# timlawrenz/DINO-X

Measured on AMD Instinct MI355X. Metric: training images/sec (source samples; 2 global views each) ViT-S/16 224px bs256/GPU, higher is better.
Workload: dtype bf16; 1 GPU; ViT-S/16 224x224x3 2.5D slice stacks, scale-aware, 2 views/sample, DINO+Gram loss, AdamW+EMA; per_gpu_batch=256, global_batch=256, local_crops=0, out_dim=8192, parallelism=dp1, hipgraph=False

## Files before the change

### dino-x_amd/csrc/block.hip

```cpp
#include <cstring>

#include "common.h"

using namespace dinox;

namespace {

dinox_gemm_args gemm_args(const void* A, const void* B, void* C, int64_t M, int64_t N, int64_t K, int out_dtype) {
  dinox_gemm_args g;
  memset(&g, 0, sizeof g);
  g.A = A; g.B = B; g.C = C;
  g.M = M; g.N = N; g.K = K;
  g.lda = K; g.ldb = K; g.ldc = N;
  g.batch = 1;
  g.strideC = M * N;
  g.in_dtype = DINOX_BF16;
  g.out_dtype = out_dtype;
  g.alpha = 1.0f;
  g.ldr = N;
  g.ldaux = N;
  return g;
}

int weight_grad(const void* dy, const void* x, float* dw, float* db, int64_t M, int64_t n_out, int64_t n_in, void* ws, int64_t ws_bytes, void* stream) {
  dinox_gemm_args g;
  memset(&g, 0, sizeof g);
  g.A = dy; g.B = x; g.C = dw;
  g.M = n_out; g.N = n_in; g.K = M;
  g.lda = n_out; g.ldb = n_in; g.ldc = n_in;
  g.batch = 1;
  g.strideC = n_out * n_in;
  g.transA = 1; g.transB = 1;
  g.in_dtype = DINOX_BF16;
  g.out_dtype = DINOX_F32;
  g.epilogue = DINOX_EPI_ACCUM;
  g.alpha = 1.0f;
  g.ldr = n_in;
  g.ldaux = n_in;
  g.colsum = db;
  const int64_t need = dinox_gemm_ws_bytes(&g);
  if (need > 0) {
    DX_REQUIRE(ws && need <= ws_bytes, DINOX_EINVAL, "block_backward: tn_ws of %lld bytes, the dW product [%lld x %lld] over %lld rows needs %lld",
               (long long)ws_bytes, (long long)n_out, (long long)n_in, (long long)M, (long long)need);
    g.ws = ws;
  }
  return dinox_gemm(&g, stream);
}

}

#define BLK_TRY(call)        \
  do {                       \
    const int rc_ = (call);  \
    if (rc_) return rc_;     \
  } while (0)

extern "C" int dinox_block_forward(const dinox_block_fwd_args* a, void* stream) {
  DX_REQUIRE(a, DINOX_EINVAL, "block_forward: null args");
  DX_REQUIRE(a->V > 0 && a->N > 0 && a->D > 0 && a->H > 0 && a->heads > 0 && a->D % a->heads == 0, DINOX_EINVAL,
             "block_forward: V=%lld N=%lld D=%d H=%d heads=%d", (long long)a->V, (long long)a->N, a->D, a->H, a->heads);
  DX_REQUIRE(a->x0 && a->o && a->x1 && a->xn2 && a->mean2 && a->rstd2 && a->act && a->x2, DINOX_EINVAL, "block_forward: null activation");
  DX_REQUIRE(a->qkv ? a->lse != nullptr : !a->train, DINOX_EINVAL, "block_forward: qkv / lse buffers (only a no-grad pass may leave qkv out)");
  DX_REQUIRE(a->n1w && a->n1b && a->n2w && a->n2b && a->wqkv && a->wproj && a->w1 && a->w2, DINOX_EINVAL, "block_forward: null parameter");
  DX_REQUIRE(a->xn1_in ? (a->mean1_in && a->rstd1_in) : (a->xn1 && a->mean1 && a->rstd1), DINOX_EINVAL, "block_forward: norm1 buffers");
  DX_REQUIRE(!a->next_g || (a->next_b && a->yn && a->meann && a->rstdn), DINOX_EINVAL, "block_forward: next LayerNorm buffers");
  DX_REQUIRE(!a->train || a->pre, DINOX_EINVAL, "block_forward: train without the side tensor");
  const int64_t M = a->V * a->N;
  const int D = a->D, H = a->H;
  const void* xn1 = a->xn1_in;
  if (!xn1) {
    BLK_TRY(dinox_layernorm_fwd(a->x0, a->n1w, a->n1b, a->xn1, a->mean1, a->rstd1, M, D, a->eps, DINOX_BF16, stream));
    xn1 = a->xn1;
  }
  if (!a->qkv) {
    BLK_TRY(dinox_qkv_attention_fwd(xn1, a->wqkv, a->bqkv, a->o, nullptr, a->lse, (int)a->V, (int)a->N, a->heads, D / a->heads, D, stream));
  } else {
    dinox_gemm_args g = gemm_args(xn1, a->wqkv, a->qkv, M, 3 * (int64_t)D, D, DINOX_BF16);
    if (a->bqkv) { g.epilogue |= DINOX_EPI_BIAS; g.bias = a->bqkv; }
    BLK_TRY(dinox_gemm(&g, stream));
    BLK_TRY(dinox_attention_fwd(a->qkv, a->o, a->lse, (int)a->V, (int)a->N, a->heads, D / a->heads, DINOX_BF16, stream));
  }
  if (a->fuse_proj_ln) {
    BLK_TRY(dinox_linear_residual_ln(a->o, a->wproj, a->bproj, a->x0, a->x1, a->n2w, a->n2b, a->eps, a->xn2, DINOX_BF16, a->mean2, a->rstd2, M, D, D, stream));
  } else {
    dinox_gemm_args g = gemm_args(a->o, a->wproj, a->x1, M, D, D, DINOX_F32);
    g.epilogue = DINOX_EPI_RESIDUAL | (a->bproj ? DINOX_EPI_BIAS : 0);
    g.bias = a->bproj;
    g.residual = a->x0;
    BLK_TRY(dinox_gemm(&g, stream));
    BLK_TRY(dinox_layernorm_fwd(a->x1, a->n2w, a->n2b, a->xn2, a->mean2, a->rstd2, M, D, a->eps, DINOX_BF16, stream));
  }
  {
    dinox_gemm_args g = gemm_args(a->xn2, a->w1, a->act, M, H, D, DINOX_BF16);
    g.epilogue = DINOX_EPI_GELU | DINOX_EPI_AUXGRAD | (a->b1 ? DINOX_EPI_BIAS : 0);
    g.bias = a->b1;
    g.aux = a->train ? a->pre : nullptr;
    BLK_TRY(dinox_gemm(&g, stream));
  }
  if (a->next_g && a->fuse_fc2_ln) {
    BLK_TRY(dinox_linear_residual_ln(a->act, a->w2, a->b2, a->x1, a->x2, a->next_g, a->next_b, a->next_eps, a->yn, a->next_dtype, a->meann, a->rstdn, M, D, H, stream));
  } else {
    dinox_gemm_args g = gemm_args(a->act, a->w2, a->x2, M, D, H, DINOX_F32);
    g.epilogue = DINOX_EPI_RESIDUAL | (a->b2 ? DINOX_EPI_BIAS : 0);
    g.bias = a->b2;
    g.residual = a->x1;
    BLK_TRY(dinox_gemm(&g, stream));
    if (a->next_g) BLK_TRY(dinox_layernorm_fwd(a->x2, a->next_g, a->next_b, a->yn, a->meann, a->rstdn, M, D, a->next_eps, a->next_dtype, stream));
  }
  return 0;
}

extern "C" int dinox_block_backward(const dinox_block_bwd_args* a, void* stream) {
  DX_REQUIRE(a, DINOX_EINVAL, "block_backward: null args");
  DX_REQUIRE(a->V > 0 && a->N > 0 && a->D > 0 && a->H > 0 && a->heads > 0 && a->D % a->heads == 0, DINOX_EINVAL,
             "block_backward: V=%lld N=%lld D=%d H=%d heads=%d", (long long)a->V, (long long)a->N, a->D, a->H, a->heads);
  DX_REQUIRE(a->g && (a->g_lowp || a->g_lowp_buf), DINOX_EINVAL, "block_backward: gradient");
  DX_REQUIRE(a->x0 && a->x1 && a->xn1 && a->xn2 && a->qkv && a->o && a->lse && a->pre && a->act && a->mean1 && a->rstd1 && a->mean2 && a->rstd2, DINOX_EINVAL,
             "block_backward: null saved tensor");
  DX_REQUIRE(a->n1w && a->n2w && a->wqkv_t && a->wproj_t && a->w1_t && a->w2_t, DINOX_EINVAL, "block_backward: null parameter");
  DX_REQUIRE(a->dwqkv && a->dwproj && a->dw1 && a->dw2 && a->dn1w && a->dn1b && a->dn2w && a->dn2b, DINOX_EINVAL, "block_backward: null gradient slice");
  DX_REQUIRE(a->dpre && a->dxn2 && a->d_o && a->dqkv && a->dxn1 && a->g1 && a->g1_lowp && a->g0_lowp && a->attn_ws && a->ln_ws, DINOX_EINVAL,
             "block_backward: null scratch");
  const int64_t M = a->V * a->N;
  const int D = a->D, H = a->H;
  const void* g_op = a->g_lowp;
  if (!g_op) {
    BLK_TRY(dinox_cast_bf16(a->g, a->g_lowp_buf, M * D, stream));
    g_op = a->g_lowp_buf;
  }
  {
    dinox_gemm_args g = gemm_args(g_op, a->w2_t, a->dpre, M, H, D, DINOX_BF16);
    g.epilogue = DINOX_EPI_DGELU | DINOX_EPI_AUXGRAD;
    g.aux = const_cast<void*>(a->pre);
    BLK_TRY(dinox_gemm(&g, stream));
  }
  BLK_TRY(weight_grad(g_op, a->act, a->dw2, a->db2, M, D, H, a->tn_ws, a->tn_ws_bytes, stream));
  const bool fuse_ln = (a->reserved & 1) != 0;
  if (!fuse_ln) {
    dinox_gemm_args g = gemm_args(a->dpre, a->w1_t, a->dxn2, M, D, H, DINOX_BF16);
    BLK_TRY(dinox_gemm(&g, stream));
  }
  BLK_TRY(weight_grad(a->dpre, a->xn2, a->dw1, a->db1, M, H, D, a->tn_ws, a->tn_ws_bytes, stream));
  if (fuse_ln)
    BLK_TRY(dinox_linear_ln_bwd(a->dpre, a->w1_t, a->x1, a->n2w, a->mean2, a->rstd2, a->g1, a->g, a->g1_lowp, a->dn2w, a->dn2b, a->ln_ws, M, (int)D,
                                (int)H, 1, stream));
  else
    BLK_TRY(dinox_layernorm_bwd(a->dxn2, a->x1, a->n2w, a->mean2, a->rstd2, a->g1, a->g, a->g1_lowp, a->dn2w, a->dn2b, a->ln_ws, M, D, DINOX_BF16, 1, stream));
  {
    dinox_gemm_args g = gemm_args(a->g1_lowp, a->wproj_t, a->d_o, M, D, D, DINOX_BF16);
    BLK_TRY(dinox_gemm(&g, stream));
  }
  BLK_TRY(weight_grad(a->g1_lowp, a->o, a->dwproj, a->dbproj, M, D, D, a->tn_ws, a->tn_ws_bytes, stream));
  BLK_TRY(dinox_attention_bwd(a->d_o, a->qkv, a->o, a->lse, a->dqkv, a->attn_ws, (int)a->V, (int)a->N, a->heads, D / a->heads, DINOX_BF16, stream));
  if (!fuse_ln) {
    dinox_gemm_args g = gemm_args(a->dqkv, a->wqkv_t, a->dxn1, M, D, 3 * (int64_t)D, DINOX_BF16);
    BLK_TRY(dinox_gemm(&g, stream));
  }
  BLK_TRY(weight_grad(a->dqkv, a->xn1, a->dwqkv, a->dbqkv, M, 3 * (int64_t)D, D, a->tn_ws, a->tn_ws_bytes, stream));
  if (fuse_ln)
    BLK_TRY(dinox_linear_ln_bwd(a->dqkv, a->wqkv_t, a->x0, a->n1w, a->mean1, a->rstd1, a->g1, a->g1, a->g0_lowp, a->dn1w, a->dn1b, a->ln_ws, M, (int)D,
                                3 * (int)D, 1, stream));
  else
    BLK_TRY(dinox_layernorm_bwd(a->dxn1, a->x0, a->n1w, a->mean1, a->rstd1, a->g1, a->g1, a->g0_lowp, a->dn1w, a->dn1b, a->ln_ws, M, D, DINOX_BF16, 1, stream));
  return 0;
}
```

### dino-x_amd/csrc/gemm.hip

```cpp
#include <cstring>

#include "common.h"
#include "kernels.h"

namespace dinox {

template <int DT>
__global__ __launch_bounds__(1024) void colsum_kernel(const void* __restrict__ x, float* __restrict__ out, int64_t M,
                                                      int64_t N, int64_t ldx, int accumulate) {
  __shared__ float red[16][64];
  const int c = threadIdx.x & 63, g = threadIdx.x >> 6;
  const int64_t n = (int64_t)blockIdx.x * 64 + c;
  float s0 = 0.f, s1 = 0.f, s2 = 0.f, s3 = 0.f;
  if (n < N) {
    int64_t r = g;
    for (; r + 48 < M; r += 64) {
      s0 += elem<DT>::ld(x, r * ldx + n);
      s1 += elem<DT>::ld(x, (r + 16) * ldx + n);
      s2 += elem<DT>::ld(x, (r + 32) * ldx + n);
      s3 += elem<DT>::ld(x, (r + 48) * ldx + n);
    }
    for (; r < M; r += 16) s0 += elem<DT>::ld(x, r * ldx + n);
  }
  red[g][c] = (s0 + s1) + (s2 + s3);
  __syncthreads();
  if (g == 0 && n < N) {
    float t[16];
#pragma unroll
    for (int k = 0; k < 16; ++k) t[k] = red[k][c];
    const float v = (((t[0] + t[1]) + (t[2] + t[3])) + ((t[4] + t[5]) + (t[6] + t[7]))) +
                    (((t[8] + t[9]) + (t[10] + t[11])) + ((t[12] + t[13]) + (t[14] + t[15])));
    out[n] = (accumulate ? out[n] : 0.f) + v;
  }
}

}

using namespace dinox;

#include <map>
#include <mutex>
#include <string>
#include <tuple>
#include <vector>
namespace {
struct TimerRec {
  int64_t launches = 0;
  std::vector<std::pair<hipEvent_t, hipEvent_t>> ev;
};
typedef std::tuple<std::string, int64_t, int64_t, int64_t, int64_t, int, int, int, int, int> TimerKey;
std::mutex g_timer_mu;
bool g_timer_on = false;
int g_timer_every = 16;
uint64_t g_timer_n = 0;
std::map<TimerKey, TimerRec> g_timer;
std::vector<hipEvent_t> g_timer_pool;

hipEvent_t timer_event() {
  if (!g_timer_pool.empty()) {
    hipEvent_t e = g_timer_pool.back();
    g_timer_pool.pop_back();
    return e;
  }
  hipEvent_t e = nullptr;
  (void)hipEventCreate(&e);
  return e;
}
}

static void to_params(const dinox_gemm_args* a, GemmParams& p) {
  p.A = a->A; p.B = a->B; p.C = a->C;
  p.M = a->M; p.N = a->N; p.K = a->K;
  p.lda = a->lda; p.ldb = a->ldb; p.ldc = a->ldc;
  p.batch = a->batch; p.strideA = a->strideA; p.strideB = a->strideB; p.strideC = a->strideC;
  p.transA = a->transA ? 1 : 0; p.transB = a->transB ? 1 : 0;
  p.in_dtype = a->in_dtype; p.out_dtype = a->out_dtype; p.epilogue = a->epilogue;
  p.alpha = a->alpha;
  p.bias = a->bias; p.residual = a->residual; p.ldr = a->ldr; p.aux = a->aux; p.ldaux = a->ldaux;
  p.colsum = a->colsum;
  p.ws = a->ws;
}

extern "C" int64_t dinox_gemm_ws_bytes(const dinox_gemm_args* a) {
  if (!a || a->M <= 0 || a->N <= 0 || a->K <= 0 || a->batch < 1) return 0;
  GemmParams p;
  to_params(a, p);
  return p.in_dtype == DINOX_BF16 ? gemm_bf16_ws_bytes(p) : 0;
}

extern "C" const char* dinox_gemm_kernel_name(const dinox_gemm_args* a) {
  if (!a) return "";
  GemmParams p;
  to_params(a, p);
  const char* v = gemm_variant_name(gemm_bf16_variant(p));
  return v ? v : "gemm_f32";
}

extern "C" int dinox_gemm(const dinox_gemm_args* a, void* stream) {
  DX_REQUIRE(a, DINOX_EINVAL, "gemm: null args");
  DX_REQUIRE(a->A && a->B && a->C, DINOX_EINVAL, "gemm: null operand");
  DX_REQUIRE(a->M > 0 && a->N > 0 && a->K > 0 && a->batch >= 1, DINOX_EINVAL, "gemm: M=%lld N=%lld K=%lld batch=%lld",
             (long long)a->M, (long long)a->N, (long long)a->K, (long long)a->batch);
  DX_REQUIRE((a->in_dtype == DINOX_F32 || a->in_dtype == DINOX_BF16) && (a->out_dtype == DINOX_F32 || a->out_dtype == DINOX_BF16),
             DINOX_EINVAL, "gemm: dtype in=%d out=%d", a->in_dtype, a->out_dtype);
  DX_REQUIRE(a->lda >= (a->transA ? a->M : a->K) && a->ldb >= (a->transB ? a->N : a->K) && a->ldc >= a->N, DINOX_EINVAL,
             "gemm: leading dimension too small (lda=%lld ldb=%lld ldc=%lld)", (long long)a->lda, (long long)a->ldb, (long long)a->ldc);
  const int e = a->epilogue;
  DX_REQUIRE(!(e & DINOX_EPI_BIAS) || a->bias, DINOX_EINVAL, "gemm: BIAS without bias pointer");
  DX_REQUIRE(!(e & DINOX_EPI_RESIDUAL) || (a->residual && a->ldr >= a->N), DINOX_EINVAL, "gemm: RESIDUAL without residual/ldr");
  DX_REQUIRE(!(e & DINOX_EPI_DGELU) || (a->aux && a->ldaux >= a->N), DINOX_EINVAL, "gemm: DGELU without aux/ldaux");
  DX_REQUIRE(!(e & DINOX_EPI_GELU) || !a->aux || a->ldaux >= a->N, DINOX_EINVAL, "gemm: GELU aux ldaux too small");
  DX_REQUIRE(!((e & DINOX_EPI_GELU) && (e & DINOX_EPI_DGELU)), DINOX_EINVAL, "gemm: GELU and DGELU are exclusive");
  DX_REQUIRE(!(e & DINOX_EPI_ACCUM) || a->out_dtype == DINOX_F32, DINOX_EINVAL, "gemm: ACCUM needs fp32 C");
  DX_REQUIRE(!a->colsum || (a->transA && a->batch == 1), DINOX_EINVAL, "gemm: colsum needs transA=1 and batch=1");
  GemmParams p;
  to_params(a, p);
  hipStream_t st = as_stream(stream);
  hipEvent_t e1 = nullptr;
  if (g_timer_on) {
    std::lock_guard<std::mutex> lk(g_timer_mu);
    if (g_timer_on) {
      const char* v = gemm_variant_name(gemm_bf16_variant(p));
      TimerRec& r = g_timer[TimerKey(v ? v : "gemm_f32", p.M, p.N, p.K, p.batch, p.epilogue, p.in_dtype, p.out_dtype,
                                     (p.aux && (p.epilogue & (DINOX_EPI_GELU | DINOX_EPI_DGELU))) ? 1 : 0, (p.batch > 1 && p.strideB == 0) ? 1 : 0)];
      r.launches++;
      ++g_timer_n;
      if (g_timer_every <= 1 || (((g_timer_n * 2654435761ull) & 0xffffffffull) * (uint64_t)g_timer_every >> 32) == 0) {
        hipEvent_t e0 = timer_event();
        e1 = timer_event();
        if (e0 && e1) {
          (void)hipEventRecord(e0, st);
          r.ev.emplace_back(e0, e1);
        } else {
          e1 = nullptr;
        }
      }
    }
  }
  int rc = DINOX_EUNSUPPORTED;
  if (p.in_dtype == DINOX_BF16) rc = launch_gemm_bf16(p, st);
  if (rc == DINOX_EUNSUPPORTED) {
    rc = 0;
    if (p.colsum)
      rc = dinox_colsum(p.A, p.colsum, p.K, p.M, p.lda, p.in_dtype, (p.epilogue & DINOX_EPI_ACCUM) ? 1 : 0, stream);
    if (!rc) rc = launch_gemm_f32(p, st);
  }
  if (e1) (void)hipEventRecord(e1, st);
  return rc;
}

extern "C" int dinox_gemm_timer_start(int every) {
  std::lock_guard<std::mutex> lk(g_timer_mu);
  for (auto& kv : g_timer)
    for (auto& pr : kv.second.ev) {
      g_timer_pool.push_back(pr.first);
      g_timer_pool.push_back(pr.second);
    }
  g_timer.clear();
  g_timer_every = every < 1 ? 1 : every;
  g_timer_n = 0;
  g_timer_on = true;
  return 0;
}

extern "C" int64_t dinox_gemm_timer_stop(char* buf, int64_t buflen) {
  std::lock_guard<std::mutex> lk(g_timer_mu);
  g_timer_on = false;
  std::string out;
  char line[512];
  for (auto& kv : g_timer) {
    double ms = 0.0;
    int64_t timed = 0;
    for (auto& pr : kv.second.ev) {
      float t = 0.f;
      if (hipEventSynchronize(pr.second) == hipSuccess && hipEventElapsedTime(&t, pr.first, pr.second) == hipSuccess) {
        ms += t;
        ++timed;
      }
      g_timer_pool.push_back(pr.first);
      g_timer_pool.push_back(pr.second);
    }
    const TimerKey& k = kv.first;
    snprintf(line, sizeof line, "%s %lld %lld %lld %lld %d %d %d %d %d %lld %lld %.6f\n", std::get<0>(k).c_str(), (long long)std::get<1>(k),
             (long long)std::get<2>(k), (long long)std::get<3>(k), (long long)std::get<4>(k), std::get<5>(k), std::get<6>(k), std::get<7>(k),
             std::get<8>(k), std::get<9>(k), (long long)kv.second.launches, (long long)timed, ms);
    out += line;
  }
  g_timer.clear();
  if (!buf || (int64_t)out.size() + 1 > buflen) return -1;
  memcpy(buf, out.c_str(), out.size() + 1);
  return (int64_t)out.size();
}

extern "C" int dinox_colsum(const void* x, float* out, int64_t M, int64_t N, int64_t ldx, int dtype, int accumulate,
                            void* stream) {
  DX_REQUIRE(x && out, DINOX_EINVAL, "colsum: null pointer");
  DX_REQUIRE(M > 0 && N > 0 && ldx >= N, DINOX_EINVAL, "colsum: M=%lld N=%lld ldx=%lld", (long long)M, (long long)N, (long long)ldx);
  DX_REQUIRE(dtype == DINOX_F32 || dtype == DINOX_BF16, DINOX_EINVAL, "colsum: dtype %d", dtype);
  hipStream_t st = as_stream(stream);
  dim3 grid((unsigned)ceil_div(N, 64));
  if (dtype == DINOX_F32)
    hipLaunchKernelGGL((colsum_kernel<DINOX_F32>), grid, dim3(1024), 0, st, x, out, M, N, ldx, accumulate ? 1 : 0);
  else
    hipLaunchKernelGGL((colsum_kernel<DINOX_BF16>), grid, dim3(1024), 0, st, x, out, M, N, ldx, accumulate ? 1 : 0);
  return check_launch("colsum");
}
```

### dino-x_amd/csrc/gemm_bf16.hip

```cpp
#include "common.h"
#include "kernels.h"

namespace dinox {

constexpr int GB_BM = 128, GB_BN = 128, GB_BK = 64, GB_THREADS = 256;
constexpr int GB_TILE_BYTES = 128 * 64 * 2;

typedef __attribute__((address_space(3))) s16x4 lds_s16x4;

__device__ __forceinline__ uint4 ldg16(const bf16_t* p) { return *reinterpret_cast<const uint4*>(p); }

__device__ __forceinline__ int xcd_remap(int bid, int nwg) {
  const int q = nwg >> 3, r = nwg & 7, xcd = bid & 7, idx = bid >> 3;
  return (xcd < r ? xcd * (q + 1) : r * (q + 1) + (xcd - r) * q) + idx;
}

struct NtStage {
  uint4 a[4], b[4];
};

__device__ __forceinline__ void nt_load(NtStage& s, const bf16_t* __restrict__ A, const bf16_t* __restrict__ B, int64_t lda,
                                        int64_t ldb, int64_t m0, int64_t n0, int64_t k0, int64_t M, int64_t N, int64_t K) {
  const int c = threadIdx.x & 7, r0 = threadIdx.x >> 3;
  const int64_t k = k0 + c * 8;
// ... 130 lines not shown
  const int o0 = k0 * 256 + ((((colb >> 6) ^ (k0 & 3)) << 6) | (colb & 63));
  const int o1 = k1 * 256 + ((((colb >> 6) ^ (k1 & 3)) << 6) | (colb & 63));
  const s16x4 lo = __builtin_amdgcn_ds_read_tr16_b64_v4i16((lds_s16x4*)(tile + o0));
  const s16x4 hi = __builtin_amdgcn_ds_read_tr16_b64_v4i16((lds_s16x4*)(tile + o1));
  s16x8 v;
  v[0] = lo[0]; v[1] = lo[1]; v[2] = lo[2]; v[3] = lo[3];
  v[4] = hi[0]; v[5] = hi[1]; v[6] = hi[2]; v[7] = hi[3];
  return __builtin_bit_cast(bf16x8, v);
}

template <int OUT_DT>
__global__ __launch_bounds__(GB_THREADS, 2) void gemm_bf16_tn(GemmParams p, int tiles_m, int tiles_n, int splits,
                                                              int64_t k_per_split) {
  extern __shared__ __attribute__((aligned(16))) char smem[];
  const int lane = threadIdx.x & 63, wv = threadIdx.x >> 6;
  const int wr = wv >> 1, wc = wv & 1;
  const int ntile = tiles_m * tiles_n;
  const int wid = xcd_remap(blockIdx.x, ntile * splits);
  const int split = wid / ntile, tile = wid % ntile;
  const int tm = tile / tiles_n, tn = tile % tiles_n;
  const int64_t m0 = (int64_t)tm * GB_BM, n0 = (int64_t)tn * GB_BN;
  const int64_t bz = blockIdx.y;
  const int64_t kbeg = (int64_t)split * k_per_split;
  int64_t kend = kbeg + k_per_split;
  if (kend > p.K) kend = p.K;
  const bf16_t* A = (const bf16_t*)p.A + bz * p.strideA;
  const bf16_t* B = (const bf16_t*)p.B + bz * p.strideB;

  f32x16 acc[2][2];
#pragma unroll
  for (int i = 0; i < 2; ++i)
#pragma unroll
    for (int j = 0; j < 2; ++j)
#pragma unroll
      for (int e = 0; e < 16; ++e) acc[i][j][e] = 0.f;

  const int nk = kend > kbeg ? (int)ceil_div(kend - kbeg, GB_BK) : 0;
  const bool cs_wave = p.colsum != nullptr && wc == 0;
  f32x16 csacc[2];
#pragma unroll
  for (int i = 0; i < 2; ++i)
#pragma unroll
    for (int e = 0; e < 16; ++e) csacc[i][e] = 0.f;
  s16x8 ones_s;
#pragma unroll
  for (int j = 0; j < 8; ++j) ones_s[j] = (short)0x3F80;
  const bf16x8 ones = __builtin_bit_cast(bf16x8, ones_s);
  TnStage st;
  if (nk > 0) {
    tn_load(st, A, B, p.lda, p.ldb, m0, n0, kbeg, kend, p.M, p.N);
    tn_store(st, smem, smem + GB_TILE_BYTES);
  }
  __syncthreads();
  for (int kt = 0; kt < nk; ++kt) {
    const int cur = kt & 1;
    const char* sa = smem + cur * 2 * GB_TILE_BYTES;
    const char* sb = sa + GB_TILE_BYTES;
    if (kt + 1 < nk) tn_load(st, A, B, p.lda, p.ldb, m0, n0, kbeg + (int64_t)(kt + 1) * GB_BK, kend, p.M, p.N);
#pragma unroll
    for (int ks = 0; ks < 4; ++ks) {
      bf16x8 af[2], bfr[2];
#pragma unroll
      for (int i = 0; i < 2; ++i) {
        af[i] = tn_frag(sa, ks * 16, wr * 64 + i * 32, lane);
        bfr[i] = tn_frag(sb, ks * 16, wc * 64 + i * 32, lane);
      }
#pragma unroll
      for (int i = 0; i < 2; ++i)
#pragma unroll
        for (int j = 0; j < 2; ++j) acc[i][j] = __builtin_amdgcn_mfma_f32_32x32x16_bf16(af[i], bfr[j], acc[i][j], 0, 0, 0);
      if (cs_wave && (kt % tiles_n) == tn) {
        csacc[0] = __builtin_amdgcn_mfma_f32_32x32x16_bf16(af[0], ones, csacc[0], 0, 0, 0);
        csacc[1] = __builtin_amdgcn_mfma_f32_32x32x16_bf16(af[1], ones, csacc[1], 0, 0, 0);
      }
    }
    if (kt + 1 < nk) {
      char* na = smem + (cur ^ 1) * 2 * GB_TILE_BYTES;
      tn_store(st, na, na + GB_TILE_BYTES);
    }
    __syncthreads();
  }

  const bool det = p.ws != nullptr && splits > 1;
  if (cs_wave && (lane & 31) == 0) {
    float* csp = det ? (float*)p.ws + (int64_t)splits * p.M * p.N + ((int64_t)split * tiles_n + tn) * p.M : nullptr;
#pragma unroll
    for (int i = 0; i < 2; ++i)
#pragma unroll
      for (int e = 0; e < 16; ++e) {
        const int64_t m = m0 + wr * 64 + i * 32 + (e & 3) + 8 * (e >> 2) + 4 * (lane >> 5);
        if (m < p.M) {
          if (det) csp[m] = csacc[i][e];
          else atomicAdd(p.colsum + m, csacc[i][e]);
        }
      }
  }

#pragma unroll
  for (int j = 0; j < 2; ++j) {
    const int64_t n = n0 + wc * 64 + j * 32 + (lane & 31);
    if (n >= p.N) continue;
    const float bias = (p.epilogue & DINOX_EPI_BIAS) ? p.bias[n] : 0.f;
#pragma unroll
    for (int i = 0; i < 2; ++i) {
#pragma unroll
      for (int e = 0; e < 16; ++e) {
        const int64_t m = m0 + wr * 64 + i * 32 + (e & 3) + 8 * (e >> 2) + 4 * (lane >> 5);
        if (m >= p.M) continue;
        if (det)
          ((float*)p.ws)[((int64_t)split * p.M + m) * p.N + n] = acc[i][j][e];
        else if (splits > 1)
          atomicAdd((float*)p.C + bz * p.strideC + m * p.ldc + n, acc[i][j][e] * p.alpha);
        else
          epilogue_store<OUT_DT>(p, bz, m, n, acc[i][j][e], bias);
      }
    }
  }
}

typedef __attribute__((address_space(3))) void lds_void_t;

template <int OUT_DT>
__global__ __launch_bounds__(GB_THREADS, 2) void gemm_bf16_tn_dma(GemmParams p, int tiles_m, int tiles_n, int splits, int64_t k_per_split) {
  extern __shared__ __attribute__((aligned(16))) char smem[];
  const int lane = threadIdx.x & 63, wv = threadIdx.x >> 6;
  const int wr = wv >> 1, wc = wv & 1;
  const int ntile = tiles_m * tiles_n;
  const int wid = xcd_remap(blockIdx.x, ntile * splits);
  const int split = wid / ntile, tile = wid % ntile;
  const int tm = tile / tiles_n, tn = tile % tiles_n;
  const int64_t m0 = (int64_t)tm * GB_BM, n0 = (int64_t)tn * GB_BN;
  const int64_t bz = blockIdx.y;
  const int64_t kbeg = (int64_t)split * k_per_split;
  int64_t kend = kbeg + k_per_split;
  if (kend > p.K) kend = p.K;
  const bf16_t* A = (const bf16_t*)p.A + bz * p.strideA;
  const bf16_t* B = (const bf16_t*)p.B + bz * p.strideB;

  f32x16 acc[2][2];
#pragma unroll
  for (int i = 0; i < 2; ++i)
#pragma unroll
    for (int j = 0; j < 2; ++j)
#pragma unroll
      for (int e = 0; e < 16; ++e) acc[i][j][e] = 0.f;

  const int nk = kend > kbeg ? (int)ceil_div(kend - kbeg, GB_BK) : 0;
  const bool cs_wave = p.colsum != nullptr && wc == 0;
  f32x16 csacc[2];
#pragma unroll
  for (int i = 0; i < 2; ++i)
#pragma unroll
    for (int e = 0; e < 16; ++e) csacc[i][e] = 0.f;
  s16x8 ones_s;
#pragma unroll
  for (int j = 0; j < 8; ++j) ones_s[j] = (short)0x3F80;
  const bf16x8 ones = __builtin_bit_cast(bf16x8, ones_s);
  const int wvu = __builtin_amdgcn_readfirstlane(wv);
  const auto rsA = __builtin_amdgcn_make_buffer_rsrc((void*)A, 0, (int)(p.K * p.lda * 2), 0x00020000);
  const auto rsB = __builtin_amdgcn_make_buffer_rsrc((void*)B, 0, (int)(p.K * p.ldb * 2), 0x00020000);
  unsigned voffA[4], voffB[4];
#pragma unroll
  for (int q = 0; q < 4; ++q) {
    const int r = (wvu * 4 + q) * 4 + (lane >> 4);
    const int cp = lane & 15;
    const int c = (((cp >> 2) ^ (r & 3)) << 2) | (cp & 3);
    int64_t ma = m0 + c * 8, nb = n0 + c * 8;
    ma = ma < p.M ? ma : p.M - 8;
    nb = nb < p.N ? nb : p.N - 8;
    voffA[q] = (unsigned)(((kbeg + r) * p.lda + ma) * 2);
    voffB[q] = (unsigned)(((kbeg + r) * p.ldb + nb) * 2);
  }
  const unsigned stepA = (unsigned)(GB_BK * p.lda * 2), stepB = (unsigned)(GB_BK * p.ldb * 2);
  auto stage = [&](int buf, int kt) {
    char* sa = smem + buf * 2 * GB_TILE_BYTES + wvu * 4096;
    char* sb = sa + GB_TILE_BYTES;
#pragma unroll
    for (int q = 0; q < 4; ++q) {
      __builtin_amdgcn_raw_ptr_buffer_load_lds(rsA, (lds_void_t*)(sa + q * 1024), 16, voffA[q] + kt * stepA, 0, 0, 0);
      __builtin_amdgcn_raw_ptr_buffer_load_lds(rsB, (lds_void_t*)(sb + q * 1024), 16, voffB[q] + kt * stepB, 0, 0, 0);
    }
  };
  if (nk > 0) stage(0, 0);
  __syncthreads();
  for (int kt = 0; kt < nk; ++kt) {
    const int cur = kt & 1;
    const char* sa = smem + cur * 2 * GB_TILE_BYTES;
    const char* sb = sa + GB_TILE_BYTES;
    if (kt + 1 < nk) stage(cur ^ 1, kt + 1);
#pragma unroll
    for (int ks = 0; ks < 4; ++ks) {
      bf16x8 af[2], bfr[2];
#pragma unroll
      for (int i = 0; i < 2; ++i) {
        af[i] = tn_frag(sa, ks * 16, wr * 64 + i * 32, lane);
        bfr[i] = tn_frag(sb, ks * 16, wc * 64 + i * 32, lane);
      }
#pragma unroll
      for (int i = 0; i < 2; ++i)
#pragma unroll
        for (int j = 0; j < 2; ++j) acc[i][j] = __builtin_amdgcn_mfma_f32_32x32x16_bf16(af[i], bfr[j], acc[i][j], 0, 0, 0);
      if (cs_wave && (kt % tiles_n) == tn) {
        csacc[0] = __builtin_amdgcn_mfma_f32_32x32x16_bf16(af[0], ones, csacc[0], 0, 0, 0);
        csacc[1] = __builtin_amdgcn_mfma_f32_32x32x16_bf16(af[1], ones, csacc[1], 0, 0, 0);
      }
    }
    __syncthreads();
  }

  const bool det = p.ws != nullptr && splits > 1;
  if (cs_wave && (lane & 31) == 0) {
    float* csp = det ? (float*)p.ws + (int64_t)splits * p.M * p.N + ((int64_t)split * tiles_n + tn) * p.M : nullptr;
#pragma unroll
    for (int i = 0; i < 2; ++i)
#pragma unroll
      for (int e = 0; e < 16; ++e) {
        const int64_t m = m0 + wr * 64 + i * 32 + (e & 3) + 8 * (e >> 2) + 4 * (lane >> 5);
        if (m < p.M) {
          if (det) csp[m] = csacc[i][e];
          else atomicAdd(p.colsum + m, csacc[i][e]);
        }
      }
  }

#pragma unroll
  for (int j = 0; j < 2; ++j) {
    const int64_t n = n0 + wc * 64 + j * 32 + (lane & 31);
    if (n >= p.N) continue;
    const float bias = (p.epilogue & DINOX_EPI_BIAS) ? p.bias[n] : 0.f;
#pragma unroll
    for (int i = 0; i < 2; ++i) {
#pragma unroll
      for (int e = 0; e < 16; ++e) {
        const int64_t m = m0 + wr * 64 + i * 32 + (e & 3) + 8 * (e >> 2) + 4 * (lane >> 5);
        if (m >= p.M) continue;
        if (det)
          ((float*)p.ws)[((int64_t)split * p.M + m) * p.N + n] = acc[i][j][e];
        else if (splits > 1)
          atomicAdd((float*)p.C + bz * p.strideC + m * p.ldc + n, acc[i][j][e] * p.alpha);
        else
          epilogue_store<OUT_DT>(p, bz, m, n, acc[i][j][e], bias);
      }
    }
  }
}

__global__ __launch_bounds__(256) void tn_reduce_kernel(const float* __restrict__ part, int splits, int64_t MN, float alpha, float* __restrict__ C,
                                                       int accumulate, const float* __restrict__ cs_part, int cs_terms, int64_t M,
                                                       float* __restrict__ colsum, int c_blocks) {
  __shared__ float4 red[4][64];
  const int l = threadIdx.x & 63, g = threadIdx.x >> 6;
  if ((int)blockIdx.x < c_blocks) {
    const int64_t n4 = MN >> 2, i = (int64_t)blockIdx.x * 64 + l;
    const int per = (splits + 3) >> 2, s_lo = g * per, s_hi = s_lo + per < splits ? s_lo + per : splits;
    float4 a = make_float4(0.f, 0.f, 0.f, 0.f);
    if (i < n4) {
      for (int s0 = s_lo; s0 < s_hi; s0 += 8) {
        float4 b[8];
#pragma unroll
        for (int u = 0; u < 8; ++u)
          b[u] = s0 + u < s_hi ? reinterpret_cast<const float4*>(part + (int64_t)(s0 + u) * MN)[i] : make_float4(0.f, 0.f, 0.f, 0.f);
#pragma unroll
        for (int u = 0; u < 8; ++u) {
          a.x += b[u].x; a.y += b[u].y; a.z += b[u].z; a.w += b[u].w;
        }
      }
    }
    red[g][l] = a;
    __syncthreads();
    if (g == 0 && i < n4) {
      const float4 r0 = red[0][l], r1 = red[1][l], r2 = red[2][l], r3 = red[3][l];
      float4 c = accumulate ? reinterpret_cast<const float4*>(C)[i] : make_float4(0.f, 0.f, 0.f, 0.f);
      c.x += alpha * ((r0.x + r1.x) + (r2.x + r3.x));
      c.y += alpha * ((r0.y + r1.y) + (r2.y + r3.y));
      c.z += alpha * ((r0.z + r1.z) + (r2.z + r3.z));
      c.w += alpha * ((r0.w + r1.w) + (r2.w + r3.w));
      reinterpret_cast<float4*>(C)[i] = c;
    }
    if (blockIdx.x == 0 && threadIdx.x < (MN & 3)) {
      const int64_t j = (n4 << 2) + threadIdx.x;
      float t = 0.f;
      for (int s2 = 0; s2 < splits; ++s2) t += part[(int64_t)s2 * MN + j];
      C[j] = (accumulate ? C[j] : 0.f) + alpha * t;
    }
  } else {
    const int64_t m = (int64_t)((int)blockIdx.x - c_blocks) * 64 + l;
    const int per = (cs_terms + 3) >> 2, t_lo = g * per, t_hi = t_lo + per < cs_terms ? t_lo + per : cs_terms;
    float a = 0.f;
    if (m < M) {
      for (int t0 = t_lo; t0 < t_hi; t0 += 8) {
        float b[8];
#pragma unroll
        for (int u = 0; u < 8; ++u) b[u] = t0 + u < t_hi ? cs_part[(int64_t)(t0 + u) * M + m] : 0.f;
#pragma unroll
        for (int u = 0; u < 8; ++u) a += b[u];
      }
    }
    red[g][l].x = a;
    __syncthreads();
    if (g == 0 && m < M) colsum[m] = (accumulate ? colsum[m] : 0.f) + ((red[0][l].x + red[1][l].x) + (red[2][l].x + red[3][l].x));
  }
}

static int launch_tn_reduce(const GemmParams& p, int splits, int tiles_n, hipStream_t st) {
  const int64_t MN = p.M * p.N;
  const int c_blocks = (int)ceil_div(MN >> 2, (int64_t)64);
  const int cs_blocks = p.colsum ? (int)ceil_div(p.M, (int64_t)64) : 0;
  const float* part = (const float*)p.ws;
  hipLaunchKernelGGL(tn_reduce_kernel, dim3((unsigned)(c_blocks + cs_blocks)), dim3(256), 0, st, part, splits, MN, p.alpha, (float*)p.C,
                     (p.epilogue & DINOX_EPI_ACCUM) ? 1 : 0, part + (int64_t)splits * MN, splits * tiles_n, p.M, p.colsum, c_blocks);
  return check_launch("gemm_bf16_tn_reduce");
}

static void tn_split_plan(const GemmParams& p, int& splits, int64_t& kps) {
  const int tiles_m = (int)ceil_div(p.M, GB_BM), tiles_n = (int)ceil_div(p.N, GB_BN);
  const int64_t ntile = (int64_t)tiles_m * tiles_n;
  splits = 1;
  const bool plain = (p.epilogue & ~DINOX_EPI_ACCUM) == 0 && p.out_dtype == DINOX_F32;
  if (plain) {
    const int64_t slots = 512, have = ntile * p.batch;
    splits = (int)(slots / have);
    const int64_t max_splits = ceil_div(p.K, 4 * GB_BK);
    if (splits > max_splits) splits = (int)max_splits;
    if (splits < 1) splits = 1;
  }
  kps = ceil_div(ceil_div(p.K, splits), GB_BK) * GB_BK;
  splits = (int)ceil_div(p.K, kps);
}

static bool aligned16(const void* p) { return (((uintptr_t)p) & 15) == 0; }

static GemmVariant nt_pp_choice(const GemmParams& p) {
  using V = GemmVariant;
  if (p.transA || p.transB) return V::None;
  const int mode = knob_int("DINOX_NT_PP", -1);
  if (mode == 0) return V::None;
  const bool ok256 = gemm_bf16_nt_pp_ok(p), ok128 = gemm_bf16_nt_pp128_ok(p);
  {
    const int m3 = knob_int("DINOX_NT_PP384", -1);
    if (m3 != 0 && mode != 2 && mode != 3 && gemm_bf16_nt_pp384_ok(p) &&
        (m3 > 0 || (p.out_dtype == DINOX_BF16 && !(p.epilogue & DINOX_EPI_RESIDUAL) && p.K >= 768 && p.M >= 8192)))
      return V::NtPp384;
  }
  if (mode == 2) return ok128 ? V::NtPp128 : V::None;
  if (mode == 3) return ok256 ? V::NtPp : V::None;
  const int64_t rem = p.N % 256;
  const bool narrow = p.N < 1024 && rem != 0 && rem <= 128;
  const V pick = narrow ? (ok128 ? V::NtPp128 : V::None) : (ok256 ? V::NtPp : V::None);
  if (mode >= 1 || pick == V::None) return pick;
  const int64_t units = ceil_div(p.M, (int64_t)256) * ceil_div(p.N, (int64_t)(narrow ? 128 : 256));
  if (narrow) {
    if (p.K >= 768) return units >= 192 ? pick : V::None;
    return (units >= 1024 && !(p.epilogue & DINOX_EPI_RESIDUAL)) ? pick : V::None;
  }
  if ((p.epilogue & DINOX_EPI_GELU) && p.K < 768) {
    if (knob_int("DINOX_FC1_AREG", 0) != 0 || units < 1024) return V::None;
  }
  return units >= 192 ? pick : V::None;
}

GemmVariant gemm_bf16_variant(const GemmParams& p) {
  using V = GemmVariant;
  if (p.in_dtype != DINOX_BF16) return V::None;
  if (!aligned16(p.A) || !aligned16(p.B) || (p.lda & 7) || (p.ldb & 7) || (p.strideA & 7) || (p.strideB & 7)) return V::None;
  if (const V pp = nt_pp_choice(p); pp != V::None) return pp;
  if (gemm_bf16_nt_glds_ok(p)) {
    const int64_t maxk = knob_int("DINOX_NT_AREG_MAXK", 576);
    static const bool no_areg = knob_set("DINOX_NT_NO_AREG");
    return !no_areg && p.K <= maxk && gemm_bf16_nt_areg_ok(p) ? V::NtAreg : V::NtGlds;
  }
  if (p.transA == 0 && p.transB == 0 && (p.K & 7) == 0) return V::Nt;
  if (p.transA == 1 && p.transB == 1 && (p.M & 7) == 0 && (p.N & 7) == 0) {
    if (p.ws) {
      int a, b, c;
      int64_t d;
      if (tn_big_plan(p, a, b, c, d)) return V::TnBig;
    }
    const bool small = p.K * p.lda * 2 < (int64_t)0x7fffffff && p.K * p.ldb * 2 < (int64_t)0x7fffffff && p.M >= 8 && p.N >= 8;
    return small ? V::TnDma : V::Tn;
  }
  return V::None;
}

static bool tn_det_ok(const GemmParams& p, GemmVariant variant, int splits) {
  return variant == GemmVariant::TnDma && splits > 1 && p.batch == 1 && p.ldc == p.N && p.out_dtype == DINOX_F32 &&
         (p.epilogue & ~DINOX_EPI_ACCUM) == 0;
}

int64_t gemm_bf16_ws_bytes(const GemmParams& p) {
  if (const int64_t big = tn_big_ws_bytes(p)) return big;
  const GemmVariant v = gemm_bf16_variant(p);
  if (v != GemmVariant::TnBig && v != GemmVariant::TnDma && v != GemmVariant::Tn) return 0;
  int splits;
  int64_t kps;
  tn_split_plan(p, splits, kps);
  if (!tn_det_ok(p, v, splits)) return 0;
  const int tiles_n = (int)ceil_div(p.N, GB_BN);
  return ((int64_t)splits * p.M * p.N + (p.colsum ? (int64_t)splits * tiles_n * p.M : 0)) * (int64_t)sizeof(float);
}

int launch_gemm_bf16(const GemmParams& p, hipStream_t st) {
  using V = GemmVariant;
  const V v = gemm_bf16_variant(p);
  switch (v) {
    case V::None: return DINOX_EUNSUPPORTED;
    case V::NtPp: return launch_gemm_bf16_nt_pp(p, st);
    case V::NtPp128: return launch_gemm_bf16_nt_pp128(p, st);
    case V::NtPp384: return launch_gemm_bf16_nt_pp384(p, st);
    case V::NtAreg: return launch_gemm_bf16_nt_areg(p, st);
    case V::NtGlds: return launch_gemm_bf16_nt_glds(p, st);
    case V::Nt: case V::TnBig: case V::TnDma: case V::Tn: break;
  }
  const int tiles_m = (int)ceil_div(p.M, GB_BM), tiles_n = (int)ceil_div(p.N, GB_BN);
  const int64_t ntile = (int64_t)tiles_m * tiles_n;
  if (ntile > 0x7fffffff || p.batch > 65535) return DINOX_EUNSUPPORTED;
  const size_t lds = 4 * GB_TILE_BYTES;
  const bool f32 = p.out_dtype == DINOX_F32;
  if (v == V::Nt) {
    dim3 grid((unsigned)ntile, (unsigned)p.batch);
    hipLaunchKernelGGL((f32 ? gemm_bf16_nt<DINOX_F32> : gemm_bf16_nt<DINOX_BF16>), grid, dim3(GB_THREADS), lds, st, p, tiles_m, tiles_n);
    return check_launch("gemm_bf16_nt");
  }
  if (v == V::TnBig) {
    int sp = 1, tn_ = 1;
    if (int rc = launch_gemm_bf16_tn_big(p, st, sp, tn_)) return rc;
    return launch_tn_reduce(p, sp, tn_, st);
  }
  int splits;
  int64_t kps;
  tn_split_plan(p, splits, kps);
  GemmParams q = p;
  const bool det = q.ws != nullptr && tn_det_ok(p, v, splits);
  if (!det) q.ws = nullptr;
  if (!det && splits > 1 && !(p.epilogue & DINOX_EPI_ACCUM)) {
    if (p.ldc == p.N && (p.batch == 1 || p.strideC == p.M * p.N)) {
      hipError_t e = hipMemsetAsync(p.C, 0, (size_t)p.batch * p.M * p.N * sizeof(float), st);
      if (e != hipSuccess) return fail((int)e, "gemm_bf16_tn: memset: %s", hipGetErrorString(e));
    } else {
      splits = 1;
      kps = ceil_div(p.K, GB_BK) * GB_BK;
    }
  }
  if (!det && p.colsum && !(p.epilogue & DINOX_EPI_ACCUM)) {
    hipError_t e = hipMemsetAsync(p.colsum, 0, (size_t)p.M * sizeof(float), st);
    if (e != hipSuccess) return fail((int)e, "gemm_bf16_tn: memset colsum: %s", hipGetErrorString(e));
  }
  if (ntile * splits > 0x7fffffff) return DINOX_EUNSUPPORTED;
  dim3 grid((unsigned)(ntile * splits), (unsigned)p.batch);
  const auto kern = v == V::TnDma ? (f32 ? gemm_bf16_tn_dma<DINOX_F32> : gemm_bf16_tn_dma<DINOX_BF16>) : (f32 ? gemm_bf16_tn<DINOX_F32> : gemm_bf16_tn<DINOX_BF16>);
  hipLaunchKernelGGL(kern, grid, dim3(GB_THREADS), lds, st, q, tiles_m, tiles_n, splits, kps);
  if (int rc = check_launch(gemm_variant_name(v))) return rc;
  if (det) return launch_tn_reduce(p, splits, tiles_n, st);
  return 0;
}

}
```

### dino-x_amd/csrc/kernels.h

```cpp
#pragma once
#include <type_traits>

#include "gemm_common.h"
#include "knobs.h"

namespace dinox {

#define GEMM_VARIANTS(X)                                                                                                       \
  X(NtPp, "gemm_bf16_nt_pp") X(NtPp128, "gemm_bf16_nt_pp128") X(NtPp384, "gemm_bf16_nt_pp384") X(NtAreg, "gemm_bf16_nt_areg") \
  X(NtGlds, "gemm_bf16_nt_glds") X(Nt, "gemm_bf16_nt") X(TnBig, "gemm_bf16_tn_big") X(TnDma, "gemm_bf16_tn_dma") X(Tn, "gemm_bf16_tn")
#define X(member, name) member,
enum class GemmVariant { None, GEMM_VARIANTS(X) };
#undef X
#define X(member, name) name,
inline const char* gemm_variant_name(GemmVariant v) {
  static const char* const names[] = {nullptr, GEMM_VARIANTS(X)};
  return names[(int)v];
}
#undef X

int launch_gemm_f32(const GemmParams& p, hipStream_t st);
GemmVariant gemm_bf16_variant(const GemmParams& p);
int launch_gemm_bf16(const GemmParams& p, hipStream_t st);
int64_t gemm_bf16_ws_bytes(const GemmParams& p);
bool gemm_bf16_nt_glds_ok(const GemmParams& p);
int launch_gemm_bf16_nt_glds(const GemmParams& p, hipStream_t st);
bool gemm_bf16_nt_areg_ok(const GemmParams& p);
int launch_gemm_bf16_nt_areg(const GemmParams& p, hipStream_t st);
bool gemm_bf16_nt_pp_ok(const GemmParams& p);
int launch_gemm_bf16_nt_pp(const GemmParams& p, hipStream_t st);
bool gemm_bf16_nt_pp128_ok(const GemmParams& p);
int launch_gemm_bf16_nt_pp128(const GemmParams& p, hipStream_t st);
bool gemm_bf16_nt_pp384_ok(const GemmParams& p);
int launch_gemm_bf16_nt_pp384(const GemmParams& p, hipStream_t st);
bool gemm_bf16_nt_pp384_ln_ok(int64_t M, int K);
int launch_gemm_bf16_nt_pp384_ln(const void* a, const void* w, const float* bias, const float* residual, float* x_out, const float* gamma,
                                 const float* beta, float eps, void* y, float* mean, float* rstd, int64_t M, int K, hipStream_t st);
int pp384_lnbwd_tiles(int64_t M);
int launch_gemm_bf16_nt_pp384_lnbwd(const void* a, const void* w, const float* x, const float* gamma, const float* mean, const float* rstd,
                                    float* dx, const float* dx_add, void* dx_lowp, float* ws, int64_t M, int K, hipStream_t st);
int tn_big_plan(const GemmParams& p, int& tiles_m, int& tiles_n, int& splits, int64_t& kps);
int64_t tn_big_ws_bytes(const GemmParams& p);
int launch_gemm_bf16_tn_big(const GemmParams& p, hipStream_t st, int& splits_out, int& tiles_n_out);

int launch_attention_ref_fwd(const void* qkv, void* o, float* lse, int B, int N, int heads, int d, int dtype, hipStream_t st);
int launch_attention_ref_bwd(const void* d_o, const void* qkv, const void* o, const float* lse, void* dqkv, int B, int N, int heads, int d, int dtype, hipStream_t st);
int launch_attention_bf16_fwd(const void* qkv, void* o, float* lse, int B, int N, int heads, int d, hipStream_t st);
int launch_attention_bf16_bwd(const void* d_o, const void* qkv, const void* o, const float* lse, void* dqkv, float* ws, int B, int N, int heads, int d, hipStream_t st);
bool attention_qkv_fused_ok(int B, int N, int heads, int d, int D);
int launch_attention_qkv_fused_fwd(const void* x, const void* w, const float* bias, void* o, void* qkv_out, float* lse, int B, int N, int heads, int d, int D, hipStream_t st);
int launch_attention_flash_fwd(const void* qkv, void* o, float* lse, int B, int N, int heads, int d, hipStream_t st);
int launch_attention_flash_bwd(const void* d_o, const void* qkv, const void* o, const float* lse, void* dqkv, float* ws, int B, int N, int heads, int d, hipStream_t st);

int launch_ntxent_rows(const float* S, int64_t lds, int M, float inv_tau, float* lse, float* row_loss, float* loss, hipStream_t st);
int launch_ntxent_coeff(const float* S, int64_t lds, const float* lse, int M, float inv_tau, float gscale, float* W, int64_t ldw, hipStream_t st);
int launch_normalize_bwd(const float* dxh, const float* xh, const float* norm, float* dx, int64_t V, int D, float eps, hipStream_t st);

bool attention_rows_ok(int B, int N, int heads, int d, int Q);
int launch_attention_rows(const void* qkv, const int* query_idx, float* probs, float* lse, int B, int N, int heads, int d, int Q, int dtype,
                          hipStream_t st);

bool attention_rollout_step_ok(int B, int N, int heads, int d);
size_t attention_rollout_step_ws_bytes(int B, int N, int heads);
int launch_attention_rollout_step(const void* qkv, const float* w_in, float* w_out, void* ws, int B, int N, int heads, int d, float residual,
                                  int dtype, hipStream_t st);

constexpr int MAE_MAX_L = 4096;
constexpr int MAE_MAX_PATCH = 32;
int launch_mae_mask_ids(const float* noise, int* ids_restore, int* ids_keep, int V, int L, int Lk, hipStream_t st);
int launch_mae_gather_unfold(const float* x, const int* ids_keep, void* u, int V, int H, int W, int patch, int Lk, int ld, int dtype,
                             hipStream_t st);
int launch_mae_tokens_fwd(const void* patches, const float* cls, const float* pos, const int* ids_keep, float* tok, int V, int L, int Lk,
                          int D, int dtype, hipStream_t st);
int launch_mae_tokens_bwd(const float* dtok, const int* ids_restore, void* dpatches, float* dcls, float* dpos, int V, int L, int Lk, int D,
                          int dtype, hipStream_t st);
int launch_mae_unshuffle_fwd(const void* e, const float* mask_token, const float* dpe, const int* ids_restore, float* xd, int V, int L,
                             int Lk, int D, int dtype, hipStream_t st);
int launch_mae_unshuffle_bwd(const float* g, const int* ids_keep, const int* ids_restore, void* de, float* dmask, float* ws, int V, int L,
                             int Lk, int D, int dtype, hipStream_t st);
int launch_mae_loss_fwd(const void* pred, const float* x, const int* ids_restore, float* loss, float* ws, int V, int H, int W, int patch,
                        int Lk, int lead, int dtype, hipStream_t st);
int launch_mae_loss_bwd(const void* pred, const float* x, const int* ids_restore, void* dpred, float gscale, int V, int H, int W, int patch,
                        int Lk, int lead, int dtype, int out_dtype, hipStream_t st);

enum { EPI_ACT_PLAIN = 0, EPI_ACT_GELU = 1, EPI_ACT_DGELU = 2 };

template <typename F>
static inline int with_epilogue_case(const GemmParams& p, F&& f) {
  const int act = (p.epilogue & DINOX_EPI_GELU) ? EPI_ACT_GELU : (p.epilogue & DINOX_EPI_DGELU) ? EPI_ACT_DGELU : EPI_ACT_PLAIN;
  const bool res = (p.epilogue & DINOX_EPI_RESIDUAL) != 0;
  auto cases = [&](auto out) -> int {
    switch (act * 2 + (res ? 1 : 0)) {
      case 0: return f(out, std::integral_constant<int, EPI_ACT_PLAIN>{}, std::false_type{});
      case 1: return f(out, std::integral_constant<int, EPI_ACT_PLAIN>{}, std::true_type{});
      case 2: return f(out, std::integral_constant<int, EPI_ACT_GELU>{}, std::false_type{});
      case 4: return f(out, std::integral_constant<int, EPI_ACT_DGELU>{}, std::false_type{});
      default: return DINOX_EUNSUPPORTED;
    }
  };
  return p.out_dtype == DINOX_BF16 ? cases(std::integral_constant<int, DINOX_BF16>{}) : cases(std::integral_constant<int, DINOX_F32>{});
}

struct PersistPlan {
  int tiles_n, units, order, stagger;
  unsigned grid;
};
static inline bool persist_plan(const GemmParams& p, int bm, int bn, int stagger_auto, PersistPlan& pl) {
  const int64_t tiles_n = ceil_div(p.N, (int64_t)bn), units = ceil_div(p.M, (int64_t)bm) * tiles_n;
  if (units > 0x3fffffff) return false;
  const int64_t ncu = device_cu_count();
  pl = {(int)tiles_n, (int)units, knob_int("DINOX_PP_ORDER", 1), knob_int("DINOX_PP_STAGGER", stagger_auto), (unsigned)(units < ncu ? units : ncu)};
  return true;
}

}
```

### dino-x_amd/csrc/layernorm.hip

```cpp
#include "common.h"
#include "kernels.h"

namespace dinox {

constexpr int LN_THREADS = 256;
constexpr int LN_MAXV = 8;
constexpr int LN_MAX_PARTS = 1024;

template <int OUT_DT, int NV>
__global__ __launch_bounds__(LN_THREADS) void ln_fwd_kernel(const float* __restrict__ x, const float* __restrict__ w,
                                                            const float* __restrict__ b, void* __restrict__ y,
                                                            float* __restrict__ mean, float* __restrict__ rstd,
                                                            int64_t rows, int dim, float eps) {
  const int lane = threadIdx.x & 63;
  const int64_t wave = (int64_t)blockIdx.x * (LN_THREADS / 64) + (threadIdx.x >> 6);
  const int64_t nwaves = (int64_t)gridDim.x * (LN_THREADS / 64);
  const int nvec = dim >> 2;
  const float inv = 1.0f / (float)dim;
  for (int64_t r = wave; r < rows; r += nwaves) {
    const float4* xr = reinterpret_cast<const float4*>(x + r * dim);
    float4 v[NV];
    float s = 0.f;
#pragma unroll
    for (int j = 0; j < NV; ++j) {
// ... 74 lines not shown
    }
    const float rs = rsqrtf(sum32(q) * (1.0f / DIM) + eps);
    if (sl == 0) {
      mean[r] = mu;
      rstd[r] = rs;
    }
#pragma unroll
    for (int j = 0; j < 3; ++j) {
      float4 o;
      o.x = (v[j].x - mu) * rs * ww[j].x + bb[j].x;
      o.y = (v[j].y - mu) * rs * ww[j].y + bb[j].y;
      o.z = (v[j].z - mu) * rs * ww[j].z + bb[j].z;
      o.w = (v[j].w - mu) * rs * ww[j].w + bb[j].w;
      if (OUT_DT == DINOX_F32) {
        store_stream(reinterpret_cast<float4*>((float*)y + r * DIM) + (sl + 32 * j), o);
      } else {
        ushort4 p;
        p.x = f32_to_bf16(o.x);
        p.y = f32_to_bf16(o.y);
        p.z = f32_to_bf16(o.z);
        p.w = f32_to_bf16(o.w);
        store_stream(reinterpret_cast<ushort4*>((bf16_t*)y + r * DIM) + (sl + 32 * j), p);
      }
    }
  };
  for (int64_t r0 = half; r0 < rows; r0 += 2 * nhalves) {
    const int64_t r1 = r0 + nhalves;
    const bool two = r1 < rows;
    float4 v0[3], v1[3];
    const float4* x0 = reinterpret_cast<const float4*>(x + r0 * DIM);
    const float4* x1 = reinterpret_cast<const float4*>(x + (two ? r1 : r0) * DIM);
#pragma unroll
    for (int j = 0; j < 3; ++j) v0[j] = x0[sl + 32 * j];
#pragma unroll
    for (int j = 0; j < 3; ++j) v1[j] = x1[sl + 32 * j];
    finish(v0, r0);
    if (two) finish(v1, r1);
  }
}

template <int OUT_DT>
__global__ __launch_bounds__(LN_THREADS) void ln_fwd_generic(const float* __restrict__ x, const float* __restrict__ w,
                                                             const float* __restrict__ b, void* __restrict__ y,
                                                             float* __restrict__ mean, float* __restrict__ rstd,
                                                             int64_t rows, int dim, float eps) {
  const int lane = threadIdx.x & 63;
  const int64_t wave = (int64_t)blockIdx.x * (LN_THREADS / 64) + (threadIdx.x >> 6);
  const int64_t nwaves = (int64_t)gridDim.x * (LN_THREADS / 64);
  const float inv = 1.0f / (float)dim;
  for (int64_t r = wave; r < rows; r += nwaves) {
    const float* xr = x + r * dim;
    float s = 0.f;
    for (int c = lane; c < dim; c += 64) s += xr[c];
    const float mu = wave_sum(s) * inv;
    float q = 0.f;
    for (int c = lane; c < dim; c += 64) {
      const float d = xr[c] - mu;
      q += d * d;
    }
    const float rs = rsqrtf(wave_sum(q) * inv + eps);
    if (lane == 0) {
      mean[r] = mu;
      rstd[r] = rs;
    }
    for (int c = lane; c < dim; c += 64) elem<OUT_DT>::st(y, r * dim + c, (xr[c] - mu) * rs * w[c] + b[c]);
  }
}

template <int DY_DT, int NV>
__global__ __launch_bounds__(LN_THREADS) void ln_bwd_kernel(const void* __restrict__ dy, const float* __restrict__ x,
                                                            const float* __restrict__ w, const float* __restrict__ mean,
                                                            const float* __restrict__ rstd, float* dx,
                                                            void* __restrict__ dx_lowp, float* __restrict__ ws,
                                                            int64_t rows, int dim, const float* dx_add) {
  extern __shared__ __attribute__((aligned(16))) float lds[];
  const int lane = threadIdx.x & 63, wv = threadIdx.x >> 6;
  const int64_t wave = (int64_t)blockIdx.x * (LN_THREADS / 64) + wv;
  const int64_t nwaves = (int64_t)gridDim.x * (LN_THREADS / 64);
  const int nvec = dim >> 2;
  const float inv = 1.0f / (float)dim;
  float4 aw[NV], ab[NV], wreg[NV];
#pragma unroll
  for (int j = 0; j < NV; ++j) {
    aw[j] = make_float4(0.f, 0.f, 0.f, 0.f);
    ab[j] = make_float4(0.f, 0.f, 0.f, 0.f);
    const int c = lane + 64 * j;
    wreg[j] = (c < nvec) ? reinterpret_cast<const float4*>(w)[c] : make_float4(0.f, 0.f, 0.f, 0.f);
  }
  for (int64_t r = wave; r < rows; r += nwaves) {
    const float mu = mean[r], rs = rstd[r];
    float4 xh[NV], g[NV], add[NV];
    float s1 = 0.f, s2 = 0.f;
#pragma unroll
    for (int j = 0; j < NV; ++j) {
      const int c = lane + 64 * j;
      add[j] = (dx_add && c < nvec) ? reinterpret_cast<const float4*>(dx_add + r * dim)[c] : make_float4(0.f, 0.f, 0.f, 0.f);
    }
#pragma unroll
    for (int j = 0; j < NV; ++j) {
      const int c = lane + 64 * j;
      float4 d = make_float4(0.f, 0.f, 0.f, 0.f), xv = make_float4(mu, mu, mu, mu);
      if (c < nvec) {
        xv = reinterpret_cast<const float4*>(x + r * dim)[c];
        if (DY_DT == DINOX_F32) {
          d = reinterpret_cast<const float4*>((const float*)dy + r * dim)[c];
        } else {
          const ushort4 p = reinterpret_cast<const ushort4*>((const bf16_t*)dy + r * dim)[c];
          d = make_float4(bf16_to_f32(p.x), bf16_to_f32(p.y), bf16_to_f32(p.z), bf16_to_f32(p.w));
        }
      }
      xh[j] = make_float4((xv.x - mu) * rs, (xv.y - mu) * rs, (xv.z - mu) * rs, (xv.w - mu) * rs);
      g[j] = make_float4(d.x * wreg[j].x, d.y * wreg[j].y, d.z * wreg[j].z, d.w * wreg[j].w);
      aw[j].x += d.x * xh[j].x; aw[j].y += d.y * xh[j].y; aw[j].z += d.z * xh[j].z; aw[j].w += d.w * xh[j].w;
      ab[j].x += d.x; ab[j].y += d.y; ab[j].z += d.z; ab[j].w += d.w;
      s1 += (g[j].x + g[j].y) + (g[j].z + g[j].w);
      s2 += (g[j].x * xh[j].x + g[j].y * xh[j].y) + (g[j].z * xh[j].z + g[j].w * xh[j].w);
    }
    const float m1 = wave_sum(s1) * inv, m2 = wave_sum(s2) * inv;
#pragma unroll
    for (int j = 0; j < NV; ++j) {
      const int c = lane + 64 * j;
      if (c < nvec) {
        float4 o;
        o.x = rs * (g[j].x - m1 - xh[j].x * m2);
        o.y = rs * (g[j].y - m1 - xh[j].y * m2);
        o.z = rs * (g[j].z - m1 - xh[j].z * m2);
        o.w = rs * (g[j].w - m1 - xh[j].w * m2);
        float4* dst = reinterpret_cast<float4*>(dx + r * dim) + c;
        o.x += add[j].x; o.y += add[j].y; o.z += add[j].z; o.w += add[j].w;
        store_stream(dst, o);
        if (dx_lowp) {
          ushort4 p;
          p.x = f32_to_bf16(o.x); p.y = f32_to_bf16(o.y); p.z = f32_to_bf16(o.z); p.w = f32_to_bf16(o.w);
          store_stream(reinterpret_cast<ushort4*>((bf16_t*)dx_lowp + r * dim) + c, p);
        }
      }
    }
  }
  float* mine = lds + (size_t)wv * 2 * dim;
#pragma unroll
  for (int j = 0; j < NV; ++j) {
    const int c = lane + 64 * j;
    if (c < nvec) {
      reinterpret_cast<float4*>(mine)[c] = aw[j];
      reinterpret_cast<float4*>(mine + dim)[c] = ab[j];
    }
  }
  __syncthreads();
  float* out = ws + (size_t)blockIdx.x * 2 * dim;
  for (int c = threadIdx.x; c < 2 * dim; c += LN_THREADS)
    out[c] = (lds[c] + lds[2 * dim + c]) + (lds[4 * dim + c] + lds[6 * dim + c]);
}

template <int DY_DT>
__global__ __launch_bounds__(LN_THREADS) void ln_bwd_384(const void* __restrict__ dy, const float* __restrict__ x,
                                                         const float* __restrict__ w, const float* __restrict__ mean,
                                                         const float* __restrict__ rstd, float* dx, void* __restrict__ dx_lowp,
                                                         float* __restrict__ ws, int64_t rows, const float* dx_add) {
  constexpr int DIM = 384;
  extern __shared__ __attribute__((aligned(16))) float lds[];
  const int lane = threadIdx.x & 63, sl = lane & 31, wv = threadIdx.x >> 6;
  const int64_t half = ((int64_t)blockIdx.x * (LN_THREADS / 64) + wv) * 2 + (lane >> 5);
  const int64_t nhalves = (int64_t)gridDim.x * (LN_THREADS / 64) * 2;
  float4 aw[3], ab[3], wreg[3];
#pragma unroll
  for (int j = 0; j < 3; ++j) {
    aw[j] = make_float4(0.f, 0.f, 0.f, 0.f);
    ab[j] = make_float4(0.f, 0.f, 0.f, 0.f);
    wreg[j] = reinterpret_cast<const float4*>(w)[sl + 32 * j];
  }
  auto sum32 = [](float v) {
#pragma unroll
    for (int o = 16; o > 0; o >>= 1) v += __shfl_xor(v, o, 64);
    return v;
  };
  auto fetch = [&](int64_t r, float4 (&xv)[3], float4 (&d)[3], float4 (&a)[3]) {
#pragma unroll
    for (int j = 0; j < 3; ++j) {
      const int c = sl + 32 * j;
      xv[j] = reinterpret_cast<const float4*>(x + r * DIM)[c];
      if (DY_DT == DINOX_F32) {
        d[j] = reinterpret_cast<const float4*>((const float*)dy + r * DIM)[c];
      } else {
        const ushort4 p = reinterpret_cast<const ushort4*>((const bf16_t*)dy + r * DIM)[c];
        d[j] = make_float4(bf16_to_f32(p.x), bf16_to_f32(p.y), bf16_to_f32(p.z), bf16_to_f32(p.w));
      }
      a[j] = dx_add ? reinterpret_cast<const float4*>(dx_add + r * DIM)[c] : make_float4(0.f, 0.f, 0.f, 0.f);
    }
  };
  auto finish = [&](int64_t r, const float4 (&xv)[3], const float4 (&d)[3], const float4 (&a)[3]) {
    const float mu = mean[r], rs = rstd[r];
    float4 xh[3], g[3];
    float s1 = 0.f, s2 = 0.f;
#pragma unroll
    for (int j = 0; j < 3; ++j) {
      xh[j] = make_float4((xv[j].x - mu) * rs, (xv[j].y - mu) * rs, (xv[j].z - mu) * rs, (xv[j].w - mu) * rs);
      g[j] = make_float4(d[j].x * wreg[j].x, d[j].y * wreg[j].y, d[j].z * wreg[j].z, d[j].w * wreg[j].w);
      aw[j].x += d[j].x * xh[j].x; aw[j].y += d[j].y * xh[j].y; aw[j].z += d[j].z * xh[j].z; aw[j].w += d[j].w * xh[j].w;
      ab[j].x += d[j].x; ab[j].y += d[j].y; ab[j].z += d[j].z; ab[j].w += d[j].w;
      s1 += (g[j].x + g[j].y) + (g[j].z + g[j].w);
      s2 += (g[j].x * xh[j].x + g[j].y * xh[j].y) + (g[j].z * xh[j].z + g[j].w * xh[j].w);
    }
    const float m1 = sum32(s1) * (1.0f / DIM), m2 = sum32(s2) * (1.0f / DIM);
#pragma unroll
    for (int j = 0; j < 3; ++j) {
      const int c = sl + 32 * j;
      float4 o;
      o.x = rs * (g[j].x - m1 - xh[j].x * m2) + a[j].x;
      o.y = rs * (g[j].y - m1 - xh[j].y * m2) + a[j].y;
      o.z = rs * (g[j].z - m1 - xh[j].z * m2) + a[j].z;
      o.w = rs * (g[j].w - m1 - xh[j].w * m2) + a[j].w;
      store_stream(reinterpret_cast<float4*>(dx + r * DIM) + c, o);
      if (dx_lowp) {
        ushort4 p;
        p.x = f32_to_bf16(o.x); p.y = f32_to_bf16(o.y); p.z = f32_to_bf16(o.z); p.w = f32_to_bf16(o.w);
        store_stream(reinterpret_cast<ushort4*>((bf16_t*)dx_lowp + r * DIM) + c, p);
      }
    }
  };
  for (int64_t r0 = half; r0 < rows; r0 += 2 * nhalves) {
    const int64_t r1 = r0 + nhalves;
    const bool two = r1 < rows;
    float4 x0[3], d0[3], a0[3], x1[3], d1[3], a1[3];
    fetch(r0, x0, d0, a0);
    fetch(two ? r1 : r0, x1, d1, a1);
    finish(r0, x0, d0, a0);
    if (two) finish(r1, x1, d1, a1);
  }
  float* mine = lds + (size_t)wv * 2 * DIM;
#pragma unroll
  for (int j = 0; j < 3; ++j) {
    float4 sw, sb;
    sw.x = aw[j].x + __shfl_xor(aw[j].x, 32, 64); sw.y = aw[j].y + __shfl_xor(aw[j].y, 32, 64);
    sw.z = aw[j].z + __shfl_xor(aw[j].z, 32, 64); sw.w = aw[j].w + __shfl_xor(aw[j].w, 32, 64);
    sb.x = ab[j].x + __shfl_xor(ab[j].x, 32, 64); sb.y = ab[j].y + __shfl_xor(ab[j].y, 32, 64);
    sb.z = ab[j].z + __shfl_xor(ab[j].z, 32, 64); sb.w = ab[j].w + __shfl_xor(ab[j].w, 32, 64);
    if (lane < 32) {
      reinterpret_cast<float4*>(mine)[sl + 32 * j] = sw;
      reinterpret_cast<float4*>(mine + DIM)[sl + 32 * j] = sb;
    }
  }
  __syncthreads();
  float* out = ws + (size_t)blockIdx.x * 2 * DIM;
  for (int c = threadIdx.x; c < 2 * DIM; c += LN_THREADS)
    out[c] = (lds[c] + lds[2 * DIM + c]) + (lds[4 * DIM + c] + lds[6 * DIM + c]);
}

template <int DY_DT>
__global__ __launch_bounds__(LN_THREADS) void ln_bwd_generic(const void* __restrict__ dy, const float* __restrict__ x,
                                                             const float* __restrict__ w, const float* __restrict__ mean,
                                                             const float* __restrict__ rstd, float* dx,
                                                             void* __restrict__ dx_lowp, float* __restrict__ ws,
                                                             int64_t rows, int dim, const float* dx_add) {
  extern __shared__ __attribute__((aligned(16))) float lds[];
  for (int c = threadIdx.x; c < 2 * dim; c += LN_THREADS) lds[c] = 0.f;
  __syncthreads();
  const int lane = threadIdx.x & 63;
  const int64_t wave = (int64_t)blockIdx.x * (LN_THREADS / 64) + (threadIdx.x >> 6);
  const int64_t nwaves = (int64_t)gridDim.x * (LN_THREADS / 64);
  const float inv = 1.0f / (float)dim;
  for (int64_t r = wave; r < rows; r += nwaves) {
    const float mu = mean[r], rs = rstd[r];
    float s1 = 0.f, s2 = 0.f;
    for (int c = lane; c < dim; c += 64) {
      const float d = elem<DY_DT>::ld(dy, r * dim + c), xh = (x[r * dim + c] - mu) * rs, g = d * w[c];
      s1 += g;
      s2 += g * xh;
      atomicAdd(&lds[c], d * xh);
      atomicAdd(&lds[dim + c], d);
    }
    const float m1 = wave_sum(s1) * inv, m2 = wave_sum(s2) * inv;
    for (int c = lane; c < dim; c += 64) {
      const float d = elem<DY_DT>::ld(dy, r * dim + c), xh = (x[r * dim + c] - mu) * rs;
      float o = rs * (d * w[c] - m1 - xh * m2);
      if (dx_add) o += dx_add[r * dim + c];
      dx[r * dim + c] = o;
      if (dx_lowp) ((bf16_t*)dx_lowp)[r * dim + c] = f32_to_bf16(o);
    }
  }
  __syncthreads();
  float* out = ws + (size_t)blockIdx.x * 2 * dim;
  for (int c = threadIdx.x; c < 2 * dim; c += LN_THREADS) out[c] = lds[c];
}

__global__ __launch_bounds__(256) void ln_bwd_reduce(const float* __restrict__ ws, float* __restrict__ dw, float* __restrict__ db,
                                                     int parts, int dim, int accumulate) {
  __shared__ float red[64][4];
  const int cl = threadIdx.x & 3, g = threadIdx.x >> 2;
  const int c = blockIdx.x * 4 + cl;
  float s = 0.f;
  if (c < 2 * dim)
    for (int p = g; p < parts; p += 64) s += ws[(size_t)p * 2 * dim + c];
  red[g][cl] = s;
  __syncthreads();
  if (g == 0 && c < 2 * dim) {
    float v = 0.f;
#pragma unroll
    for (int k = 0; k < 64; ++k) v += red[k][cl];
    float* dst = c < dim ? &dw[c] : &db[c - dim];
    *dst = (accumulate ? *dst : 0.f) + v;
  }
}

static int ln_parts(int64_t rows) {
  int64_t p = ceil_div(rows, LN_THREADS / 64);
  return (int)(p < LN_MAX_PARTS ? p : LN_MAX_PARTS);
}

static bool ln_use384() {
  static const bool no384 = knob_set("DINOX_LN_NO384");
  return !no384;
}

}

using namespace dinox;

extern "C" int dinox_layernorm_fwd(const float* x, const float* w, const float* b, void* y, float* mean, float* rstd,
                                   int64_t rows, int dim, float eps, int out_dtype, void* stream) {
  DX_REQUIRE(x && w && b && y && mean && rstd, DINOX_EINVAL, "layernorm_fwd: null pointer");
  DX_REQUIRE(rows > 0 && dim > 0, DINOX_EINVAL, "layernorm_fwd: rows=%lld dim=%d", (long long)rows, dim);
  DX_REQUIRE(out_dtype == DINOX_F32 || out_dtype == DINOX_BF16, DINOX_EINVAL, "layernorm_fwd: dtype %d", out_dtype);
  int64_t blocks = ceil_div(rows, LN_THREADS / 64);
  if (blocks > 256 * 16) blocks = 256 * 16;
  hipStream_t st = as_stream(stream);
  const bool fast = (dim % 4 == 0) && dim <= 256 * LN_MAXV;
  if (dim == 384 && ln_use384() && (((uintptr_t)x | (uintptr_t)y | (uintptr_t)w | (uintptr_t)b) & 15) == 0) {
    int64_t blk = ceil_div(rows, (int64_t)(LN_THREADS / 64) * 2 * 2);
    if (blk > 256 * 8) blk = 256 * 8;
    hipLaunchKernelGGL((out_dtype == DINOX_F32 ? ln_fwd_384<DINOX_F32> : ln_fwd_384<DINOX_BF16>), dim3((unsigned)blk), dim3(LN_THREADS), 0, st, x, w, b, y, mean, rstd, rows, eps);
    return check_launch("layernorm_fwd");
  }
#define LN_FWD(DT, NV) hipLaunchKernelGGL((ln_fwd_kernel<DT, NV>), dim3((unsigned)blocks), dim3(LN_THREADS), 0, st, x, w, b, y, mean, rstd, rows, dim, eps)
  if (fast) {
    const int nv = (int)ceil_div(dim / 4, 64);
    if (out_dtype == DINOX_F32) {
      if (nv <= 1) LN_FWD(DINOX_F32, 1); else if (nv <= 2) LN_FWD(DINOX_F32, 2); else if (nv <= 4) LN_FWD(DINOX_F32, 4); else LN_FWD(DINOX_F32, 8);
    } else {
      if (nv <= 1) LN_FWD(DINOX_BF16, 1); else if (nv <= 2) LN_FWD(DINOX_BF16, 2); else if (nv <= 4) LN_FWD(DINOX_BF16, 4); else LN_FWD(DINOX_BF16, 8);
    }
  } else {
    hipLaunchKernelGGL((out_dtype == DINOX_F32 ? ln_fwd_generic<DINOX_F32> : ln_fwd_generic<DINOX_BF16>), dim3((unsigned)blocks), dim3(LN_THREADS), 0, st, x, w, b, y, mean, rstd, rows, dim, eps);
  }
#undef LN_FWD
  return check_launch("layernorm_fwd");
}

extern "C" int64_t dinox_layernorm_bwd_ws_bytes(int64_t rows, int dim) {
  if (rows <= 0 || dim <= 0) return 0;
  return (int64_t)ln_parts(rows) * 2 * dim * (int64_t)sizeof(float);
}

extern "C" int dinox_layernorm_bwd(const void* dy, const float* x, const float* w, const float* mean, const float* rstd,
                                   float* dx, const float* dx_add, void* dx_lowp, float* dw, float* db, void* ws,
                                   int64_t rows, int dim, int dy_dtype, int accumulate, void* stream) {
  DX_REQUIRE(dy && x && w && mean && rstd && dx && dw && db && ws, DINOX_EINVAL, "layernorm_bwd: null pointer");
  DX_REQUIRE(rows > 0 && dim > 0, DINOX_EINVAL, "layernorm_bwd: rows=%lld dim=%d", (long long)rows, dim);
  DX_REQUIRE(dy_dtype == DINOX_F32 || dy_dtype == DINOX_BF16, DINOX_EINVAL, "layernorm_bwd: dtype %d", dy_dtype);
  const int parts = ln_parts(rows);
  hipStream_t st = as_stream(stream);
  const size_t lds = (size_t)(LN_THREADS / 64) * 2 * dim * sizeof(float);
  const bool fast = (dim % 4 == 0) && dim <= 256 * LN_MAXV && lds <= 64 * 1024;
  float* wsf = (float*)ws;
  const bool al16 = (((uintptr_t)x | (uintptr_t)dy | (uintptr_t)dx | (uintptr_t)dx_add | (uintptr_t)dx_lowp | (uintptr_t)w) & 15) == 0;
  if (dim == 384 && ln_use384() && al16) {
    const int64_t want = ceil_div(rows, (int64_t)(LN_THREADS / 64) * 2 * 2);
    const int nblk = (int)(want < parts ? want : (parts < 768 ? parts : 768));
    hipLaunchKernelGGL((dy_dtype == DINOX_F32 ? ln_bwd_384<DINOX_F32> : ln_bwd_384<DINOX_BF16>), dim3(nblk), dim3(LN_THREADS), lds, st, dy, x, w, mean, rstd, dx, dx_lowp, wsf, rows, dx_add);
    if (int rc = check_launch("layernorm_bwd")) return rc;
    hipLaunchKernelGGL(ln_bwd_reduce, dim3((unsigned)ceil_div(2 * dim, 4)), dim3(256), 0, st, wsf, dw, db, nblk, dim, accumulate ? 1 : 0);
    return check_launch("layernorm_bwd_reduce");
  }
#define LN_BWD(DT, NV) hipLaunchKernelGGL((ln_bwd_kernel<DT, NV>), dim3(parts), dim3(LN_THREADS), lds, st, dy, x, w, mean, rstd, dx, dx_lowp, wsf, rows, dim, dx_add)
  if (fast) {
    const int nv = (int)ceil_div(dim / 4, 64);
    if (dy_dtype == DINOX_F32) {
      if (nv <= 1) LN_BWD(DINOX_F32, 1); else if (nv <= 2) LN_BWD(DINOX_F32, 2); else if (nv <= 4) LN_BWD(DINOX_F32, 4); else LN_BWD(DINOX_F32, 8);
    } else {
      if (nv <= 1) LN_BWD(DINOX_BF16, 1); else if (nv <= 2) LN_BWD(DINOX_BF16, 2); else if (nv <= 4) LN_BWD(DINOX_BF16, 4); else LN_BWD(DINOX_BF16, 8);
    }
  } else {
    const size_t l2 = (size_t)2 * dim * sizeof(float);
    DX_REQUIRE(l2 <= 64 * 1024, DINOX_EUNSUPPORTED, "layernorm_bwd: dim %d too large", dim);
    hipLaunchKernelGGL((dy_dtype == DINOX_F32 ? ln_bwd_generic<DINOX_F32> : ln_bwd_generic<DINOX_BF16>), dim3(parts), dim3(LN_THREADS), l2, st, dy, x, w, mean, rstd, dx, dx_lowp, wsf, rows, dim, dx_add);
  }
#undef LN_BWD
  int rc = check_launch("layernorm_bwd");
  if (rc) return rc;
  hipLaunchKernelGGL(ln_bwd_reduce, dim3((unsigned)ceil_div(2 * dim, 4)), dim3(256), 0, st, wsf, dw, db, parts, dim, accumulate ? 1 : 0);
  return check_launch("layernorm_bwd_reduce");
}

extern "C" int dinox_linear_ln_bwd_ok(int64_t M, int N, int K) {
  return (N == 384 && gemm_bf16_nt_pp384_ln_ok(M, K) && pp384_lnbwd_tiles(M) <= ln_parts(M)) ? 1 : 0;
}

extern "C" int dinox_linear_ln_bwd(const void* a, const void* w, const float* x, const float* gamma, const float* mean, const float* rstd,
                                   float* dx, const float* dx_add, void* dx_lowp, float* dgamma, float* dbeta, void* ws, int64_t M, int N,
                                   int K, int accumulate, void* stream) {
  DX_REQUIRE(a && w && x && gamma && mean && rstd && dx && dgamma && dbeta && ws, DINOX_EINVAL, "linear_ln_bwd: null pointer");
  DX_REQUIRE(dinox_linear_ln_bwd_ok(M, N, K), DINOX_EUNSUPPORTED, "linear_ln_bwd: M=%lld N=%d K=%d", (long long)M, N, K);
  DX_REQUIRE((((uintptr_t)a | (uintptr_t)w | (uintptr_t)x | (uintptr_t)dx | (uintptr_t)dx_add | (uintptr_t)dx_lowp | (uintptr_t)gamma) & 15) == 0,
             DINOX_EALIGN, "linear_ln_bwd: operands must be 16-byte aligned");
  hipStream_t st = as_stream(stream);
  if (int rc = launch_gemm_bf16_nt_pp384_lnbwd(a, w, x, gamma, mean, rstd, dx, dx_add, dx_lowp, (float*)ws, M, K, st)) return rc;
  hipLaunchKernelGGL(ln_bwd_reduce, dim3((unsigned)ceil_div(2 * 384, 4)), dim3(256), 0, st, (const float*)ws, dgamma, dbeta, pp384_lnbwd_tiles(M), 384,
                     accumulate ? 1 : 0);
  return check_launch("linear_ln_bwd_reduce");
}
```

### dino-x_amd/dinox/_lib.py

```python
from __future__ import annotations

import ctypes as C
import os

import torch

_HERE = os.path.dirname(os.path.abspath(__file__))
LIB_PATH = os.environ.get("DINOX_LIB") or os.path.join(_HERE, "libdinox_hip.so")

F32, BF16, U16, I16 = 0, 1, 2, 3
FMT_HU_FLOAT, FMT_HU16_PNG, FMT_WINDOWED_FLOAT = 0, 1, 2
EUNSUPPORTED = -2
EPI_BIAS, EPI_GELU, EPI_DGELU, EPI_RESIDUAL, EPI_ACCUM, EPI_AUXGRAD = 1, 2, 4, 8, 16, 32

vp, i32, i64, f32 = C.c_void_p, C.c_int32, C.c_int64, C.c_float


class GemmArgs(C.Structure):
    _fields_ = [
        ("A", vp), ("B", vp), ("C", vp),
        ("M", i64), ("N", i64), ("K", i64),
        ("lda", i64), ("ldb", i64), ("ldc", i64),
        ("batch", i64), ("strideA", i64), ("strideB", i64), ("strideC", i64),
        ("transA", i32), ("transB", i32), ("in_dtype", i32), ("out_dtype", i32), ("epilogue", i32),
        ("alpha", f32),
        ("bias", vp), ("residual", vp), ("ldr", i64), ("aux", vp), ("ldaux", i64), ("colsum", vp), ("ws", vp),
    ]


class BlockFwdArgs(C.Structure):
    _fields_ = [
        ("V", i64), ("N", i64), ("D", i32), ("H", i32), ("heads", i32), ("train", i32), ("fuse_proj_ln", i32), ("fuse_fc2_ln", i32), ("eps", f32),
        ("x0", vp), ("xn1_in", vp), ("mean1_in", vp), ("rstd1_in", vp), ("xn1", vp), ("mean1", vp), ("rstd1", vp),
        ("qkv", vp), ("o", vp), ("lse", vp), ("x1", vp), ("xn2", vp), ("mean2", vp), ("rstd2", vp), ("act", vp), ("pre", vp), ("x2", vp),
        ("next_g", vp), ("next_b", vp), ("next_eps", f32), ("next_dtype", i32), ("yn", vp), ("meann", vp), ("rstdn", vp),
        ("n1w", vp), ("n1b", vp), ("n2w", vp), ("n2b", vp), ("wqkv", vp), ("wproj", vp), ("w1", vp), ("w2", vp),
        ("bqkv", vp), ("bproj", vp), ("b1", vp), ("b2", vp),
    ]


class BlockBwdArgs(C.Structure):
    _fields_ = [
        ("V", i64), ("N", i64), ("D", i32), ("H", i32), ("heads", i32), ("reserved", i32),
        ("g", vp), ("g_lowp", vp), ("g_lowp_buf", vp),
        ("x0", vp), ("x1", vp), ("xn1", vp), ("xn2", vp), ("qkv", vp), ("o", vp), ("lse", vp), ("pre", vp), ("act", vp),
        ("mean1", vp), ("rstd1", vp), ("mean2", vp), ("rstd2", vp), ("n1w", vp), ("n2w", vp),
        ("wqkv_t", vp), ("wproj_t", vp), ("w1_t", vp), ("w2_t", vp),
        ("dwqkv", vp), ("dbqkv", vp), ("dwproj", vp), ("dbproj", vp), ("dw1", vp), ("db1", vp), ("dw2", vp), ("db2", vp),
        ("dn1w", vp), ("dn1b", vp), ("dn2w", vp), ("dn2b", vp),
        ("dpre", vp), ("dxn2", vp), ("d_o", vp), ("dqkv", vp), ("dxn1", vp), ("g1", vp), ("g1_lowp", vp), ("g0_lowp", vp),
        ("attn_ws", vp), ("ln_ws", vp), ("tn_ws", vp), ("tn_ws_bytes", i64),
    ]


SIGNATURES = {
    "dinox_version": (i32, []),
    "dinox_last_error": (C.c_char_p, []),
    "dinox_device_ok": (i32, []),
    "dinox_gemm": (i32, [C.POINTER(GemmArgs), vp]),
    "dinox_gemm_kernel_name": (C.c_char_p, [C.POINTER(GemmArgs)]),
    "dinox_gemm_ws_bytes": (i64, [C.POINTER(GemmArgs)]),
    "dinox_colsum": (i32, [vp, vp, i64, i64, i64, i32, i32, vp]),
    "dinox_linear_residual_ln_ok": (i32, [i64, i32, i32]),
    "dinox_linear_residual_ln": (i32, [vp, vp, vp, vp, vp, vp, vp, f32, vp, i32, vp, vp, i64, i32, i32, vp]),
    "dinox_layernorm_fwd": (i32, [vp, vp, vp, vp, vp, vp, i64, i32, f32, i32, vp]),
    "dinox_layernorm_bwd_ws_bytes": (i64, [i64, i32]),
    "dinox_layernorm_bwd": (i32, [vp, vp, vp, vp, vp, vp, vp, vp, vp, vp, vp, i64, i32, i32, i32, vp]),
    "dinox_linear_ln_bwd_ok": (i32, [i64, i32, i32]),
    "dinox_linear_ln_bwd": (i32, [vp, vp, vp, vp, vp, vp, vp, vp, vp, vp, vp, vp, i64, i32, i32, i32, vp]),
    "dinox_attention_fwd": (i32, [vp, vp, vp, i32, i32, i32, i32, i32, vp]),
    "dinox_attention_bwd_ws_bytes": (i64, [i32, i32, i32]),
    "dinox_attention_bwd": (i32, [vp, vp, vp, vp, vp, vp, i32, i32, i32, i32, i32, vp]),
    "dinox_qkv_attention_ok": (i32, [i32, i32, i32, i32, i32]),
    "dinox_qkv_attention_fwd": (i32, [vp, vp, vp, vp, vp, vp, i32, i32, i32, i32, i32, vp]),
    "dinox_patch_unfold": (i32, [vp, vp, i32, i32, i32, i32, i32, vp]),
    "dinox_patch_unfold_ld": (i32, [vp, vp, i32, i32, i32, i32, i32, i32, vp]),
    "dinox_tokens_fwd": (i32, [vp, vp, vp, vp, vp, vp, i32, i32, i32, i32, i32, vp]),
    "dinox_tokens_bwd": (i32, [vp, vp, vp, vp, vp, vp, i32, i32, i32, i32, i32, vp]),
    "dinox_scale_embed_fwd": (i32, [vp] * 12 + [i32, i32, i32, f32, vp]),
    "dinox_scale_embed_bwd_ws_bytes": (i64, [i32, i32, i32]),
    "dinox_scale_embed_bwd": (i32, [vp] * 17 + [i32, i32, i32, vp]),
    "dinox_dino_ce": (i32, [vp, vp, vp, f32, f32, f32, vp, vp, vp, i32, i32, vp]),
    "dinox_dino_ce_multi": (i32, [vp, vp, vp, f32, f32, f32, vp, vp, vp, i32, i32, i32, i32, vp]),
    "dinox_colmean": (i32, [vp, vp, i32, i32, vp]),
    "dinox_center_ema": (i32, [vp, vp, f32, i32, vp]),
    "dinox_gram_normalize": (i32, [vp, vp, vp, vp, vp, vp, i32, i32, i32, i32, vp]),
    "dinox_sqsum": (i32, [vp, i64, f32, vp, vp, vp]),
    "dinox_gram_normalize_bwd": (i32, [vp, vp, vp, vp, vp, i32, i32, i32, i32, i32, vp]),
    "dinox_slice_views_lds_bytes": (i64, [i32, i32]),
    "dinox_slice_views": (i32, [vp, vp, vp, vp, i32, i32, i32, vp]),
    "dinox_slice_views_patches": (i32, [vp, vp, vp, vp, i32, i32, i32, i32, i32, i32, vp]),
    "dinox_encode_preprocess_lds_bytes": (i64, [i32, i32]),
    "dinox_encode_preprocess": (i32, [vp, i32, vp, i32, vp, i32, i32, i32, C.c_double, C.c_double, i32, vp]),
    "dinox_softmax_rows": (i32, [vp, vp, i64, i32, i32, i64, vp]),
    "dinox_softmax_bwd_rows": (i32, [vp, vp, vp, f32, i64, i32, i32, i64, vp]),
    "dinox_koleo_normalize": (i32, [vp, vp, vp, vp, i64, i32, f32, vp]),
    "dinox_koleo_nn": (i32, [vp, i64, vp, vp, i32, i32, i32, i32, vp, vp, vp]),
    "dinox_koleo_loss": (i32, [vp, i32, f32, vp, vp]),
    "dinox_koleo_bwd": (i32, [vp, vp, vp, vp, i32, i32, i32, i32, f32, f32, f32, vp, vp]),
    "dinox_ntxent_rows": (i32, [vp, i64, i32, f32, vp, vp, vp, vp]),
    "dinox_ntxent_coeff": (i32, [vp, i64, vp, i32, f32, f32, vp, i64, vp]),
    "dinox_normalize_bwd": (i32, [vp, vp, vp, vp, i64, i32, f32, vp]),
    "dinox_mae_mask_ids": (i32, [vp, vp, vp, i32, i32, i32, vp]),
    "dinox_mae_gather_unfold": (i32, [vp, vp, vp, i32, i32, i32, i32, i32, i32, i32, vp]),
    "dinox_mae_tokens_fwd": (i32, [vp, vp, vp, vp, vp, i32, i32, i32, i32, i32, vp]),
    "dinox_mae_tokens_bwd": (i32, [vp, vp, vp, vp, vp, i32, i32, i32, i32, i32, vp]),
    "dinox_mae_unshuffle_fwd": (i32, [vp, vp, vp, vp, vp, i32, i32, i32, i32, i32, vp]),
    "dinox_mae_unshuffle_bwd": (i32, [vp, vp, vp, vp, vp, vp, i32, i32, i32, i32, i32, vp]),
    "dinox_mae_loss_fwd": (i32, [vp, vp, vp, vp, vp, i32, i32, i32, i32, i32, i32, i32, vp]),
    "dinox_mae_loss_bwd": (i32, [vp, vp, vp, vp, f32, i32, i32, i32, i32, i32, i32, i32, i32, vp]),
    "dinox_attention_rows_ok": (i32, [i32, i32, i32, i32, i32]),
    "dinox_attention_rows": (i32, [vp, vp, vp, vp, i32, i32, i32, i32, i32, i32, vp]),
    "dinox_attention_rollout_step_ok": (i32, [i32, i32, i32, i32]),
    "dinox_attention_rollout_step": (i32, [vp, vp, vp, vp, i32, i32, i32, i32, f32, i32, vp]),
    "dinox_adamw_ema": (i32, [vp, vp, vp, vp, vp, i64, f32, f32, f32, f32, f32, i32, f32, f32, vp, vp, vp]),
    "dinox_adamw_ema_dev": (i32, [vp, vp, vp, vp, vp, i64, vp, f32, f32, f32, f32, f32, f32, vp, vp, vp]),
    "dinox_sumsq": (i32, [vp, i64, vp, vp, vp]),
    "dinox_cast_bf16": (i32, [vp, vp, i64, vp]),
    "dinox_cast_transpose_bf16": (i32, [vp, vp, i32, i32, vp]),
    "dinox_cast_transpose_bf16_multi": (i32, [vp, vp, vp, i32, i64, vp]),
    "dinox_take_rows": (i32, [vp, vp, i64, i64, i32, i64, i32, vp]),
    "dinox_put_rows": (i32, [vp, vp, i64, i64, i32, i64, i32, i32, vp]),
    "dinox_axpy": (i32, [vp, vp, f32, i64, vp]),
    "dinox_lincomb3": (i32, [vp, vp, vp, f32, f32, vp, vp]),
    "dinox_zero": (i32, [vp, i64, vp]),
    "dinox_gelu_fwd": (i32, [vp, vp, i64, vp]),
    "dinox_gelu_bwd": (i32, [vp, vp, vp, i64, vp]),
    "dinox_block_forward": (i32, [C.POINTER(BlockFwdArgs), vp]),
    "dinox_block_backward": (i32, [C.POINTER(BlockBwdArgs), vp]),
    "dinox_retrieval_ws_bytes": (i64, [i64, i64, i64]),
    "dinox_retrieval_rank": (i32, [vp, i64, vp, i64, vp, i64, i64, i64, vp, vp, vp, vp, vp, vp]),
    "dinox_retrieval_rank_windowed_ws_bytes": (i64, [i64, i64, i64]),
    "dinox_retrieval_rank_windowed": (i32, [vp, i64, vp, i64, vp, vp, vp, i64, i64, i64, vp, vp, vp, vp, vp, vp]),
    "dinox_row_dots": (i32, [vp, i64, vp, i64, i64, i64, vp, vp]),
    "dinox_knn_ws_bytes": (i64, [i64, i64, i64, i32]),
    "dinox_knn_topk": (i32, [vp, i64, vp, i64, vp, i64, i64, i64, i32, vp, vp, vp, vp]),
    "dinox_gram_ws_bytes": (i64, [i64, i64]),
    "dinox_gram_f32": (i32, [vp, i64, i64, i64, vp, vp, vp, vp, vp]),
    "dinox_softmax_probe_ws_bytes": (i64, [i64, i64, i32]),
    "dinox_softmax_probe": (i32, [vp, i64, vp, i64, i64, i32, vp, vp, vp, vp, vp, vp]),
    "dinox_gemm_timer_start": (i32, [i32]),
    "dinox_gemm_timer_stop": (i64, [C.c_char_p, i64]),
}


SIZE_T_SIGNATURES = {
    "dinox_attention_rollout_step_ws_bytes": (C.c_size_t, [i32, i32, i32]),
}

class DinoxLibraryError(ImportError):
    pass


def _load() -> C.CDLL:
    if not os.path.exists(LIB_PATH):
        raise DinoxLibraryError(
            f"{LIB_PATH} not found: the HIP kernel library is the only compute path of this package "
            "(no CPU/eager fallback). Build it with `python -c 'import __graft_entry__ as g; g.build()'` "
            "or `make -C dino-x_amd/csrc`.")
    try:
        lib = C.CDLL(LIB_PATH)
    except OSError as e:
        raise DinoxLibraryError(f"cannot load {LIB_PATH}: {e}") from e
    for name, (res, args) in {**SIGNATURES, **SIZE_T_SIGNATURES}.items():
        try:
            fn = getattr(lib, name)
        except AttributeError as e:
            raise DinoxLibraryError(f"{LIB_PATH} does not export {name}; rebuild it") from e
        fn.restype = res
        fn.argtypes = args
    return lib


lib = _load()


def last_error() -> str:
    return lib.dinox_last_error().decode("utf-8", "replace")


def check(rc: int, what: str) -> None:
    if rc != 0:
        raise RuntimeError(f"{what} failed (code {rc}): {last_error()}")
```

### dino-x_amd/dinox/ops.py

```python
from __future__ import annotations

import contextlib
import ctypes as C
import math
import operator
import os
import weakref
from typing import Optional

import torch

from . import _lib
from ._lib import BF16, EPI_ACCUM, EPI_AUXGRAD, EPI_BIAS, EPI_DGELU, EPI_GELU, EPI_RESIDUAL, F32, BlockBwdArgs, BlockFwdArgs, GemmArgs, check, lib

Tensor = torch.Tensor
_OVERRIDE: list = []


@contextlib.contextmanager
def compute_dtype(dtype: torch.dtype):
    if dtype not in (torch.float32, torch.bfloat16):
        raise ValueError("compute dtype must be torch.float32 or torch.bfloat16")
    _OVERRIDE.append(dtype)
    try:
        yield
    finally:
        _OVERRIDE.pop()


def current_dtype() -> torch.dtype:
    if _OVERRIDE:
        return _OVERRIDE[-1]
    if torch.is_autocast_enabled("cuda"):
        dt = torch.get_autocast_dtype("cuda")
        if dt != torch.bfloat16:
            raise RuntimeError(f"the HIP path supports bfloat16 autocast only (got {dt}); use --amp-dtype bfloat16")
        return torch.bfloat16
    return torch.float32


def _code(dtype: torch.dtype) -> int:
    if dtype == torch.float32:
        return F32
    if dtype == torch.bfloat16:
        return BF16
    raise TypeError(f"unsupported dtype {dtype}")


def _stream() -> int:
    return torch.cuda.current_stream().cuda_stream


def _p(t: Optional[Tensor]):
    return None if t is None else t.data_ptr()


def _need_cuda(*ts: Tensor) -> None:
    for t in ts:
        if t is not None and not t.is_cuda:
            raise RuntimeError(
                "dinox: tensors must be on a CUDA/HIP device -- the MI355X kernel library is the only compute "
                "path (no CPU fallback). Move the model and inputs to 'cuda'.")


def _c(t: Tensor) -> Tensor:
    return t if t.is_contiguous() else t.contiguous()


class GemmTimer:

    def __init__(self, every: int = 16) -> None:
        self.every = max(1, int(every))
        self.text = ""

    def start(self) -> None:
        check(lib.dinox_gemm_timer_start(self.every), "dinox_gemm_timer_start")

    def stop(self) -> None:
        buf = C.create_string_buffer(1 << 20)
        n = lib.dinox_gemm_timer_stop(buf, len(buf))
        if n < 0:
            raise RuntimeError("dinox_gemm_timer_stop: record buffer too small")
        self.text += buf.value.decode()

    def __enter__(self):
        self.start()
        return self

    def __exit__(self, *exc):
        self.stop()
        return False

    @staticmethod
    def algorithmic_bytes(M, N, K, batch, epilogue, in_dtype, out_dtype, has_aux, shared_b) -> float:
        isz = 2 if in_dtype == BF16 else 4
        osz = 2 if out_dtype == BF16 else 4
        mn = float(M) * N * batch
        b = float(M) * K * batch * isz + float(N) * K * isz * (1 if shared_b else batch) + mn * osz
        if epilogue & EPI_RESIDUAL:
            b += mn * 4
        if has_aux and (epilogue & (EPI_GELU | EPI_DGELU)):
            b += mn * osz
        if epilogue & EPI_ACCUM:
            b += mn * 4
        return b

    def summary(self) -> dict:
        out: dict = {}
        untimed = []
        for line in self.text.splitlines():
            f = line.split()
            if len(f) != 13:
                continue
            name = f[0]
            M, N, K, batch, epi, idt, odt, aux, shb, launches, timed = (int(v) for v in f[1:12])
            ms = float(f[12])
            fl = 2.0 * M * N * K * batch * launches
            by = self.algorithmic_bytes(M, N, K, batch, epi, idt, odt, aux, shb) * launches
            d = out.setdefault(name, {"launches": 0, "timed": 0, "flops": 0.0, "bytes": 0.0, "ms": 0.0, "_tb": 0.0, "_tms": 0.0})
            d["launches"] += launches
            d["flops"] += fl
            d["bytes"] += by
            if timed:
                d["timed"] += timed
                d["ms"] += ms / timed * launches
                d["_tb"] += by / launches * timed
                d["_tms"] += ms
            else:
                untimed.append((name, by))
        for name, by in untimed:
            d = out[name]
            if d["_tb"] > 0:
                d["ms"] += by * d["_tms"] / d["_tb"]
        for name in [k for k, d in out.items() if d["timed"] == 0]:
            del out[name]
        for d in out.values():
            del d["_tb"], d["_tms"]
        self.text = ""
        return out


TRACE_KERNELS: Optional[list] = None


def gemm(A: Tensor, B: Tensor, *, transA=False, transB=False, out: Optional[Tensor] = None,
         out_dtype: Optional[torch.dtype] = None, bias: Optional[Tensor] = None, gelu=False, aux: Optional[Tensor] = None,
         dgelu=False, residual: Optional[Tensor] = None, accumulate=False, alpha: float = 1.0,
         colsum_out: Optional[Tensor] = None, auxgrad=False) -> Tensor:
    _need_cuda(A, B)
    assert A.dtype == B.dtype, (A.dtype, B.dtype)
    A, B = _c(A), _c(B)
    batched = A.dim() == 3
    if batched:
        batch = A.shape[0]
        a2, b2 = A.shape[1:], (B.shape[1:] if B.dim() == 3 else B.shape)
    else:
        batch, a2, b2 = 1, A.shape, B.shape
    M, K = (a2[1], a2[0]) if transA else (a2[0], a2[1])
    N, Kb = (b2[1], b2[0]) if transB else (b2[0], b2[1])
    assert K == Kb, f"inner dims differ: {tuple(A.shape)} vs {tuple(B.shape)} (transA={transA}, transB={transB})"
    odt = out_dtype or (out.dtype if out is not None else A.dtype)
    if out is None:
        out = torch.empty((batch, M, N) if batched else (M, N), dtype=odt, device=A.device)
    else:
        assert out.is_contiguous() and out.dtype == odt and out.numel() == batch * M * N
    epi = 0
    if bias is not None:
        epi |= EPI_BIAS
        assert bias.dtype == torch.float32 and bias.numel() == N
    if gelu:
        epi |= EPI_GELU
    if dgelu:
        epi |= EPI_DGELU
        assert aux is not None
    if aux is not None:
        assert aux.dtype == odt and aux.is_contiguous() and aux.numel() == batch * M * N
    if residual is not None:
        epi |= EPI_RESIDUAL
        assert residual.dtype == torch.float32 and residual.is_contiguous() and residual.numel() == batch * M * N
    if accumulate:
        epi |= EPI_ACCUM
    if auxgrad:
        epi |= EPI_AUXGRAD
    if colsum_out is not None:
        assert transA and not batched and colsum_out.dtype == torch.float32 and colsum_out.numel() == M and colsum_out.is_contiguous()
    g = GemmArgs(
        A=_p(A), B=_p(B), C=_p(out), M=M, N=N, K=K, lda=a2[1], ldb=b2[1], ldc=N, batch=batch,
        strideA=a2[0] * a2[1] if batched else 0, strideB=(b2[0] * b2[1] if (batched and B.dim() == 3) else 0),
        strideC=M * N, transA=int(transA), transB=int(transB), in_dtype=_code(A.dtype), out_dtype=_code(odt),
        epilogue=epi, alpha=alpha, bias=_p(bias), residual=_p(residual), ldr=N, aux=_p(aux), ldaux=N, colsum=_p(colsum_out), ws=None)
    if (transA and transB and not batched and odt == torch.float32 and K >= 4096 and not (epi & ~EPI_ACCUM)
            and ((M + 127) // 128) * ((N + 127) // 128) < 256 and lib.dinox_gemm_kernel_name(C.byref(g)).decode().startswith("gemm_f32")):
        tiles = ((M + 127) // 128) * ((N + 127) // 128)
        splits = max(1, min(K // 1024, 1024 // tiles))
        while splits > 1 and K % splits:
            splits -= 1
        if splits > 1:
            kc = K // splits
            part = torch.empty((splits, M, N), dtype=torch.float32, device=A.device)
            g2 = GemmArgs(A=_p(A), B=_p(B), C=_p(part), M=M, N=N, K=kc, lda=a2[1], ldb=b2[1], ldc=N, batch=splits, strideA=kc * a2[1],
                          strideB=kc * b2[1], strideC=M * N, transA=1, transB=1, in_dtype=_code(A.dtype), out_dtype=F32, epilogue=0, alpha=alpha,
                          bias=None, residual=None, ldr=N, aux=None, ldaux=N, colsum=None, ws=None)
            if TRACE_KERNELS is not None:
                TRACE_KERNELS.append(lib.dinox_gemm_kernel_name(C.byref(g2)).decode())
            check(lib.dinox_gemm(C.byref(g2), _stream()), "dinox_gemm")
            colsum(part.view(splits, M * N), out=out.view(-1), accumulate=accumulate)
            if colsum_out is not None:
                check(lib.dinox_colsum(_p(A), _p(colsum_out), K, M, a2[1], _code(A.dtype), int(accumulate), _stream()), "dinox_colsum")
            return out
    if transA and transB and not batched and A.dtype == torch.bfloat16 and not _TN_ATOMICS:
        need = lib.dinox_gemm_ws_bytes(C.byref(g))
        if need:
            g.ws = _p(_tn_workspace(need, A.device))
    if TRACE_KERNELS is not None:
        TRACE_KERNELS.append(lib.dinox_gemm_kernel_name(C.byref(g)).decode())
    check(lib.dinox_gemm(C.byref(g), _stream()), "dinox_gemm")
    return out


_TN_ATOMICS = bool(os.environ.get("DINOX_TN_ATOMICS"))
_TN_WS: dict = {}


def _tn_workspace(nbytes: int, device) -> Tensor:
    key = (device, _stream())
    ws = _TN_WS.get(key)
    if ws is None or ws.numel() < nbytes:
        ws = _TN_WS[key] = torch.empty(max(nbytes, 40 << 20), dtype=torch.uint8, device=device)
    return ws


def gemm_nt_f32_splitk(A: Tensor, B: Tensor, splits: int = 0) -> Tensor:
    _need_cuda(A, B)
    assert A.dtype == torch.float32 and B.dtype == torch.float32 and A.is_contiguous() and B.is_contiguous() and A.dim() == 2 and B.dim() == 2
    M, K = A.shape
    N = B.shape[0]
    assert B.shape[1] == K
    if splits <= 0:
        tiles = ((M + 127) // 128) * ((N + 127) // 128)
        splits = max(1, min(K // 256, 256 // max(tiles, 1)))
    while splits > 1 and K % splits:
        splits -= 1
    if splits == 1:
        return gemm(A, B, out_dtype=torch.float32)
    kc = K // splits
    part = torch.empty((splits, M, N), dtype=torch.float32, device=A.device)
    g = GemmArgs(A=_p(A), B=_p(B), C=_p(part), M=M, N=N, K=kc, lda=K, ldb=K, ldc=N, batch=splits, strideA=kc, strideB=kc, strideC=M * N,
                 transA=0, transB=0, in_dtype=F32, out_dtype=F32, epilogue=0, alpha=1.0, bias=None, residual=None, ldr=N, aux=None, ldaux=N,
                 colsum=None, ws=None)
    if TRACE_KERNELS is not None:
        TRACE_KERNELS.append(lib.dinox_gemm_kernel_name(C.byref(g)).decode())
    check(lib.dinox_gemm(C.byref(g), _stream()), "dinox_gemm")
    return colsum(part.view(splits, M * N)).view(M, N)


def colsum(x: Tensor, out: Optional[Tensor] = None, accumulate=False) -> Tensor:
    x2 = _c(x).reshape(-1, x.shape[-1])
    if out is None:
        out = torch.empty(x2.shape[1], dtype=torch.float32, device=x.device)
    check(lib.dinox_colsum(_p(x2), _p(out), x2.shape[0], x2.shape[1], x2.shape[1], _code(x.dtype), int(accumulate), _stream()), "dinox_colsum")
    return out


def cast_bf16(x: Tensor, out: Optional[Tensor] = None) -> Tensor:
    x = _c(x)
    if out is None:
        out = torch.empty(x.shape, dtype=torch.bfloat16, device=x.device)
    else:
        assert out.dtype == torch.bfloat16 and out.is_contiguous() and out.numel() == x.numel()
    check(lib.dinox_cast_bf16(_p(x), _p(out), x.numel(), _stream()), "dinox_cast_bf16")
    return out


def cast_transpose_bf16(w: Tensor) -> Tensor:
    w = _c(w)
    R, Cc = w.shape
    out = torch.empty((Cc, R), dtype=torch.bfloat16, device=w.device)
    check(lib.dinox_cast_transpose_bf16(_p(w), _p(out), R, Cc, _stream()), "dinox_cast_transpose_bf16")
    return out


def to_mode(x: Tensor, dt: torch.dtype) -> Tensor:
    if x.dtype == dt:
        return _c(x)
    if dt == torch.bfloat16 and x.dtype == torch.float32:
        return cast_bf16(x)
    if dt == torch.float32 and x.dtype == torch.bfloat16:
        return x.float()
    raise TypeError(f"cannot bring {x.dtype} to {dt}")


class ArenaShadow:

    def __init__(self, flat: Tensor, params, offsets) -> None:
        self.flat, self.params, self.offsets = flat, list(params), list(offsets)
        self.index = {p.data_ptr(): i for i, p in enumerate(self.params) if p.numel()}
        self.plain: Optional[Tensor] = None
        self.trans: Optional[Tensor] = None
        self.versions: list = []
        self.wanted: dict = {}
        self.table: Optional[Tensor] = None
        self.table_for: tuple = ()
        self.tiles = 0
        self.served_t: set = set()

    def refresh(self) -> None:
        self.plain = cast_bf16(self.flat, out=self.plain)
        self.versions = [p._version for p in self.params]
        self.served_t = set()
        if self.wanted:
            key = tuple(sorted(self.wanted))
            if key != self.table_for:
                rows, tiles = [], 0
                for i in key:
                    R, Cc = self.wanted[i]
                    rows.append([self.offsets[i], R, Cc, tiles])
# ... 258 lines not shown
    if _bf16_attention_needs_products(qkv, N, d, fwd=True):
        q32 = qkv.float()
        o32 = torch.empty((B, N, Cc), dtype=torch.float32, device=qkv.device)
        _attention_fwd_f32_products(q32, heads, o32, lse)
        return o32.to(qkv.dtype), lse
    check(lib.dinox_attention_fwd(_p(qkv), _p(o), _p(lse), B, N, heads, d, _code(qkv.dtype), _stream()), "dinox_attention_fwd")
    return o, lse


_QKV_FUSED = {"1": True, "0": False}.get(os.environ.get("DINOX_QKV_FUSED", ""))


def _qkv_fused(D: int) -> bool:
    return _QKV_FUSED if _QKV_FUSED is not None else D <= 512


def qkv_attention_ok(B: int, N: int, heads: int, D: int, C: int) -> bool:
    return C % heads == 0 and bool(lib.dinox_qkv_attention_ok(B, N, heads, C // heads, D))


def qkv_attention(x: Tensor, w: Tensor, bias: Optional[Tensor], heads: int, want_qkv: bool = False, want_lse: bool = False):
    _need_cuda(x, w)
    x, w = _c(x), _c(w)
    B, N, D = x.shape
    C = w.shape[0] // 3
    assert x.dtype == torch.bfloat16 and w.dtype == torch.bfloat16 and w.shape == (3 * C, D) and C % heads == 0
    o = torch.empty((B, N, C), dtype=torch.bfloat16, device=x.device)
    qkv = torch.empty((B, N, 3 * C), dtype=torch.bfloat16, device=x.device) if want_qkv else None
    lse = torch.empty((B, heads, N), dtype=torch.float32, device=x.device) if want_lse else None
    if TRACE_KERNELS is not None:
        TRACE_KERNELS.append("attn_qkv_fused_fwd")
    check(lib.dinox_qkv_attention_fwd(_p(x), _p(w), _p(None if bias is None else _c(bias)), _p(o), _p(qkv), _p(lse), B, N, heads, C // heads, D,
                                      _stream()), "dinox_qkv_attention_fwd")
    return o, qkv, lse


def attention_bwd(do: Tensor, qkv: Tensor, o: Tensor, lse: Tensor, heads: int) -> Tensor:
    do = to_mode(do, qkv.dtype)
    B, N, C3 = qkv.shape
    d = C3 // 3 // heads
    dqkv = torch.empty_like(qkv)
    if _use_f32_products(qkv, N, d):
        _attention_bwd_f32_products(_c(do), _c(qkv), o, lse, heads, dqkv)
        return dqkv
    if _bf16_attention_needs_products(qkv, N, d, fwd=False):
        d32 = torch.empty(qkv.shape, dtype=torch.float32, device=qkv.device)
        _attention_bwd_f32_products(_c(do).float(), _c(qkv).float(), o, lse, heads, d32)
        return d32.to(qkv.dtype)
    ws = torch.empty(lib.dinox_attention_bwd_ws_bytes(B, N, heads), dtype=torch.uint8, device=qkv.device)
    check(lib.dinox_attention_bwd(_p(do), _p(qkv), _p(o), _p(lse), _p(dqkv), _p(ws), B, N, heads, d, _code(qkv.dtype), _stream()),
          "dinox_attention_bwd")
    return dqkv


class LayerNormFn(torch.autograd.Function):

    @staticmethod
    def forward(ctx, x, w, b, out_dtype, eps):
        y, mean, rstd = layernorm_fwd(x, w, b, out_dtype, eps)
        ctx.save_for_backward(x, w, mean, rstd, b)
        ctx.mode_bf16 = current_dtype() == torch.bfloat16
        if ctx.needs_input_grad[1]:
            grad_sink.use(w, b)
        return y

    @staticmethod
    def backward(ctx, dy):
        x, w, mean, rstd, b = ctx.saved_tensors
        dx, dw, db, lowp = layernorm_bwd(dy, x, w, mean, rstd, want_lowp=ctx.mode_bf16, b=b if ctx.needs_input_grad[1] else None)
        if lowp is not None:
            lowp_cache.put(dx, lowp)
        return dx, dw, db, None, None


class LayerNormPrecomputedFn(torch.autograd.Function):

    @staticmethod
    def forward(ctx, x, w, b, y, mean, rstd):
        ctx.save_for_backward(x, w, mean, rstd, b)
        ctx.mode_bf16 = current_dtype() == torch.bfloat16
        if ctx.needs_input_grad[1]:
            grad_sink.use(w, b)
        return y.view_as(y)

    @staticmethod
    def backward(ctx, dy):
        x, w, mean, rstd, b = ctx.saved_tensors
        dx, dw, db, lowp = layernorm_bwd(dy, x.reshape(-1, x.shape[-1]), w, mean, rstd, want_lowp=ctx.mode_bf16,
                                         b=b if ctx.needs_input_grad[1] else None)
        dx = dx.view(x.shape)
        if lowp is not None:
            lowp_cache.put(dx, lowp.view(x.shape))
        return dx, dw, db, None, None, None


class _LowpCache:

    def __init__(self) -> None:
        self.key = None
        self.val = None

    def put(self, t: Tensor, lowp: Tensor) -> None:
        self.key, self.val = (t.data_ptr(), t._version, tuple(t.shape)), lowp

    def take(self, t: Tensor) -> Optional[Tensor]:
        if self.key == (t.data_ptr(), t._version, tuple(t.shape)):
            v, self.key, self.val = self.val, None, None
            return v
        return None


lowp_cache = _LowpCache()


def grad_operand(g: Tensor, dt: torch.dtype) -> Tensor:
    if dt == torch.float32:
        return _c(g) if g.dtype == torch.float32 else g.float()
    if g.dtype == torch.bfloat16:
        return _c(g)
    hit = lowp_cache.take(g)
    return hit if hit is not None else cast_bf16(g)


class _GradSink:

    def __init__(self) -> None:
        self.slots: dict = {}
        self.uses: dict = {}
        self.on_ready = None
        self.owner = None
        self.recomputing = 0

    def register(self, owner, params, on_ready=None) -> None:
        self.slots = {p.data_ptr(): (i, p) for i, p in enumerate(params) if p.requires_grad and p.numel()}
        self.uses, self.on_ready, self.owner = {}, on_ready, owner

    def clear(self) -> None:
        self.slots, self.uses, self.on_ready, self.owner = {}, {}, None, None

    def lookup(self, w: Optional[Tensor]):
        if w is None or not self.slots:
            return None
        slot = self.slots.get(w.data_ptr())
        if slot is None:
            return None
        g = slot[1].grad
        if g is None or g.dtype != torch.float32 or not g.is_contiguous() or g.shape != w.shape:
            return None
        return slot

    def use(self, *ws) -> None:
        if self.on_ready is None or self.recomputing:
            return
        for w in ws:
            slot = self.lookup(w)
            if slot is not None:
                self.uses[slot[0]] = self.uses.get(slot[0], 0) + 1

    def ready(self, slot) -> None:
        if self.on_ready is None:
            return
        left = self.uses.get(slot[0], 1) - 1
        self.uses[slot[0]] = max(left, 0)
        if left <= 0:
            self.on_ready(slot[0])


grad_sink = _GradSink()


@contextlib.contextmanager
def _recompute_scope():
    grad_sink.recomputing += 1
    try:
        yield
    finally:
        grad_sink.recomputing -= 1


def checkpoint_contexts():
    return contextlib.nullcontext(), _recompute_scope()


def small_grad(param: Optional[Tensor], g: Optional[Tensor]) -> Optional[Tensor]:
    if g is None or param is None:
        return g
    slot = grad_sink.lookup(param)
    if slot is None or g.dtype != torch.float32 or not g.is_contiguous():
        return g
    axpy_(slot[1].grad.view(-1), g.view(-1), 1.0)
    grad_sink.ready(slot)
    return None


class _DwStream:

    def __init__(self) -> None:
        self.enabled = bool(os.environ.get("DINOX_DW_STREAM"))
        self.streams: dict = {}
        self.dirty = False

    def side(self, device):
        st = self.streams.get(device)
        if st is None:
            st = self.streams[device] = torch.cuda.Stream(device=device)
        return st

    def run(self, fn, *tensors) -> None:
        main = torch.cuda.current_stream()
        side = self.side(tensors[0].device)
        side.wait_stream(main)
        with torch.cuda.stream(side):
            fn()
        for t in tensors:
            t.record_stream(side)
        self.dirty = True

    def join(self) -> None:
        if self.dirty:
            main = torch.cuda.current_stream()
            for st in self.streams.values():
                main.wait_stream(st)
            self.dirty = False


dw_stream = _DwStream()


def weight_grad(dy: Tensor, x: Tensor, w: Tensor, bias: Optional[Tensor], want_db: bool):
    sw = grad_sink.lookup(w)
    sb = grad_sink.lookup(bias) if want_db else None
    if sw is not None and (not want_db or sb is not None):
        def product():
            gemm(dy, x, transA=True, transB=True, out=sw[1].grad.view(w.shape[0], -1), accumulate=True,
                 colsum_out=sb[1].grad if want_db else None)
        if dw_stream.enabled and dy.is_cuda:
            dw_stream.run(product, dy, x)
        else:
            product()
        grad_sink.ready(sw)
        if want_db:
            grad_sink.ready(sb)
        return None, None
    db = torch.empty(w.shape[0], dtype=torch.float32, device=dy.device) if want_db else None
    dw = gemm(dy, x, transA=True, transB=True, out_dtype=torch.float32, colsum_out=db)
    return dw.reshape(w.shape), db


_BLOCK_NATIVE = os.environ.get("DINOX_BLOCK_NATIVE", "1") != "0"


def _block_native_ok(dt: torch.dtype, x0: Tensor, wqkv: Tensor) -> bool:
    return _BLOCK_NATIVE and dt == torch.bfloat16 and x0.is_cuda and TRACE_KERNELS is None and not dw_stream.enabled


def _block_forward_native(ctx, x0, n1w, n1b, wqkv, bqkv, wproj, bproj, n2w, n2b, w1, b1, w2, b2, heads, eps, pre_ln, next_ln, train):
    dt = torch.bfloat16
    V, N, D = x0.shape
    M, H = V * N, w1.shape[0]
    dev = x0.device
    bf = lambda *shape: torch.empty(shape, dtype=torch.bfloat16, device=dev)
    f32 = lambda *shape: torch.empty(shape, dtype=torch.float32, device=dev)
    if pre_ln is None:
        xn1, mean1, rstd1 = bf(V, N, D), f32(M), f32(M)
    else:
        xn1, mean1, rstd1 = pre_ln
    if not train and _qkv_fused(D) and qkv_attention_ok(V, N, heads, D, D):
        qkv, o, lse = None, bf(V, N, D), None
    else:
        qkv, o, lse = bf(M, 3 * D), bf(V, N, D), f32(V, heads, N)
    x1, xn2, mean2, rstd2 = f32(M, D), bf(M, D), f32(M), f32(M)
    act = bf(M, H)
    pre = bf(M, H) if train else None
    x2 = f32(V, N, D)
    nxt = None
    wops = [weight_operand(w_, dt) for w_ in (wqkv, wproj, w1, w2)]
    a = BlockFwdArgs(V=V, N=N, D=D, H=H, heads=heads, train=int(train), fuse_proj_ln=int(rowln_ok(M, D, D, dt)), fuse_fc2_ln=0, eps=eps,
                     x0=_p(x0), qkv=_p(qkv), o=_p(o), lse=_p(lse), x1=_p(x1), xn2=_p(xn2), mean2=_p(mean2), rstd2=_p(rstd2), act=_p(act), pre=_p(pre),
                     x2=_p(x2), n1w=_p(n1w), n1b=_p(n1b), n2w=_p(n2w), n2b=_p(n2b), wqkv=_p(wops[0]), wproj=_p(wops[1]), w1=_p(wops[2]), w2=_p(wops[3]),
                     bqkv=_p(bqkv), bproj=_p(bproj), b1=_p(b1), b2=_p(b2))
    if pre_ln is None:
        a.xn1, a.mean1, a.rstd1 = _p(xn1), _p(mean1), _p(rstd1)
    else:
        a.xn1_in, a.mean1_in, a.rstd1_in = _p(xn1), _p(mean1), _p(rstd1)
    if next_ln is not None:
        ydt = next_ln[3] or dt
        yn, mn, rn = torch.empty((V, N, D), dtype=ydt, device=dev), f32(M), f32(M)
        a.next_g, a.next_b, a.next_eps, a.next_dtype = _p(next_ln[0]), _p(next_ln[1]), next_ln[2], _code(ydt)
        a.yn, a.meann, a.rstdn = _p(yn), _p(mn), _p(rn)
        a.fuse_fc2_ln = int(rowln_ok(M, D, H, dt, ydt))
        nxt = (yn, mn, rn)
    check(lib.dinox_block_forward(C.byref(a), _stream()), "dinox_block_forward")
    if train:
        ctx.save_for_backward(x0, x1, xn1, xn2, qkv, o, lse, pre, act, mean1, rstd1, mean2, rstd2, n1w, n2w, wqkv, wproj, w1, w2,
                              bqkv, bproj, b1, b2, n1b, n2b)
        ctx.dt, ctx.heads, ctx.shape, ctx.native = dt, heads, (V, N, D), True
        grad_sink.use(wqkv, bqkv, wproj, bproj, w1, b1, w2, b2, n1w, n1b, n2w, n2b)
    if next_ln is None:
        return x2
    ctx.mark_non_differentiable(*nxt)
    return (x2,) + nxt


_BLOCK_TN_WS: dict = {}


def _block_tn_ws_bytes(M: int, D: int, H: int) -> int:
    key = (M, D, H)
    hit = _BLOCK_TN_WS.get(key)
    if hit is None:
        hit = 0
        for n_out, n_in in ((D, H), (H, D), (D, D), (3 * D, D)):
            g = GemmArgs(A=0x1000, B=0x1000, C=0x1000, M=n_out, N=n_in, K=M, lda=n_out, ldb=n_in, ldc=n_in, batch=1, strideA=0, strideB=0, strideC=n_out * n_in,
                         transA=1, transB=1, in_dtype=BF16, out_dtype=F32, epilogue=EPI_ACCUM, alpha=1.0, bias=None, residual=None, ldr=n_in, aux=None,
                         ldaux=n_in, colsum=0x1000, ws=0x1000)
            hit = max(hit, int(lib.dinox_gemm_ws_bytes(C.byref(g))))
        _BLOCK_TN_WS[key] = hit
    return hit


def _block_backward_native(ctx, g: Tensor, saved):
    (x0, x1, xn1, xn2, qkv, o, lse, pre, act, mean1, rstd1, mean2, rstd2, n1w, n2w, wqkv, wproj, w1, w2, bqkv, bproj, b1, b2,
     n1b, n2b) = saved
    slots = [grad_sink.lookup(t) for t in (wqkv, bqkv, wproj, bproj, w1, b1, w2, b2, n1w, n1b, n2w, n2b)]
    have = [t is not None for t in (wqkv, bqkv, wproj, bproj, w1, b1, w2, b2, n1w, n1b, n2w, n2b)]
    if any(h and s is None for h, s in zip(have, slots)) or not all(have[i] for i in (0, 2, 4, 6, 8, 9, 10, 11)):
        return None
    dt, heads = torch.bfloat16, ctx.heads
    V, N, D = ctx.shape
    M, H = V * N, w1.shape[0]
    dev = g.device
    bf = lambda *shape: torch.empty(shape, dtype=torch.bfloat16, device=dev)
    g_lp = lowp_cache.take(g)
    g1 = torch.empty((V, N, D), dtype=torch.float32, device=dev)
    g0_lp = bf(V, N, D)
    gp = lambda sl: None if sl is None else sl[1].grad.data_ptr()
    tn_ws = _tn_workspace(max(_block_tn_ws_bytes(M, D, H), 1), dev)
    scratch = dict(dpre=bf(M, H), dxn2=bf(M, D), d_o=bf(M, D), dqkv=bf(M, 3 * D), dxn1=bf(M, D), g1_lowp=bf(M, D),
                   g_lowp_buf=None if g_lp is not None else bf(M, D),
                   attn_ws=torch.empty(lib.dinox_attention_bwd_ws_bytes(V, N, heads), dtype=torch.uint8, device=dev),
                   ln_ws=torch.empty(lib.dinox_layernorm_bwd_ws_bytes(M, D), dtype=torch.uint8, device=dev))
    wts = [weight_operand(w_, dt, transposed=True) for w_ in (wqkv, wproj, w1, w2)]
    fuse_ln = linear_ln_bwd_ok(M, D, H, dt) and linear_ln_bwd_ok(M, D, 3 * D, dt)
    a = BlockBwdArgs(V=V, N=N, D=D, H=H, heads=heads, reserved=int(fuse_ln), g=_p(g), g_lowp=_p(g_lp), g_lowp_buf=_p(scratch["g_lowp_buf"]),
                     x0=_p(x0), x1=_p(x1), xn1=_p(xn1), xn2=_p(xn2), qkv=_p(qkv), o=_p(o), lse=_p(lse), pre=_p(pre), act=_p(act), mean1=_p(mean1),
                     rstd1=_p(rstd1), mean2=_p(mean2), rstd2=_p(rstd2), n1w=_p(n1w), n2w=_p(n2w),
                     wqkv_t=_p(wts[0]), wproj_t=_p(wts[1]), w1_t=_p(wts[2]), w2_t=_p(wts[3]),
                     dwqkv=gp(slots[0]), dbqkv=gp(slots[1]), dwproj=gp(slots[2]), dbproj=gp(slots[3]), dw1=gp(slots[4]), db1=gp(slots[5]),
                     dw2=gp(slots[6]), db2=gp(slots[7]), dn1w=gp(slots[8]), dn1b=gp(slots[9]), dn2w=gp(slots[10]), dn2b=gp(slots[11]),
                     dpre=_p(scratch["dpre"]), dxn2=_p(scratch["dxn2"]), d_o=_p(scratch["d_o"]), dqkv=_p(scratch["dqkv"]), dxn1=_p(scratch["dxn1"]),
                     g1=_p(g1), g1_lowp=_p(scratch["g1_lowp"]), g0_lowp=_p(g0_lp), attn_ws=_p(scratch["attn_ws"]), ln_ws=_p(scratch["ln_ws"]),
                     tn_ws=_p(tn_ws), tn_ws_bytes=tn_ws.numel())
    check(lib.dinox_block_backward(C.byref(a), _stream()), "dinox_block_backward")
    for sl in slots:
        if sl is not None:
            grad_sink.ready(sl)
    lowp_cache.put(g1, g0_lp)
    return (g1,) + (None,) * 16


_outer_grad_mode = [True]


def block_fn(*args):
    prev = _outer_grad_mode[0]
    _outer_grad_mode[0] = torch.is_grad_enabled()
    try:
        return BlockFn.apply(*args)
    finally:
        _outer_grad_mode[0] = prev


class BlockFn(torch.autograd.Function):

    @staticmethod
    def forward(ctx, x0, n1w, n1b, wqkv, bqkv, wproj, bproj, n2w, n2b, w1, b1, w2, b2, heads, eps, pre_ln=None, next_ln=None):
        _need_cuda(x0, wqkv)
        ctx.set_materialize_grads(False)
        dt = current_dtype()
        x0 = _c(x0 if x0.dtype == torch.float32 else x0.float())
        V, N, D = x0.shape
        M = V * N
        train = any(ctx.needs_input_grad) and _outer_grad_mode[0]
        if _block_native_ok(dt, x0, wqkv):
            return _block_forward_native(ctx, x0, n1w, n1b, wqkv, bqkv, wproj, bproj, n2w, n2b, w1, b1, w2, b2, heads, eps, pre_ln, next_ln, train)
        ctx.native = False
        if pre_ln is None:
            xn1, mean1, rstd1 = layernorm_fwd(x0, n1w, n1b, dt, eps)
        else:
            xn1, mean1, rstd1 = pre_ln
        if not train and dt == torch.bfloat16 and _qkv_fused(D) and qkv_attention_ok(V, N, heads, D, D):
            o, qkv, lse = qkv_attention(xn1.view(V, N, D), weight_operand(wqkv, dt), bqkv, heads)
        else:
            qkv = gemm(xn1.view(M, D), weight_operand(wqkv, dt), bias=bqkv, out_dtype=dt)
            o, lse = attention_fwd(qkv.view(V, N, 3 * D), heads)
        if rowln_ok(M, D, D, dt):
            x1, xn2, mean2, rstd2 = linear_residual_ln(o.view(M, D), weight_operand(wproj, dt), bproj, x0.view(M, D), n2w, n2b, eps, dt)
        else:
            x1 = gemm(o.view(M, D), weight_operand(wproj, dt), bias=bproj, residual=x0.view(M, D), out_dtype=torch.float32)
            xn2, mean2, rstd2 = layernorm_fwd(x1, n2w, n2b, dt, eps)
        nxt = None
        if True:
            H = w1.shape[0]
            pre = torch.empty((M, H), dtype=dt, device=x0.device) if train else None
            act = gemm(xn2, weight_operand(w1, dt), bias=b1, gelu=True, aux=pre, auxgrad=True, out_dtype=dt)
            if next_ln is not None and rowln_ok(M, D, H, dt, next_ln[3] or dt):
                x2, yn, mn, rn = linear_residual_ln(act, weight_operand(w2, dt), b2, x1, next_ln[0], next_ln[1], next_ln[2], next_ln[3] or dt)
                nxt = (yn.view(V, N, D), mn, rn)
            else:
                x2 = gemm(act, weight_operand(w2, dt), bias=b2, residual=x1, out_dtype=torch.float32)
            if train:
                ctx.save_for_backward(x0, x1, xn1, xn2, qkv, o, lse, pre, act, mean1, rstd1, mean2, rstd2, n1w, n2w, wqkv, wproj, w1, w2,
                                      bqkv, bproj, b1, b2, n1b, n2b)
                ctx.dt, ctx.heads, ctx.shape = dt, heads, (V, N, D)
                grad_sink.use(wqkv, bqkv, wproj, bproj, w1, b1, w2, b2, n1w, n1b, n2w, n2b)
        x2 = x2.view(V, N, D)
        if next_ln is None:
            return x2
        if nxt is None:
            yn, mn, rn = layernorm_fwd(x2, next_ln[0], next_ln[1], next_ln[3] or dt, next_ln[2])
            nxt = (yn, mn, rn)
        ctx.mark_non_differentiable(*nxt)
        return (x2,) + nxt

    @staticmethod
    def backward(ctx, g, *_unused):
        (x0, x1, xn1, xn2, qkv, o, lse, pre, act, mean1, rstd1, mean2, rstd2, n1w, n2w, wqkv, wproj, w1, w2, bqkv, bproj, b1, b2,
         n1b, n2b) = ctx.saved_tensors
        dt, heads = ctx.dt, ctx.heads
        V, N, D = ctx.shape
        M = V * N
        dev = g.device
        g = _c(g if g.dtype == torch.float32 else g.float())
        bf = dt == torch.bfloat16
        if ctx.native:
            native = _block_backward_native(ctx, g, (x0, x1, xn1, xn2, qkv, o, lse, pre, act, mean1, rstd1, mean2, rstd2, n1w, n2w, wqkv, wproj, w1, w2,
                                                     bqkv, bproj, b1, b2, n1b, n2b))
            if native is not None:
                return native

        def wt(w):
            return (w.detach(), dict(transB=True)) if not bf else (weight_operand(w, dt, transposed=True), {})

        g_op = grad_operand(g, dt).view(M, D)
        b, kw = wt(w2)
        dpre = gemm(g_op, b, dgelu=True, aux=pre, auxgrad=True, out_dtype=dt, **kw)
        dw2, db2 = weight_grad(g_op, act, w2, b2, b2 is not None)
        b, kw = wt(w1)
        fuse_ln = bf and linear_ln_bwd_ok(M, D, dpre.shape[1], dt) and linear_ln_bwd_ok(M, D, 3 * D, dt)
        if not fuse_ln:
            dxn2 = gemm(dpre, b, out_dtype=dt, **kw)
        dw1, db1 = weight_grad(dpre, xn2.view(M, D), w1, b1, b1 is not None)
        if fuse_ln:
            g1, dn2w, dn2b, g1_lp = linear_ln_bwd(dpre, b, x1, n2w, mean2, rstd2, dx_add=g.view(M, D), want_lowp=True, b=n2b)
        else:
            g1, dn2w, dn2b, g1_lp = layernorm_bwd(dxn2, x1, n2w, mean2, rstd2, dx_add=g.view(M, D), want_lowp=bf, b=n2b)
        del dpre
        g1_op = g1_lp if bf else g1
        b, kw = wt(wproj)
        do = gemm(g1_op, b, out_dtype=dt, **kw)
        dwp, dbp = weight_grad(g1_op, o.view(M, D), wproj, bproj, bproj is not None)
        dqkv = attention_bwd(do.view(V, N, D), qkv.view(V, N, 3 * D), o, lse, heads).view(M, 3 * D)
        b, kw = wt(wqkv)
        if not fuse_ln:
            dxn1 = gemm(dqkv, b, out_dtype=dt, **kw)
        dwq, dbq = weight_grad(dqkv, xn1.view(M, D), wqkv, bqkv, bqkv is not None)
        if not bf:
            dw_stream.join()
        if fuse_ln:
            g0, dn1w, dn1b, g0_lp = linear_ln_bwd(dqkv, b, x0, n1w, mean1, rstd1, dx=g1, dx_add=g1, want_lowp=True, b=n1b)
        else:
            g0, dn1w, dn1b, g0_lp = layernorm_bwd(dxn1, x0, n1w, mean1, rstd1, dx=g1, dx_add=g1, want_lowp=bf, b=n1b)
        g0 = g0.view(V, N, D)
        if g0_lp is not None:
            lowp_cache.put(g0, g0_lp.view(V, N, D))
        return g0, dn1w, dn1b, dwq, dbq, dwp, dbp, dn2w, dn2b, dw1, db1, dw2, db2, None, None, None, None


class LinearFn(torch.autograd.Function):

    @staticmethod
    def forward(ctx, x, w, b, residual, out_dtype):
        _need_cuda(x, w)
        dt = current_dtype()
        xm = to_mode(x, dt)
        K = xm.shape[-1]
        x2 = xm.reshape(-1, K)
        odt = torch.float32 if residual is not None else (out_dtype or dt)
        y = gemm(x2, weight_operand(w, dt), bias=b, residual=None if residual is None else _c(residual).reshape(-1, w.shape[0]),
                 out_dtype=odt)
        ctx.save_for_backward(x2, w, b)
        if ctx.needs_input_grad[1]:
            grad_sink.use(w, b if ctx.needs_input_grad[2] else None)
        ctx.dt, ctx.has_bias, ctx.has_res, ctx.xshape, ctx.xdtype = dt, b is not None, residual is not None, x.shape, x.dtype
        return y.reshape(*x.shape[:-1], w.shape[0])

    @staticmethod
    def backward(ctx, dy):
        x2, w, b = ctx.saved_tensors
        dt = ctx.dt
        dy2 = to_mode(dy.reshape(-1, w.shape[0]), dt)
        dx = dw = db = None
        if ctx.needs_input_grad[0]:
            if dt == torch.float32:
                dx = gemm(dy2, w.detach(), transB=True, out_dtype=ctx.xdtype)
            else:
                dx = gemm(dy2, weight_operand(w, dt, transposed=True), out_dtype=ctx.xdtype if ctx.xdtype == dt else dt)
                if dx.dtype != ctx.xdtype:
                    dx = dx.to(ctx.xdtype)
            dx = dx.reshape(ctx.xshape)
        want_db = ctx.has_bias and ctx.needs_input_grad[2]
        if ctx.needs_input_grad[1]:
            dw, db = weight_grad(dy2, x2, w, b, want_db)
        elif want_db:
            db = colsum(dy2)
        dres = dy if ctx.has_res else None
        return dx, dw, db, dres, None


class MlpFn(torch.autograd.Function):

    @staticmethod
    def forward(ctx, x, w1, b1, w2, b2, residual, out_dtype):
        _need_cuda(x, w1, w2)
        dt = current_dtype()
        xm = to_mode(x, dt)
        x2 = xm.reshape(-1, xm.shape[-1])
        M, H = x2.shape[0], w1.shape[0]
        pre = torch.empty((M, H), dtype=dt, device=x.device) if any(ctx.needs_input_grad[:5]) else None
        act = gemm(x2, weight_operand(w1, dt), bias=b1, gelu=True, aux=pre, auxgrad=True, out_dtype=dt)
        odt = torch.float32 if residual is not None else (out_dtype or dt)
        y = gemm(act, weight_operand(w2, dt), bias=b2, residual=None if residual is None else _c(residual).reshape(M, w2.shape[0]),
                 out_dtype=odt)
        ctx.save_for_backward(x2, w1, w2, pre, act, b1, b2)
        if pre is not None:
            grad_sink.use(w1, b1, w2, b2)
        ctx.dt, ctx.has_res, ctx.xshape, ctx.xdtype = dt, residual is not None, x.shape, x.dtype
        return y.reshape(*x.shape[:-1], w2.shape[0])

    @staticmethod
    def backward(ctx, dy):
        x2, w1, w2, pre, act, b1, b2 = ctx.saved_tensors
        dt = ctx.dt
        dy2 = to_mode(dy.reshape(-1, w2.shape[0]), dt)
        if dt == torch.float32:
            dpre = gemm(dy2, w2.detach(), transB=True, dgelu=True, aux=pre, auxgrad=True, out_dtype=dt)
        else:
            dpre = gemm(dy2, weight_operand(w2, dt, transposed=True), dgelu=True, aux=pre, auxgrad=True, out_dtype=dt)
        dw2, db2 = weight_grad(dy2, act, w2, b2, b2 is not None)
        dx = None
        if ctx.needs_input_grad[0]:
            if dt == torch.float32:
                dx = gemm(dpre, w1.detach(), transB=True, out_dtype=dt)
            else:
                dx = gemm(dpre, weight_operand(w1, dt, transposed=True), out_dtype=dt)
            if dx.dtype != ctx.xdtype:
                dx = dx.to(ctx.xdtype)
            dx = dx.reshape(ctx.xshape)
        dw1, db1 = weight_grad(dpre, x2, w1, b1, b1 is not None)
        return dx, dw1, db1, dw2, db2, (dy if ctx.has_res else None), None


class AttentionCoreFn(torch.autograd.Function):

    @staticmethod
    def forward(ctx, qkv, heads):
        o, lse = attention_fwd(qkv, heads)
        ctx.save_for_backward(qkv, o, lse)
        ctx.heads = heads
        return o

    @staticmethod
    def backward(ctx, do):
        qkv, o, lse = ctx.saved_tensors
        return attention_bwd(do, qkv, o, lse, ctx.heads), None


ATTENTION_ROWS_MAX_Q = 8
ATTENTION_ROWS_MAX_D = 256


def attention_rows(qkv: Tensor, heads: int, query_idx, want_lse: bool = False):
    if not isinstance(qkv, Tensor) or not qkv.is_cuda:
        raise ValueError("attention_rows: qkv must be a tensor on a CUDA/HIP device (the MI355X kernel library is the only compute path)")
    if qkv.dtype not in (torch.float32, torch.bfloat16):
        raise ValueError(f"attention_rows: qkv must be float32 or bfloat16, got {qkv.dtype}")
    if qkv.dim() == 5:
        if qkv.shape[2] != 3 or qkv.shape[3] != heads:
            raise ValueError(f"attention_rows: a 5-D qkv must be [B, N, 3, heads={heads}, d], got {tuple(qkv.shape)}")
        qkv = qkv.reshape(qkv.shape[0], qkv.shape[1], -1)
    if qkv.dim() != 3:
        raise ValueError(f"attention_rows: qkv must be [B, N, 3 heads d], got {tuple(qkv.shape)}")
    B, N, C3 = qkv.shape
    if not isinstance(heads, int) or heads < 1 or C3 % (3 * heads) or B < 1 or N < 1 or C3 < 1:
        raise ValueError(f"attention_rows: qkv {tuple(qkv.shape)} is not [B >= 1, N >= 1, 3 x heads={heads} x d]")
    d = C3 // (3 * heads)
    if d > ATTENTION_ROWS_MAX_D:
        raise ValueError(f"attention_rows: head size {d} above {ATTENTION_ROWS_MAX_D}")
    if isinstance(query_idx, Tensor):
        if query_idx.dim() != 1 or query_idx.dtype not in (torch.int32, torch.int64):
            raise ValueError(f"attention_rows: query_idx must be a 1-D int32 / int64 tensor, got {query_idx.dtype} {tuple(query_idx.shape)}")
        idx = query_idx.tolist()
    else:
        idx = list(query_idx)
        if not all(isinstance(i, int) and not isinstance(i, bool) for i in idx):
            raise ValueError(f"attention_rows: query_idx must hold integers, got {idx}")
    Q = len(idx)
    if not 1 <= Q <= ATTENTION_ROWS_MAX_Q:
        raise ValueError(f"attention_rows: 1 to {ATTENTION_ROWS_MAX_Q} query rows, got {Q}")
    if any(i < 0 or i >= N for i in idx):
        raise ValueError(f"attention_rows: query_idx {idx} outside [0, {N})")
    if not lib.dinox_attention_rows_ok(B, N, heads, d, Q):
        raise ValueError(f"attention_rows: B={B} N={N} heads={heads} d={d} Q={Q} outside the kernel")
    qkv = _c(qkv.detach())
    qi = torch.tensor(idx, dtype=torch.int32, device=qkv.device)
    probs = torch.empty((B, heads, Q, N), dtype=torch.float32, device=qkv.device)
    lse = torch.empty((B, heads, Q), dtype=torch.float32, device=qkv.device) if want_lse else None
    if TRACE_KERNELS is not None:
        TRACE_KERNELS.append("attention_rows")
    check(lib.dinox_attention_rows(_p(qkv), _p(qi), _p(probs), _p(lse), B, N, heads, d, Q, _code(qkv.dtype), _stream()), "dinox_attention_rows")
    return (probs, lse) if want_lse else probs


ATTENTION_ROLLOUT_MAX_N = 4096


def attention_rollout_step(qkv: Tensor, heads: int, w: Tensor, residual: float = 0.5) -> Tensor:
    if not isinstance(qkv, Tensor) or not qkv.is_cuda:
        raise ValueError("attention_rollout_step: qkv must be a tensor on a CUDA/HIP device (the MI355X kernel library is the only compute path)")
    if qkv.dtype not in (torch.float32, torch.bfloat16):
        raise ValueError(f"attention_rollout_step: qkv must be float32 or bfloat16, got {qkv.dtype}")
    if qkv.dim() == 5:
        if qkv.shape[2] != 3 or qkv.shape[3] != heads:
            raise ValueError(f"attention_rollout_step: a 5-D qkv must be [B, N, 3, heads={heads}, d], got {tuple(qkv.shape)}")
        qkv = qkv.reshape(qkv.shape[0], qkv.shape[1], -1)
    if qkv.dim() != 3:
        raise ValueError(f"attention_rollout_step: qkv must be [B, N, 3 heads d], got {tuple(qkv.shape)}")
    B, N, C3 = qkv.shape
    if not isinstance(heads, int) or isinstance(heads, bool) or heads < 1 or C3 % (3 * heads) or B < 1 or N < 1 or C3 < 1:
        raise ValueError(f"attention_rollout_step: qkv {tuple(qkv.shape)} is not [B >= 1, N >= 1, 3 x heads={heads} x d]")
    d = C3 // (3 * heads)
    if d > ATTENTION_ROWS_MAX_D or N > ATTENTION_ROLLOUT_MAX_N:
        raise ValueError(f"attention_rollout_step: head size {d} above {ATTENTION_ROWS_MAX_D} or {N} tokens above {ATTENTION_ROLLOUT_MAX_N}")
    if not isinstance(w, Tensor) or w.device != qkv.device:
        raise ValueError("attention_rollout_step: w must be a tensor on the device of qkv")
    if w.dim() != 2 or tuple(w.shape) != (B, N) or not w.dtype.is_floating_point:
        raise ValueError(f"attention_rollout_step: w must be a float tensor [B={B}, N={N}], got {w.dtype} {tuple(w.shape)}")
# ... 999 lines not shown
```

### include/dinox.h

```cpp
#ifndef DINOX_H
#define DINOX_H

#include <stddef.h>
#include <stdint.h>

#ifdef __cplusplus
extern "C" {
#endif

#define DINOX_ABI_VERSION 3

#define DINOX_F32 0
#define DINOX_BF16 1
#define DINOX_U16 2
#define DINOX_I16 3

#define DINOX_OK 0
#define DINOX_EINVAL (-1)
#define DINOX_EUNSUPPORTED (-2)
#define DINOX_EALIGN (-3)

int dinox_version(void);
const char* dinox_last_error(void);
int dinox_device_ok(void);

#define DINOX_EPI_BIAS 1
#define DINOX_EPI_GELU 2
#define DINOX_EPI_DGELU 4
#define DINOX_EPI_RESIDUAL 8
#define DINOX_EPI_ACCUM 16
#define DINOX_EPI_AUXGRAD 32

typedef struct dinox_gemm_args {
  const void* A;
  const void* B;
  void* C;
  int64_t M, N, K;
  int64_t lda, ldb, ldc;
  int64_t batch;
  int64_t strideA, strideB, strideC;
  int32_t transA, transB;
  int32_t in_dtype, out_dtype;
  int32_t epilogue;
  float alpha;
  const float* bias;
  const float* residual;
  int64_t ldr;
  void* aux;
  int64_t ldaux;
  float* colsum;
  void* ws;
} dinox_gemm_args;

int dinox_gemm(const dinox_gemm_args* args, void* stream);
int64_t dinox_gemm_ws_bytes(const dinox_gemm_args* args);
const char* dinox_gemm_kernel_name(const dinox_gemm_args* args);

int dinox_colsum(const void* x, float* out, int64_t M, int64_t N, int64_t ldx, int dtype, int accumulate,
                 void* stream);

int dinox_linear_residual_ln_ok(int64_t M, int N, int K);
int dinox_linear_residual_ln(const void* a, const void* w, const float* bias, const float* residual, float* x_out,
                             const float* gamma, const float* beta, float eps, void* y, int y_dtype, float* mean,
                             float* rstd, int64_t M, int N, int K, void* stream);

int dinox_layernorm_fwd(const float* x, const float* w, const float* b, void* y, float* mean, float* rstd,
                        int64_t rows, int dim, float eps, int out_dtype, void* stream);
int64_t dinox_layernorm_bwd_ws_bytes(int64_t rows, int dim);
int dinox_layernorm_bwd(const void* dy, const float* x, const float* w, const float* mean, const float* rstd,
                        float* dx, const float* dx_add, void* dx_lowp, float* dw, float* db, void* ws,
                        int64_t rows, int dim, int dy_dtype, int accumulate, void* stream);
int dinox_linear_ln_bwd_ok(int64_t M, int N, int K);
int dinox_linear_ln_bwd(const void* a, const void* w, const float* x, const float* gamma, const float* mean, const float* rstd,
                        float* dx, const float* dx_add, void* dx_lowp, float* dgamma, float* dbeta, void* ws, int64_t M, int N,
                        int K, int accumulate, void* stream);

int dinox_attention_fwd(const void* qkv, void* o, float* lse, int B, int N, int heads, int d, int dtype,
                        void* stream);
int dinox_softmax_rows(float* s, float* lse, int64_t rows, int n, int rows_per_image, int64_t lse_image_stride, void* stream);
int dinox_softmax_bwd_rows(float* s, float* dp, const float* lse, float scale, int64_t rows, int n, int rows_per_image,
                           int64_t lse_image_stride, void* stream);
int64_t dinox_attention_bwd_ws_bytes(int B, int N, int heads);
int dinox_attention_bwd(const void* d_o, const void* qkv, const void* o, const float* lse, void* dqkv, void* ws,
                        int B, int N, int heads, int d, int dtype, void* stream);
int dinox_qkv_attention_ok(int B, int N, int heads, int d, int D);
int dinox_qkv_attention_fwd(const void* x, const void* wqkv, const float* bias, void* o, void* qkv_out, float* lse, int B, int N,
                            int heads, int d, int D, void* stream);

int dinox_patch_unfold(const float* x, void* u, int V, int H, int W, int patch, int out_dtype, void* stream);
int dinox_patch_unfold_ld(const float* x, void* u, int V, int H, int W, int patch, int ld, int out_dtype, void* stream);
int dinox_tokens_fwd(const void* patches, const float* cls, const float* pos, const float* registers,
                     const float* scale, float* tokens, int V, int P, int R, int D, int patches_dtype,
                     void* stream);
int dinox_tokens_bwd(const float* dtokens, void* dpatches, float* dcls, float* dpos, float* dregs,
                     float* dscale, int V, int P, int R, int D, int patches_dtype, void* stream);

int dinox_scale_embed_fwd(const float* spacing, const float* w0, const float* b0, const float* w2,
                          const float* b2, const float* lnw, const float* lnb, float* out, float* hpre,
                          float* e, float* mean, float* rstd, int V, int h, int D, float eps, void* stream);
int64_t dinox_scale_embed_bwd_ws_bytes(int V, int h, int D);
int dinox_scale_embed_bwd(const float* dout, const float* spacing, const float* w0, const float* w2,
                          const float* lnw, const float* hpre, const float* e, const float* mean,
                          const float* rstd, float* dw0, float* db0, float* dw2, float* db2, float* dlnw,
                          float* dlnb, float* dspacing, void* ws, int V, int h, int D, void* stream);

int dinox_dino_ce(const float* s, const float* t, const float* center, float student_temp, float teacher_temp,
                  float grad_scale, float* loss, float* ds, float* row_loss, int rows2B, int K, void* stream);
int dinox_dino_ce_multi(const float* s, const float* t, const float* center, float student_temp, float teacher_temp,
                        float grad_scale, float* loss, float* ds, float* ws, int B, int n_global, int n_views, int K,
                        void* stream);
int dinox_colmean(const float* t, float* out, int rows, int K, void* stream);
int dinox_center_ema(float* center, const float* batch_mean, float momentum, int K, void* stream);

int dinox_gram_normalize(const float* sfeats, const float* tfeats, void* cat, void* catneg, void* shat,
                         float* snorm, int V, int N, int D, int out_dtype, void* stream);
int dinox_sqsum(const float* x, int64_t n, float scale, float* loss, float* ws, void* stream);
int dinox_gram_normalize_bwd(const float* dxh, const void* shat, const float* snorm, const float* sfeats,
                             float* dfeats, int V, int N, int D, int shat_dtype, int accumulate, void* stream);

int64_t dinox_slice_views_lds_bytes(int S, int max_crop);
int dinox_slice_views(const void* raw_u16, const int64_t* view_i, const float* view_f, float* out, int V, int S, int max_crop,
                      void* stream);
int dinox_slice_views_patches(const void* raw_u16, const int64_t* view_i, const float* view_f, void* u, int V, int S, int max_crop,
                              int patch, int ld, int out_dtype, void* stream);

#define DINOX_FMT_HU_FLOAT 0
#define DINOX_FMT_HU16_PNG 1
#define DINOX_FMT_WINDOWED_FLOAT 2
int64_t dinox_encode_preprocess_lds_bytes(int S, int max_side);
int dinox_encode_preprocess(const void* src, int src_dtype, const int64_t* jobs, int n_jobs, float* out, int n_images, int S,
                            int max_side, double lo, double hi, int format, void* stream);

int dinox_koleo_normalize(const float* x, float* xh, float* norm, float* sq, int64_t V, int D, float eps, void* stream);
int dinox_koleo_nn(const float* G, int64_t ldg, const float* sq_all, const float* xh_all, int row0, int V_l, int V_g, int D,
                   int* idx, float* dist, void* stream);
int dinox_koleo_loss(const float* dist, int V, float eps, float* loss, void* stream);
int dinox_koleo_bwd(const float* xh_all, const int* idx_all, const float* dist_all, const float* norm_loc, int row0, int V_l,
                    int V_g, int D, float gscale, float eps, float norm_eps, float* dx, void* stream);

int dinox_ntxent_rows(const float* S, int64_t lds, int M, float inv_tau, float* lse, float* row_loss, float* loss, void* stream);
int dinox_ntxent_coeff(const float* S, int64_t lds, const float* lse, int M, float inv_tau, float gscale, float* W, int64_t ldw,
                       void* stream);
int dinox_normalize_bwd(const float* dxh, const float* xh, const float* norm, float* dx, int64_t V, int D, float eps, void* stream);

int dinox_mae_mask_ids(const float* noise, int* ids_restore, int* ids_keep, int V, int L, int Lk, void* stream);
int dinox_mae_gather_unfold(const float* x, const int* ids_keep, void* u, int V, int H, int W, int patch, int Lk, int ld, int out_dtype,
                            void* stream);
int dinox_mae_tokens_fwd(const void* patches, const float* cls, const float* pos, const int* ids_keep, float* tokens, int V, int L, int Lk,
                         int D, int patches_dtype, void* stream);
int dinox_mae_tokens_bwd(const float* dtokens, const int* ids_restore, void* dpatches, float* dcls, float* dpos, int V, int L, int Lk, int D,
                         int patches_dtype, void* stream);
int dinox_mae_unshuffle_fwd(const void* e, const float* mask_token, const float* dec_pos, const int* ids_restore, float* xd, int V, int L,
                            int Lk, int D, int e_dtype, void* stream);
int dinox_mae_unshuffle_bwd(const float* g, const int* ids_keep, const int* ids_restore, void* de, float* dmask_token, float* ws, int V,
                            int L, int Lk, int D, int de_dtype, void* stream);
int dinox_mae_loss_fwd(const void* pred, const float* x, const int* ids_restore, float* loss, float* ws, int V, int H, int W, int patch,
                       int Lk, int lead, int pred_dtype, void* stream);
int dinox_mae_loss_bwd(const void* pred, const float* x, const int* ids_restore, void* dpred, float gscale, int V, int H, int W, int patch,
                       int Lk, int lead, int pred_dtype, int dpred_dtype, void* stream);

int dinox_attention_rows_ok(int B, int N, int heads, int d, int Q);
int dinox_attention_rows(const void* qkv, const int* query_idx, float* probs, float* lse, int B, int N, int heads, int d, int Q, int dtype,
                         void* stream);

int dinox_attention_rollout_step_ok(int B, int N, int heads, int d);
size_t dinox_attention_rollout_step_ws_bytes(int B, int N, int heads);
int dinox_attention_rollout_step(const void* qkv, const float* w_in, float* w_out, void* ws, int B, int N, int heads, int d, float residual,
                                 int dtype, void* stream);

int dinox_adamw_ema(float* p, const float* g, float* m, float* v, float* teacher, int64_t n, float lr,
                    float weight_decay, float beta1, float beta2, float eps, int step_t, float ema,
                    float grad_scale, float* gnorm_sq, float* ws, void* stream);
int dinox_adamw_ema_dev(float* p, const float* g, float* m, float* v, float* teacher, int64_t n, const float* hyper,
                        float weight_decay, float beta1, float beta2, float eps, float ema, float grad_scale,
                        float* gnorm_sq, float* ws, void* stream);
int dinox_sumsq(const float* x, int64_t n, float* out, float* ws, void* stream);
int dinox_cast_bf16(const float* src, void* dst, int64_t n, void* stream);
int dinox_cast_transpose_bf16(const float* src, void* dst, int R, int C, void* stream);
int dinox_cast_transpose_bf16_multi(const float* src_base, void* dst_base, const int64_t* table, int n_mats,
                                    int64_t total_tiles, void* stream);
int dinox_take_rows(const float* src, void* dst, int64_t V, int64_t src_stride, int D, int64_t dst_row0, int dst_dtype,
                    void* stream);
int dinox_put_rows(const void* src, float* dst, int64_t V, int64_t dst_stride, int D, int64_t src_row0, int src_dtype,
                   int accumulate, void* stream);
int dinox_axpy(float* y, const float* x, float alpha, int64_t n, void* stream);
int dinox_lincomb3(const float* a, const float* b, const float* c, float wb, float wc, float* out, void* stream);
int dinox_zero(void* p, int64_t bytes, void* stream);
int dinox_gelu_fwd(const float* x, float* y, int64_t n, void* stream);
int dinox_gelu_bwd(const float* dy, const float* x, float* dx, int64_t n, void* stream);

typedef struct dinox_block_fwd_args {
  int64_t V, N;
  int32_t D, H, heads;
  int32_t train;
  int32_t fuse_proj_ln, fuse_fc2_ln;
  float eps;
  const float* x0;
  const void* xn1_in; const float* mean1_in; const float* rstd1_in;
  void* xn1; float* mean1; float* rstd1;
  void* qkv; void* o; float* lse;
  float* x1; void* xn2; float* mean2; float* rstd2;
  void* act; void* pre;
  float* x2;
  const float* next_g; const float* next_b; float next_eps; int32_t next_dtype;
  void* yn; float* meann; float* rstdn;
  const float *n1w, *n1b, *n2w, *n2b;
  const void *wqkv, *wproj, *w1, *w2;
  const float *bqkv, *bproj, *b1, *b2;
} dinox_block_fwd_args;

typedef struct dinox_block_bwd_args {
  int64_t V, N;
  int32_t D, H, heads;
  int32_t reserved;
  const float* g; const void* g_lowp; void* g_lowp_buf;
  const float* x0; const float* x1; const void* xn1; const void* xn2; const void* qkv; const void* o; const float* lse;
  const void* pre; const void* act; const float *mean1, *rstd1, *mean2, *rstd2;
  const float *n1w, *n2w;
  const void *wqkv_t, *wproj_t, *w1_t, *w2_t;
  float *dwqkv, *dbqkv, *dwproj, *dbproj, *dw1, *db1, *dw2, *db2, *dn1w, *dn1b, *dn2w, *dn2b;
  void* dpre; void* dxn2; void* d_o; void* dqkv; void* dxn1;
  float* g1; void* g1_lowp; void* g0_lowp;
  void* attn_ws; void* ln_ws; void* tn_ws; int64_t tn_ws_bytes;
} dinox_block_bwd_args;

int dinox_block_forward(const dinox_block_fwd_args* args, void* stream);
int dinox_block_backward(const dinox_block_bwd_args* args, void* stream);

int64_t dinox_retrieval_ws_bytes(int64_t Nq, int64_t Nk, int64_t D);
int dinox_retrieval_rank(const float* q, int64_t ldq, const float* k, int64_t ldk, const int32_t* target, int64_t Nq, int64_t Nk, int64_t D,
                         int32_t* rank, int32_t* best_idx, float* best_val, float* pos_val, void* ws, void* stream);

int64_t dinox_retrieval_rank_windowed_ws_bytes(int64_t Nq, int64_t Nk, int64_t D);
int dinox_retrieval_rank_windowed(const float* q, int64_t ldq, const float* k, int64_t ldk, const int32_t* target, const int32_t* key_lo,
                                  const int32_t* key_hi, int64_t Nq, int64_t Nk, int64_t D, int32_t* rank, int32_t* best_idx, float* best_val,
                                  float* pos_val, void* ws, void* stream);

int dinox_row_dots(const float* a, int64_t lda, const float* b, int64_t ldb, int64_t N, int64_t D, float* out, void* stream);

int64_t dinox_knn_ws_bytes(int64_t Nq, int64_t Nk, int64_t D, int K);
int dinox_knn_topk(const float* q, int64_t ldq, const float* k, int64_t ldk, const int32_t* exclude, int64_t Nq, int64_t Nk, int64_t D, int K,
                   int32_t* out_idx, float* out_val, void* ws, void* stream);

int64_t dinox_gram_ws_bytes(int64_t N, int64_t D);
int dinox_gram_f32(const float* x, int64_t ldx, int64_t N, int64_t D, const float* shift, double* gram, double* colsum, void* ws, void* stream);

int64_t dinox_softmax_probe_ws_bytes(int64_t N, int64_t D, int C);
int dinox_softmax_probe(const float* x, int64_t ldx, const int32_t* label, int64_t N, int64_t D, int C, const float* theta, double* loss,
                        double* grad, float* prob, void* ws, void* stream);

int dinox_gemm_timer_start(int every);
int64_t dinox_gemm_timer_stop(char* buf, int64_t buflen);

#ifdef __cplusplus
}
#endif
#endif
```

Before: 7291 samples/s.

## Batch deferred split-K and LayerNorm gradient reductions into one launch per block backward

Block backward no longer launches a separate reduction kernel after each of the four weight-gradient split-K GEMMs and the two LayerNorm backward passes. Each call records its reduction as a segment, and one multi-segment reduce kernel runs at the end of the block. This cuts kernel launches and small, poorly occupied reduction kernels per block. In exchange each dW product and LN pass needs its own workspace region, so tn_ws and ln_ws grow, and the partial sums stay in memory longer.

```diff
diff --git a/dino-x_amd/csrc/block.hip b/dino-x_amd/csrc/block.hip
--- a/dino-x_amd/csrc/block.hip
+++ b/dino-x_amd/csrc/block.hip
@@ -1,6 +1,7 @@
 #include <cstring>
 
 #include "common.h"
+#include "knobs.h"
 
 using namespace dinox;
 
@@ -22,7 +23,7 @@
   return g;
 }
 
-int weight_grad(const void* dy, const void* x, float* dw, float* db, int64_t M, int64_t n_out, int64_t n_in, void* ws, int64_t ws_bytes, void* stream) {
+dinox_gemm_args weight_grad_args(const void* dy, const void* x, float* dw, float* db, int64_t M, int64_t n_out, int64_t n_in) {
   dinox_gemm_args g;
   memset(&g, 0, sizeof g);
   g.A = dy; g.B = x; g.C = dw;
@@ -38,13 +39,49 @@
   g.ldr = n_in;
   g.ldaux = n_in;
   g.colsum = db;
+  return g;
+}
+
+struct Deferred {
+  dinox_reduce_seg seg[DINOX_REDUCE_MAX_SEGS];
+  int n = 0;
+};
+
+int weight_grad(const void* dy, const void* x, float* dw, float* db, int64_t M, int64_t n_out, int64_t n_in, void* ws, int64_t ws_bytes, Deferred* later,
+                void* stream) {
+  dinox_gemm_args g = weight_grad_args(dy, x, dw, db, M, n_out, n_in);
   const int64_t need = dinox_gemm_ws_bytes(&g);
   if (need > 0) {
     DX_REQUIRE(ws && need <= ws_bytes, DINOX_EINVAL, "block_backward: tn_ws of %lld bytes, the dW product [%lld x %lld] over %lld rows needs %lld",
                (long long)ws_bytes, (long long)n_out, (long long)n_in, (long long)M, (long long)need);
     g.ws = ws;
   }
-  return dinox_gemm(&g, stream);
+  if (!later) return dinox_gemm(&g, stream);
+  int n = 0;
+  const int rc = dinox_gemm_deferred(&g, later->seg + later->n, &n, stream);
+  later->n += n;
+  return rc;
+}
+
+int layernorm_bwd(const void* dy, const float* x, const float* w, const float* mean, const float* rstd, float* dx, const float* dx_add, void* dx_lowp,
+                  float* dw, float* db, void* ws, int64_t M, int D, dinox_reduce_seg* segs, void* stream) {
+  if (segs) return dinox_layernorm_bwd_deferred(dy, x, w, mean, rstd, dx, dx_add, dx_lowp, dw, db, ws, M, D, DINOX_BF16, 1, segs, stream);
+  return dinox_layernorm_bwd(dy, x, w, mean, rstd, dx, dx_add, dx_lowp, dw, db, ws, M, D, DINOX_BF16, 1, stream);
+}
+
+int linear_ln_bwd(const void* a, const void* w, const float* x, const float* gamma, const float* mean, const float* rstd, float* dx, const float* dx_add,
+                  void* dx_lowp, float* dgamma, float* dbeta, void* ws, int64_t M, int N, int K, dinox_reduce_seg* segs, void* stream) {
+  if (segs) return dinox_linear_ln_bwd_deferred(a, w, x, gamma, mean, rstd, dx, dx_add, dx_lowp, dgamma, dbeta, ws, M, N, K, 1, segs, stream);
+  return dinox_linear_ln_bwd(a, w, x, gamma, mean, rstd, dx, dx_add, dx_lowp, dgamma, dbeta, ws, M, N, K, 1, stream);
+}
+
+int64_t region(int64_t bytes) { return (bytes + 255) & ~(int64_t)255; }
+
+bool batched_mode(int flags) { return (flags & DINOX_BLOCK_BWD_BATCHED) != 0 && knob_int("DINOX_BLOCK_REDUCE", 1) != 0; }
+
+void dw_shapes(int D, int H, int64_t (&sh)[4][2]) {
+  const int64_t v[4][2] = {{D, H}, {H, D}, {D, D}, {3 * (int64_t)D, D}};
+  memcpy(sh, v, sizeof v);
 }
 
 }
@@ -110,6 +147,25 @@
   return 0;
 }
 
+extern "C" int64_t dinox_block_backward_tn_ws_bytes(int64_t M, int D, int H, int flags) {
+  if (M <= 0 || D <= 0 || H <= 0) return 0;
+  int64_t sh[4][2];
+  dw_shapes(D, H, sh);
+  const bool batched = batched_mode(flags);
+  const void* al = reinterpret_cast<const void*>((uintptr_t)0x1000);
+  int64_t total = 0;
+  for (int i = 0; i < 4; ++i) {
+    dinox_gemm_args g = weight_grad_args(al, al, (float*)al, (float*)al, M, sh[i][0], sh[i][1]);
+    const int64_t need = dinox_gemm_ws_bytes(&g);
+    total = batched ? total + region(need) : (need > total ? need : total);
+  }
+  return total;
+}
+
+extern "C" int64_t dinox_block_backward_ln_ws_bytes(int64_t M, int D, int flags) {
+  return (batched_mode(flags) ? 2 : 1) * region(dinox_layernorm_bwd_ws_bytes(M, D));
+}
+
 extern "C" int dinox_block_backward(const dinox_block_bwd_args* a, void* stream) {
   DX_REQUIRE(a, DINOX_EINVAL, "block_backward: null args");
   DX_REQUIRE(a->V > 0 && a->N > 0 && a->D > 0 && a->H > 0 && a->heads > 0 && a->D % a->heads == 0, DINOX_EINVAL,
@@ -123,6 +179,30 @@
              "block_backward: null scratch");
   const int64_t M = a->V * a->N;
   const int D = a->D, H = a->H;
+  const bool batched = batched_mode(a->reserved);
+  Deferred deferred;
+  Deferred* const later = batched ? &deferred : nullptr;
+  char* tn_at[4] = {(char*)a->tn_ws, (char*)a->tn_ws, (char*)a->tn_ws, (char*)a->tn_ws};
+  int64_t tn_room[4] = {a->tn_ws_bytes, a->tn_ws_bytes, a->tn_ws_bytes, a->tn_ws_bytes};
+  float* ln_at[2] = {(float*)a->ln_ws, (float*)a->ln_ws};
+  if (batched) {
+    int64_t sh[4][2], off = 0;
+    dw_shapes(D, H, sh);
+    const void* dys[4] = {a->g_lowp ? a->g_lowp : a->g_lowp_buf, a->dpre, a->g1_lowp, a->dqkv};
+    const void* xs[4] = {a->act, a->xn2, a->o, a->xn1};
+    float* dbs[4] = {a->db2, a->db1, a->dbproj, a->dbqkv};
+    for (int i = 0; i < 4; ++i) {
+      dinox_gemm_args g = weight_grad_args(dys[i], xs[i], a->dw2, dbs[i], M, sh[i][0], sh[i][1]);
+      const int64_t need = region(dinox_gemm_ws_bytes(&g));
+      tn_at[i] = (char*)a->tn_ws + off;
+      tn_room[i] = need;
+      off += need;
+    }
+    DX_REQUIRE(off == 0 || (a->tn_ws && off <= a->tn_ws_bytes), DINOX_EINVAL,
+               "block_backward: tn_ws of %lld bytes, the batched reduction of the four dW products (D=%d H=%d over %lld rows) needs %lld (one region each)",
+               (long long)a->tn_ws_bytes, D, H, (long long)M, (long long)off);
+    ln_at[1] = (float*)((char*)a->ln_ws + region(dinox_layernorm_bwd_ws_bytes(M, D)));
+  }
   const void* g_op = a->g_lowp;
   if (!g_op) {
     BLK_TRY(dinox_cast_bf16(a->g, a->g_lowp_buf, M * D, stream));
@@ -134,33 +214,38 @@
     g.aux = const_cast<void*>(a->pre);
     BLK_TRY(dinox_gemm(&g, stream));
   }
-  BLK_TRY(weight_grad(g_op, a->act, a->dw2, a->db2, M, D, H, a->tn_ws, a->tn_ws_bytes, stream));
+  BLK_TRY(weight_grad(g_op, a->act, a->dw2, a->db2, M, D, H, tn_at[0], tn_room[0], later, stream));
   const bool fuse_ln = (a->reserved & 1) != 0;
   if (!fuse_ln) {
     dinox_gemm_args g = gemm_args(a->dpre, a->w1_t, a->dxn2, M, D, H, DINOX_BF16);
     BLK_TRY(dinox_gemm(&g, stream));
   }
-  BLK_TRY(weight_grad(a->dpre, a->xn2, a->dw1, a->db1, M, H, D, a->tn_ws, a->tn_ws_bytes, stream));
+  BLK_TRY(weight_grad(a->dpre, a->xn2, a->dw1, a->db1, M, H, D, tn_at[1], tn_room[1], later, stream));
+  dinox_reduce_seg* const ln2_segs = later ? later->seg + later->n : nullptr;
+  if (later) later->n += 2;
   if (fuse_ln)
-    BLK_TRY(dinox_linear_ln_bwd(a->dpre, a->w1_t, a->x1, a->n2w, a->mean2, a->rstd2, a->g1, a->g, a->g1_lowp, a->dn2w, a->dn2b, a->ln_ws, M, (int)D,
-                                (int)H, 1, stream));
+    BLK_TRY(linear_ln_bwd(a->dpre, a->w1_t, a->x1, a->n2w, a->mean2, a->rstd2, a->g1, a->g, a->g1_lowp, a->dn2w, a->dn2b, ln_at[0], M, (int)D, (int)H,
+                          ln2_segs, stream));
   else
-    BLK_TRY(dinox_layernorm_bwd(a->dxn2, a->x1, a->n2w, a->mean2, a->rstd2, a->g1, a->g, a->g1_lowp, a->dn2w, a->dn2b, a->ln_ws, M, D, DINOX_BF16, 1, stream));
+    BLK_TRY(layernorm_bwd(a->dxn2, a->x1, a->n2w, a->mean2, a->rstd2, a->g1, a->g, a->g1_lowp, a->dn2w, a->dn2b, ln_at[0], M, D, ln2_segs, stream));
   {
     dinox_gemm_args g = gemm_args(a->g1_lowp, a->wproj_t, a->d_o, M, D, D, DINOX_BF16);
     BLK_TRY(dinox_gemm(&g, stream));
   }
-  BLK_TRY(weight_grad(a->g1_lowp, a->o, a->dwproj, a->dbproj, M, D, D, a->tn_ws, a->tn_ws_bytes, stream));
+  BLK_TRY(weight_grad(a->g1_lowp, a->o, a->dwproj, a->dbproj, M, D, D, tn_at[2], tn_room[2], later, stream));
   BLK_TRY(dinox_attention_bwd(a->d_o, a->qkv, a->o, a->lse, a->dqkv, a->attn_ws, (int)a->V, (int)a->N, a->heads, D / a->heads, DINOX_BF16, stream));
   if (!fuse_ln) {
     dinox_gemm_args g = gemm_args(a->dqkv, a->wqkv_t, a->dxn1, M, D, 3 * (int64_t)D, DINOX_BF16);
     BLK_TRY(dinox_gemm(&g, stream));
   }
-  BLK_TRY(weight_grad(a->dqkv, a->xn1, a->dwqkv, a->dbqkv, M, 3 * (int64_t)D, D, a->tn_ws, a->tn_ws_bytes, stream));
+  BLK_TRY(weight_grad(a->dqkv, a->xn1, a->dwqkv, a->dbqkv, M, 3 * (int64_t)D, D, tn_at[3], tn_room[3], later, stream));
+  dinox_reduce_seg* const ln1_segs = later ? later->seg + later->n : nullptr;
+  if (later) later->n += 2;
   if (fuse_ln)
-    BLK_TRY(dinox_linear_ln_bwd(a->dqkv, a->wqkv_t, a->x0, a->n1w, a->mean1, a->rstd1, a->g1, a->g1, a->g0_lowp, a->dn1w, a->dn1b, a->ln_ws, M, (int)D,
-                                3 * (int)D, 1, stream));
+    BLK_TRY(linear_ln_bwd(a->dqkv, a->wqkv_t, a->x0, a->n1w, a->mean1, a->rstd1, a->g1, a->g1, a->g0_lowp, a->dn1w, a->dn1b, ln_at[1], M, (int)D,
+                          3 * (int)D, ln1_segs, stream));
   else
-    BLK_TRY(dinox_layernorm_bwd(a->dxn1, a->x0, a->n1w, a->mean1, a->rstd1, a->g1, a->g1, a->g0_lowp, a->dn1w, a->dn1b, a->ln_ws, M, D, DINOX_BF16, 1, stream));
+    BLK_TRY(layernorm_bwd(a->dxn1, a->x0, a->n1w, a->mean1, a->rstd1, a->g1, a->g1, a->g0_lowp, a->dn1w, a->dn1b, ln_at[1], M, D, ln1_segs, stream));
+  if (later && later->n > 0) BLK_TRY(dinox_reduce_segments(later->seg, later->n, stream));
   return 0;
 }
diff --git a/dino-x_amd/csrc/gemm.hip b/dino-x_amd/csrc/gemm.hip
--- a/dino-x_amd/csrc/gemm.hip
+++ b/dino-x_amd/csrc/gemm.hip
@@ -96,7 +96,7 @@
   return v ? v : "gemm_f32";
 }
 
-extern "C" int dinox_gemm(const dinox_gemm_args* a, void* stream) {
+static int gemm_call(const dinox_gemm_args* a, void* stream, dinox_reduce_seg* segs, int* n_segs) {
   DX_REQUIRE(a, DINOX_EINVAL, "gemm: null args");
   DX_REQUIRE(a->A && a->B && a->C, DINOX_EINVAL, "gemm: null operand");
   DX_REQUIRE(a->M > 0 && a->N > 0 && a->K > 0 && a->batch >= 1, DINOX_EINVAL, "gemm: M=%lld N=%lld K=%lld batch=%lld",
@@ -138,7 +138,7 @@
     }
   }
   int rc = DINOX_EUNSUPPORTED;
-  if (p.in_dtype == DINOX_BF16) rc = launch_gemm_bf16(p, st);
+  if (p.in_dtype == DINOX_BF16) rc = launch_gemm_bf16(p, st, segs, n_segs);
   if (rc == DINOX_EUNSUPPORTED) {
     rc = 0;
     if (p.colsum)
@@ -147,6 +147,23 @@
   }
   if (e1) (void)hipEventRecord(e1, st);
   return rc;
+}
+
+extern "C" int dinox_gemm(const dinox_gemm_args* a, void* stream) { return gemm_call(a, stream, nullptr, nullptr); }
+
+extern "C" int dinox_gemm_deferred(const dinox_gemm_args* a, dinox_reduce_seg* segs, int* n_segs, void* stream) {
+  DX_REQUIRE(segs && n_segs, DINOX_EINVAL, "gemm_deferred: null segment output");
+  *n_segs = 0;
+  return gemm_call(a, stream, segs, n_segs);
+}
+
+extern "C" int dinox_split_reduce(const float* part, int splits, int64_t MN, float alpha, float* C, int accumulate, const float* cs_part,
+                                  int cs_terms, int64_t M, float* colsum, void* stream) {
+  DX_REQUIRE(part && C && splits >= 1 && MN >= 4 && MN <= (int64_t)0x7fffffff * 64, DINOX_EINVAL, "split_reduce: part=%p C=%p splits=%d MN=%lld",
+             (const void*)part, (void*)C, splits, (long long)MN);
+  DX_REQUIRE(((((uintptr_t)part) | ((uintptr_t)C)) & 15) == 0, DINOX_EALIGN, "split_reduce: part and C must be 16-byte aligned");
+  DX_REQUIRE(!colsum || (cs_part && cs_terms >= 1 && M > 0), DINOX_EINVAL, "split_reduce: colsum without cs_part / cs_terms / M");
+  return launch_tn_reduce_raw(part, splits, MN, alpha, C, accumulate ? 1 : 0, cs_part, cs_terms, M, colsum, as_stream(stream));
 }
 
 extern "C" int dinox_gemm_timer_start(int every) {
diff --git a/dino-x_amd/csrc/gemm_bf16.hip b/dino-x_amd/csrc/gemm_bf16.hip
--- a/dino-x_amd/csrc/gemm_bf16.hip
+++ b/dino-x_amd/csrc/gemm_bf16.hip
@@ -456,14 +456,29 @@
   }
 }
 
-static int launch_tn_reduce(const GemmParams& p, int splits, int tiles_n, hipStream_t st) {
+int launch_tn_reduce_raw(const float* part, int splits, int64_t MN, float alpha, float* C, int accumulate, const float* cs_part, int cs_terms,
+                         int64_t M, float* colsum, hipStream_t st) {
+  const int c_blocks = (int)ceil_div(MN >> 2, (int64_t)64);
+  const int cs_blocks = colsum ? (int)ceil_div(M, (int64_t)64) : 0;
+  hipLaunchKernelGGL(tn_reduce_kernel, dim3((unsigned)(c_blocks + cs_blocks)), dim3(256), 0, st, part, splits, MN, alpha, C, accumulate, cs_part, cs_terms,
+                     M, colsum, c_blocks);
+  return check_launch("gemm_bf16_tn_reduce");
+}
+
+static int launch_tn_reduce(const GemmParams& p, int splits, int tiles_n, hipStream_t st, dinox_reduce_seg* defer, int* n_defer) {
   const int64_t MN = p.M * p.N;
-  const int c_blocks = (int)ceil_div(MN >> 2, (int64_t)64);
-  const int cs_blocks = p.colsum ? (int)ceil_div(p.M, (int64_t)64) : 0;
   const float* part = (const float*)p.ws;
-  hipLaunchKernelGGL(tn_reduce_kernel, dim3((unsigned)(c_blocks + cs_blocks)), dim3(256), 0, st, part, splits, MN, p.alpha, (float*)p.C,
-                     (p.epilogue & DINOX_EPI_ACCUM) ? 1 : 0, part + (int64_t)splits * MN, splits * tiles_n, p.M, p.colsum, c_blocks);
-  return check_launch("gemm_bf16_tn_reduce");
+  const int accumulate = (p.epilogue & DINOX_EPI_ACCUM) ? 1 : 0;
+  if (defer) {
+    defer[0] = dinox_reduce_seg{part, (float*)p.C, MN, MN, splits, DINOX_REDUCE_VEC4, p.alpha, accumulate};
+    *n_defer = 1;
+    if (p.colsum) {
+      defer[1] = dinox_reduce_seg{part + (int64_t)splits * MN, p.colsum, p.M, p.M, splits * tiles_n, DINOX_REDUCE_SCALAR4, 1.0f, accumulate};
+      *n_defer = 2;
+    }
+    return 0;
+  }
+  return launch_tn_reduce_raw(part, splits, MN, p.alpha, (float*)p.C, accumulate, part + (int64_t)splits * MN, splits * tiles_n, p.M, p.colsum, st);
 }
 
 static void tn_split_plan(const GemmParams& p, int& splits, int64_t& kps) {
@@ -553,8 +568,9 @@
   return ((int64_t)splits * p.M * p.N + (p.colsum ? (int64_t)splits * tiles_n * p.M : 0)) * (int64_t)sizeof(float);
 }
 
-int launch_gemm_bf16(const GemmParams& p, hipStream_t st) {
+int launch_gemm_bf16(const GemmParams& p, hipStream_t st, dinox_reduce_seg* defer, int* n_defer) {
   using V = GemmVariant;
+  if (defer) *n_defer = 0;
   const V v = gemm_bf16_variant(p);
   switch (v) {
     case V::None: return DINOX_EUNSUPPORTED;
@@ -578,7 +594,7 @@
   if (v == V::TnBig) {
     int sp = 1, tn_ = 1;
     if (int rc = launch_gemm_bf16_tn_big(p, st, sp, tn_)) return rc;
-    return launch_tn_reduce(p, sp, tn_, st);
+    return launch_tn_reduce(p, sp, tn_, st, defer, n_defer);
   }
   int splits;
   int64_t kps;
@@ -604,7 +620,7 @@
   const auto kern = v == V::TnDma ? (f32 ? gemm_bf16_tn_dma<DINOX_F32> : gemm_bf16_tn_dma<DINOX_BF16>) : (f32 ? gemm_bf16_tn<DINOX_F32> : gemm_bf16_tn<DINOX_BF16>);
   hipLaunchKernelGGL(kern, grid, dim3(GB_THREADS), lds, st, q, tiles_m, tiles_n, splits, kps);
   if (int rc = check_launch(gemm_variant_name(v))) return rc;
-  if (det) return launch_tn_reduce(p, splits, tiles_n, st);
+  if (det) return launch_tn_reduce(p, splits, tiles_n, st, defer, n_defer);
   return 0;
 }
 
diff --git a/dino-x_amd/csrc/kernels.h b/dino-x_amd/csrc/kernels.h
--- a/dino-x_amd/csrc/kernels.h
+++ b/dino-x_amd/csrc/kernels.h
@@ -21,7 +21,9 @@
 
 int launch_gemm_f32(const GemmParams& p, hipStream_t st);
 GemmVariant gemm_bf16_variant(const GemmParams& p);
-int launch_gemm_bf16(const GemmParams& p, hipStream_t st);
+int launch_gemm_bf16(const GemmParams& p, hipStream_t st, dinox_reduce_seg* defer = nullptr, int* n_defer = nullptr);
+int launch_tn_reduce_raw(const float* part, int splits, int64_t MN, float alpha, float* C, int accumulate, const float* cs_part, int cs_terms,
+                         int64_t M, float* colsum, hipStream_t st);
 int64_t gemm_bf16_ws_bytes(const GemmParams& p);
 bool gemm_bf16_nt_glds_ok(const GemmParams& p);
 int launch_gemm_bf16_nt_glds(const GemmParams& p, hipStream_t st);
@@ -42,6 +44,8 @@
 int tn_big_plan(const GemmParams& p, int& tiles_m, int& tiles_n, int& splits, int64_t& kps);
 int64_t tn_big_ws_bytes(const GemmParams& p);
 int launch_gemm_bf16_tn_big(const GemmParams& p, hipStream_t st, int& splits_out, int& tiles_n_out);
+
+int launch_reduce_segments(const dinox_reduce_seg* segs, int n_segs, hipStream_t st);
 
 int launch_attention_ref_fwd(const void* qkv, void* o, float* lse, int B, int N, int heads, int d, int dtype, hipStream_t st);
 int launch_attention_ref_bwd(const void* d_o, const void* qkv, const void* o, const float* lse, void* dqkv, int B, int N, int heads, int d, int dtype, hipStream_t st);
diff --git a/dino-x_amd/csrc/layernorm.hip b/dino-x_amd/csrc/layernorm.hip
--- a/dino-x_amd/csrc/layernorm.hip
+++ b/dino-x_amd/csrc/layernorm.hip
@@ -400,6 +400,16 @@
   }
 }
 
+static int ln_reduce(const float* ws, float* dw, float* db, int parts, int dim, int accumulate, dinox_reduce_seg* defer, hipStream_t st, const char* what) {
+  if (defer) {
+    defer[0] = dinox_reduce_seg{ws, dw, dim, 2 * (int64_t)dim, parts, DINOX_REDUCE_MOD64, 1.0f, accumulate};
+    defer[1] = dinox_reduce_seg{ws + dim, db, dim, 2 * (int64_t)dim, parts, DINOX_REDUCE_MOD64, 1.0f, accumulate};
+    return 0;
+  }
+  hipLaunchKernelGGL(ln_bwd_reduce, dim3((unsigned)ceil_div(2 * dim, 4)), dim3(256), 0, st, ws, dw, db, parts, dim, accumulate);
+  return check_launch(what);
+}
+
 static int ln_parts(int64_t rows) {
   int64_t p = ceil_div(rows, LN_THREADS / 64);
   return (int)(p < LN_MAX_PARTS ? p : LN_MAX_PARTS);
@@ -449,9 +459,9 @@
   return (int64_t)ln_parts(rows) * 2 * dim * (int64_t)sizeof(float);
 }
 
-extern "C" int dinox_layernorm_bwd(const void* dy, const float* x, const float* w, const float* mean, const float* rstd,
-                                   float* dx, const float* dx_add, void* dx_lowp, float* dw, float* db, void* ws,
-                                   int64_t rows, int dim, int dy_dtype, int accumulate, void* stream) {
+static int layernorm_bwd_call(const void* dy, const float* x, const float* w, const float* mean, const float* rstd, float* dx, const float* dx_add,
+                              void* dx_lowp, float* dw, float* db, void* ws, int64_t rows, int dim, int dy_dtype, int accumulate,
+                              dinox_reduce_seg* defer, void* stream) {
   DX_REQUIRE(dy && x && w && mean && rstd && dx && dw && db && ws, DINOX_EINVAL, "layernorm_bwd: null pointer");
   DX_REQUIRE(rows > 0 && dim > 0, DINOX_EINVAL, "layernorm_bwd: rows=%lld dim=%d", (long long)rows, dim);
   DX_REQUIRE(dy_dtype == DINOX_F32 || dy_dtype == DINOX_BF16, DINOX_EINVAL, "layernorm_bwd: dtype %d", dy_dtype);
@@ -466,8 +476,7 @@
     const int nblk = (int)(want < parts ? want : (parts < 768 ? parts : 768));
     hipLaunchKernelGGL((dy_dtype == DINOX_F32 ? ln_bwd_384<DINOX_F32> : ln_bwd_384<DINOX_BF16>), dim3(nblk), dim3(LN_THREADS), lds, st, dy, x, w, mean, rstd, dx, dx_lowp, wsf, rows, dx_add);
     if (int rc = check_launch("layernorm_bwd")) return rc;
-    hipLaunchKernelGGL(ln_bwd_reduce, dim3((unsigned)ceil_div(2 * dim, 4)), dim3(256), 0, st, wsf, dw, db, nblk, dim, accumulate ? 1 : 0);
-    return check_launch("layernorm_bwd_reduce");
+    return ln_reduce(wsf, dw, db, nblk, dim, accumulate ? 1 : 0, defer, st, "layernorm_bwd_reduce");
   }
 #define LN_BWD(DT, NV) hipLaunchKernelGGL((ln_bwd_kernel<DT, NV>), dim3(parts), dim3(LN_THREADS), lds, st, dy, x, w, mean, rstd, dx, dx_lowp, wsf, rows, dim, dx_add)
   if (fast) {
@@ -485,24 +494,47 @@
 #undef LN_BWD
   int rc = check_launch("layernorm_bwd");
   if (rc) return rc;
-  hipLaunchKernelGGL(ln_bwd_reduce, dim3((unsigned)ceil_div(2 * dim, 4)), dim3(256), 0, st, wsf, dw, db, parts, dim, accumulate ? 1 : 0);
-  return check_launch("layernorm_bwd_reduce");
+  return ln_reduce(wsf, dw, db, parts, dim, accumulate ? 1 : 0, defer, st, "layernorm_bwd_reduce");
+}
+
+extern "C" int dinox_layernorm_bwd(const void* dy, const float* x, const float* w, const float* mean, const float* rstd,
+                                   float* dx, const float* dx_add, void* dx_lowp, float* dw, float* db, void* ws,
+                                   int64_t rows, int dim, int dy_dtype, int accumulate, void* stream) {
+  return layernorm_bwd_call(dy, x, w, mean, rstd, dx, dx_add, dx_lowp, dw, db, ws, rows, dim, dy_dtype, accumulate, nullptr, stream);
+}
+
+extern "C" int dinox_layernorm_bwd_deferred(const void* dy, const float* x, const float* w, const float* mean, const float* rstd,
+                                            float* dx, const float* dx_add, void* dx_lowp, float* dw, float* db, void* ws,
+                                            int64_t rows, int dim, int dy_dtype, int accumulate, dinox_reduce_seg* segs, void* stream) {
+  DX_REQUIRE(segs, DINOX_EINVAL, "layernorm_bwd_deferred: null segment output");
+  return layernorm_bwd_call(dy, x, w, mean, rstd, dx, dx_add, dx_lowp, dw, db, ws, rows, dim, dy_dtype, accumulate, segs, stream);
 }
 
 extern "C" int dinox_linear_ln_bwd_ok(int64_t M, int N, int K) {
   return (N == 384 && gemm_bf16_nt_pp384_ln_ok(M, K) && pp384_lnbwd_tiles(M) <= ln_parts(M)) ? 1 : 0;
 }
 
-extern "C" int dinox_linear_ln_bwd(const void* a, const void* w, const float* x, const float* gamma, const float* mean, const float* rstd,
-                                   float* dx, const float* dx_add, void* dx_lowp, float* dgamma, float* dbeta, void* ws, int64_t M, int N,
-                                   int K, int accumulate, void* stream) {
+static int linear_ln_bwd_call(const void* a, const void* w, const float* x, const float* gamma, const float* mean, const float* rstd, float* dx,
+                              const float* dx_add, void* dx_lowp, float* dgamma, float* dbeta, void* ws, int64_t M, int N, int K, int accumulate,
+                              dinox_reduce_seg* defer, void* stream) {
   DX_REQUIRE(a && w && x && gamma && mean && rstd && dx && dgamma && dbeta && ws, DINOX_EINVAL, "linear_ln_bwd: null pointer");
   DX_REQUIRE(dinox_linear_ln_bwd_ok(M, N, K), DINOX_EUNSUPPORTED, "linear_ln_bwd: M=%lld N=%d K=%d", (long long)M, N, K);
   DX_REQUIRE((((uintptr_t)a | (uintptr_t)w | (uintptr_t)x | (uintptr_t)dx | (uintptr_t)dx_add | (uintptr_t)dx_lowp | (uintptr_t)gamma) & 15) == 0,
              DINOX_EALIGN, "linear_ln_bwd: operands must be 16-byte aligned");
   hipStream_t st = as_stream(stream);
   if (int rc = launch_gemm_bf16_nt_pp384_lnbwd(a, w, x, gamma, mean, rstd, dx, dx_add, dx_lowp, (float*)ws, M, K, st)) return rc;
-  hipLaunchKernelGGL(ln_bwd_reduce, dim3((unsigned)ceil_div(2 * 384, 4)), dim3(256), 0, st, (const float*)ws, dgamma, dbeta, pp384_lnbwd_tiles(M), 384,
-                     accumulate ? 1 : 0);
-  return check_launch("linear_ln_bwd_reduce");
-}
+  return ln_reduce((const float*)ws, dgamma, dbeta, pp384_lnbwd_tiles(M), 384, accumulate ? 1 : 0, defer, st, "linear_ln_bwd_reduce");
+}
+
+extern "C" int dinox_linear_ln_bwd(const void* a, const void* w, const float* x, const float* gamma, const float* mean, const float* rstd,
+                                   float* dx, const float* dx_add, void* dx_lowp, float* dgamma, float* dbeta, void* ws, int64_t M, int N,
+                                   int K, int accumulate, void* stream) {
+  return linear_ln_bwd_call(a, w, x, gamma, mean, rstd, dx, dx_add, dx_lowp, dgamma, dbeta, ws, M, N, K, accumulate, nullptr, stream);
+}
+
+extern "C" int dinox_linear_ln_bwd_deferred(const void* a, const void* w, const float* x, const float* gamma, const float* mean, const float* rstd,
+                                            float* dx, const float* dx_add, void* dx_lowp, float* dgamma, float* dbeta, void* ws, int64_t M, int N,
+                                            int K, int accumulate, dinox_reduce_seg* segs, void* stream) {
+  DX_REQUIRE(segs, DINOX_EINVAL, "linear_ln_bwd_deferred: null segment output");
+  return linear_ln_bwd_call(a, w, x, gamma, mean, rstd, dx, dx_add, dx_lowp, dgamma, dbeta, ws, M, N, K, accumulate, segs, stream);
+}
diff --git a/dino-x_amd/csrc/reduce_multi.hip b/dino-x_amd/csrc/reduce_multi.hip
--- /dev/null
+++ b/dino-x_amd/csrc/reduce_multi.hip
@@ -0,0 +1,143 @@
+#include <cstring>
+
+#include "common.h"
+#include "kernels.h"
+
+namespace dinox {
+
+struct ReduceTable {
+  dinox_reduce_seg seg[DINOX_REDUCE_MAX_SEGS];
+  int first[DINOX_REDUCE_MAX_SEGS + 1];
+  int n;
+};
+
+__global__ __launch_bounds__(256) void reduce_multi_kernel(const ReduceTable t) {
+  __shared__ float4 red[4][64];
+  const int total = t.first[t.n];
+  for (int unit = blockIdx.x; unit < total; unit += gridDim.x) {
+    int si = 0;
+    while (si + 1 < t.n && t.first[si + 1] <= unit) ++si;
+    const int b = unit - t.first[si];
+    const float* __restrict__ part = t.seg[si].part;
+    float* __restrict__ dst = t.seg[si].dst;
+    const int64_t count = t.seg[si].count, stride = t.seg[si].stride;
+    const int terms = t.seg[si].terms, order = t.seg[si].order, accumulate = t.seg[si].accumulate;
+    const float alpha = t.seg[si].alpha;
+    if (order == DINOX_REDUCE_VEC4) {
+      const int l = threadIdx.x & 63, g = threadIdx.x >> 6;
+      const int64_t n4 = count >> 2, i = (int64_t)b * 64 + l;
+      const int per = (terms + 3) >> 2, s_lo = g * per, s_hi = s_lo + per < terms ? s_lo + per : terms;
+      float4 a = make_float4(0.f, 0.f, 0.f, 0.f);
+      if (i < n4) {
+        for (int s0 = s_lo; s0 < s_hi; s0 += 8) {
+          float4 v[8];
+#pragma unroll
+          for (int u = 0; u < 8; ++u)
+            v[u] = s0 + u < s_hi ? reinterpret_cast<const float4*>(part + (int64_t)(s0 + u) * stride)[i] : make_float4(0.f, 0.f, 0.f, 0.f);
+#pragma unroll
+          for (int u = 0; u < 8; ++u) {
+            a.x += v[u].x; a.y += v[u].y; a.z += v[u].z; a.w += v[u].w;
+          }
+        }
+      }
+      red[g][l] = a;
+      __syncthreads();
+      if (g == 0 && i < n4) {
+        const float4 r0 = red[0][l], r1 = red[1][l], r2 = red[2][l], r3 = red[3][l];
+        float4 c = accumulate ? reinterpret_cast<const float4*>(dst)[i] : make_float4(0.f, 0.f, 0.f, 0.f);
+        c.x += alpha * ((r0.x + r1.x) + (r2.x + r3.x));
+        c.y += alpha * ((r0.y + r1.y) + (r2.y + r3.y));
+        c.z += alpha * ((r0.z + r1.z) + (r2.z + r3.z));
+        c.w += alpha * ((r0.w + r1.w) + (r2.w + r3.w));
+        reinterpret_cast<float4*>(dst)[i] = c;
+      }
+      if (b == 0 && threadIdx.x < (count & 3)) {
+        const int64_t j = (n4 << 2) + threadIdx.x;
+        float s = 0.f;
+        for (int s2 = 0; s2 < terms; ++s2) s += part[(int64_t)s2 * stride + j];
+        dst[j] = (accumulate ? dst[j] : 0.f) + alpha * s;
+      }
+    } else if (order == DINOX_REDUCE_SCALAR4) {
+      const int l = threadIdx.x & 63, g = threadIdx.x >> 6;
+      const int64_t m = (int64_t)b * 64 + l;
+      const int per = (terms + 3) >> 2, t_lo = g * per, t_hi = t_lo + per < terms ? t_lo + per : terms;
+      float a = 0.f;
+      if (m < count) {
+        for (int t0 = t_lo; t0 < t_hi; t0 += 8) {
+          float v[8];
+#pragma unroll
+          for (int u = 0; u < 8; ++u) v[u] = t0 + u < t_hi ? part[(int64_t)(t0 + u) * stride + m] : 0.f;
+#pragma unroll
+          for (int u = 0; u < 8; ++u) a += v[u];
+        }
+      }
+      red[g][l].x = a;
+      __syncthreads();
+      if (g == 0 && m < count) dst[m] = (accumulate ? dst[m] : 0.f) + ((red[0][l].x + red[1][l].x) + (red[2][l].x + red[3][l].x));
+    } else {
+      float* const r = reinterpret_cast<float*>(red);
+      const int cl = threadIdx.x & 3, g = threadIdx.x >> 2;
+      const int64_t c = (int64_t)b * 4 + cl;
+      float s = 0.f;
+      if (c < count)
+        for (int p = g; p < terms; p += 64) s += part[(size_t)p * stride + c];
+      r[g * 4 + cl] = s;
+      __syncthreads();
+      if (g == 0 && c < count) {
+        float v = 0.f;
+#pragma unroll
+        for (int k = 0; k < 64; ++k) v += r[k * 4 + cl];
+        dst[c] = (accumulate ? dst[c] : 0.f) + v;
+      }
+    }
+    __syncthreads();
+  }
+}
+
+static int64_t seg_units(const dinox_reduce_seg& s) {
+  if (s.order == DINOX_REDUCE_VEC4) {
+    const int64_t u = ceil_div(s.count >> 2, (int64_t)64);
+    return u > 0 ? u : 1;
+  }
+  return ceil_div(s.count, (int64_t)(s.order == DINOX_REDUCE_SCALAR4 ? 64 : 4));
+}
+
+int launch_reduce_segments(const dinox_reduce_seg* segs, int n_segs, hipStream_t st) {
+  ReduceTable t;
+  memset(&t, 0, sizeof t);
+  int64_t units = 0;
+  int k = 0;
+  for (int order : {DINOX_REDUCE_MOD64, DINOX_REDUCE_SCALAR4, DINOX_REDUCE_VEC4})
+    for (int i = 0; i < n_segs; ++i) {
+      if (segs[i].order != order) continue;
+      t.seg[k] = segs[i];
+      t.first[k++] = (int)units;
+      units += seg_units(segs[i]);
+      if (units > 0x7fffffff) return fail(DINOX_EINVAL, "reduce_segments: %lld workgroup units", (long long)units);
+    }
+  t.first[k] = (int)units;
+  t.n = k;
+  const int64_t resident = (int64_t)device_cu_count() * 8;
+  hipLaunchKernelGGL(reduce_multi_kernel, dim3((unsigned)(units < resident ? units : resident)), dim3(256), 0, st, t);
+  return check_launch("reduce_segments");
+}
+
+}
+
+using namespace dinox;
+
+extern "C" int dinox_reduce_segments(const dinox_reduce_seg* segs, int n_segs, void* stream) {
+  DX_REQUIRE(segs && n_segs >= 1 && n_segs <= DINOX_REDUCE_MAX_SEGS, DINOX_EINVAL, "reduce_segments: %d segments (1 .. %d)", n_segs,
+             DINOX_REDUCE_MAX_SEGS);
+  for (int i = 0; i < n_segs; ++i) {
+    const dinox_reduce_seg& s = segs[i];
+    DX_REQUIRE(s.part && s.dst && s.count > 0 && s.terms >= 1 && (s.terms == 1 || s.stride >= s.count), DINOX_EINVAL,
+               "reduce_segments: segment %d: part=%p dst=%p count=%lld terms=%d stride=%lld", i, (const void*)s.part, (void*)s.dst,
+               (long long)s.count, s.terms, (long long)s.stride);
+    DX_REQUIRE(s.order == DINOX_REDUCE_VEC4 || s.order == DINOX_REDUCE_SCALAR4 || s.order == DINOX_REDUCE_MOD64, DINOX_EINVAL,
+               "reduce_segments: segment %d: order %d", i, s.order);
+    DX_REQUIRE(s.order != DINOX_REDUCE_VEC4 || ((((uintptr_t)s.part) | ((uintptr_t)s.dst)) & 15) == 0, DINOX_EALIGN,
+               "reduce_segments: segment %d: part and dst of a VEC4 segment must be 16-byte aligned", i);
+  }
+  return launch_reduce_segments(segs, n_segs, as_stream(stream));
+}
diff --git a/dino-x_amd/dinox/_lib.py b/dino-x_amd/dinox/_lib.py
--- a/dino-x_amd/dinox/_lib.py
+++ b/dino-x_amd/dinox/_lib.py
@@ -53,6 +53,13 @@
     ]
 
 
+class ReduceSeg(C.Structure):
+    _fields_ = [("part", vp), ("dst", vp), ("count", i64), ("stride", i64), ("terms", i32), ("order", i32), ("alpha", f32), ("accumulate", i32)]
+
+
+REDUCE_VEC4, REDUCE_SCALAR4, REDUCE_MOD64, REDUCE_MAX_SEGS = 0, 1, 2, 16
+BLOCK_BWD_FUSE_LN, BLOCK_BWD_BATCHED = 1, 2
+
 SIGNATURES = {
     "dinox_version": (i32, []),
     "dinox_last_error": (C.c_char_p, []),
@@ -60,6 +67,9 @@
     "dinox_gemm": (i32, [C.POINTER(GemmArgs), vp]),
     "dinox_gemm_kernel_name": (C.c_char_p, [C.POINTER(GemmArgs)]),
     "dinox_gemm_ws_bytes": (i64, [C.POINTER(GemmArgs)]),
+    "dinox_gemm_deferred": (i32, [C.POINTER(GemmArgs), C.POINTER(ReduceSeg), C.POINTER(C.c_int), vp]),
+    "dinox_reduce_segments": (i32, [C.POINTER(ReduceSeg), i32, vp]),
+    "dinox_split_reduce": (i32, [vp, i32, i64, f32, vp, i32, vp, i32, i64, vp, vp]),
     "dinox_colsum": (i32, [vp, vp, i64, i64, i64, i32, i32, vp]),
     "dinox_linear_residual_ln_ok": (i32, [i64, i32, i32]),
     "dinox_linear_residual_ln": (i32, [vp, vp, vp, vp, vp, vp, vp, f32, vp, i32, vp, vp, i64, i32, i32, vp]),
@@ -68,6 +78,8 @@
     "dinox_layernorm_bwd": (i32, [vp, vp, vp, vp, vp, vp, vp, vp, vp, vp, vp, i64, i32, i32, i32, vp]),
     "dinox_linear_ln_bwd_ok": (i32, [i64, i32, i32]),
     "dinox_linear_ln_bwd": (i32, [vp, vp, vp, vp, vp, vp, vp, vp, vp, vp, vp, vp, i64, i32, i32, i32, vp]),
+    "dinox_layernorm_bwd_deferred": (i32, [vp, vp, vp, vp, vp, vp, vp, vp, vp, vp, vp, i64, i32, i32, i32, C.POINTER(ReduceSeg), vp]),
+    "dinox_linear_ln_bwd_deferred": (i32, [vp, vp, vp, vp, vp, vp, vp, vp, vp, vp, vp, vp, i64, i32, i32, i32, C.POINTER(ReduceSeg), vp]),
     "dinox_attention_fwd": (i32, [vp, vp, vp, i32, i32, i32, i32, i32, vp]),
     "dinox_attention_bwd_ws_bytes": (i64, [i32, i32, i32]),
     "dinox_attention_bwd": (i32, [vp, vp, vp, vp, vp, vp, i32, i32, i32, i32, i32, vp]),
@@ -128,6 +140,8 @@
     "dinox_gelu_bwd": (i32, [vp, vp, vp, i64, vp]),
     "dinox_block_forward": (i32, [C.POINTER(BlockFwdArgs), vp]),
     "dinox_block_backward": (i32, [C.POINTER(BlockBwdArgs), vp]),
+    "dinox_block_backward_tn_ws_bytes": (i64, [i64, i32, i32, i32]),
+    "dinox_block_backward_ln_ws_bytes": (i64, [i64, i32, i32]),
     "dinox_retrieval_ws_bytes": (i64, [i64, i64, i64]),
     "dinox_retrieval_rank": (i32, [vp, i64, vp, i64, vp, i64, i64, i64, vp, vp, vp, vp, vp, vp]),
     "dinox_retrieval_rank_windowed_ws_bytes": (i64, [i64, i64, i64]),
diff --git a/dino-x_amd/dinox/ops.py b/dino-x_amd/dinox/ops.py
--- a/dino-x_amd/dinox/ops.py
+++ b/dino-x_amd/dinox/ops.py
@@ -11,7 +11,7 @@
 import torch
 
 from . import _lib
-from ._lib import BF16, EPI_ACCUM, EPI_AUXGRAD, EPI_BIAS, EPI_DGELU, EPI_GELU, EPI_RESIDUAL, F32, BlockBwdArgs, BlockFwdArgs, GemmArgs, check, lib
+from ._lib import BF16, BLOCK_BWD_BATCHED, BLOCK_BWD_FUSE_LN, EPI_ACCUM, EPI_AUXGRAD, EPI_BIAS, EPI_DGELU, EPI_GELU, EPI_RESIDUAL, F32, BlockBwdArgs, BlockFwdArgs, GemmArgs, check, lib
 
 Tensor = torch.Tensor
 _OVERRIDE: list = []
@@ -876,21 +876,8 @@
     return (x2,) + nxt
 
 
-_BLOCK_TN_WS: dict = {}
-
-
-def _block_tn_ws_bytes(M: int, D: int, H: int) -> int:
-    key = (M, D, H)
-    hit = _BLOCK_TN_WS.get(key)
-    if hit is None:
-        hit = 0
-        for n_out, n_in in ((D, H), (H, D), (D, D), (3 * D, D)):
-            g = GemmArgs(A=0x1000, B=0x1000, C=0x1000, M=n_out, N=n_in, K=M, lda=n_out, ldb=n_in, ldc=n_in, batch=1, strideA=0, strideB=0, strideC=n_out * n_in,
-                         transA=1, transB=1, in_dtype=BF16, out_dtype=F32, epilogue=EPI_ACCUM, alpha=1.0, bias=None, residual=None, ldr=n_in, aux=None,
-                         ldaux=n_in, colsum=0x1000, ws=0x1000)
-            hit = max(hit, int(lib.dinox_gemm_ws_bytes(C.byref(g))))
-        _BLOCK_TN_WS[key] = hit
-    return hit
+def _block_ws_bytes(M: int, D: int, H: int, flags: int):
+    return int(lib.dinox_block_backward_tn_ws_bytes(M, D, H, flags)), int(lib.dinox_block_backward_ln_ws_bytes(M, D, flags))
 
 
 def _block_backward_native(ctx, g: Tensor, saved):
@@ -909,14 +896,16 @@
     g1 = torch.empty((V, N, D), dtype=torch.float32, device=dev)
     g0_lp = bf(V, N, D)
     gp = lambda sl: None if sl is None else sl[1].grad.data_ptr()
-    tn_ws = _tn_workspace(max(_block_tn_ws_bytes(M, D, H), 1), dev)
+    fuse_ln = linear_ln_bwd_ok(M, D, H, dt) and linear_ln_bwd_ok(M, D, 3 * D, dt)
+    flags = (BLOCK_BWD_FUSE_LN if fuse_ln else 0) | BLOCK_BWD_BATCHED
+    tn_bytes, ln_bytes = _block_ws_bytes(M, D, H, flags)
+    tn_ws = _tn_workspace(max(tn_bytes, 1), dev)
     scratch = dict(dpre=bf(M, H), dxn2=bf(M, D), d_o=bf(M, D), dqkv=bf(M, 3 * D), dxn1=bf(M, D), g1_lowp=bf(M, D),
                    g_lowp_buf=None if g_lp is not None else bf(M, D),
                    attn_ws=torch.empty(lib.dinox_attention_bwd_ws_bytes(V, N, heads), dtype=torch.uint8, device=dev),
-                   ln_ws=torch.empty(lib.dinox_layernorm_bwd_ws_bytes(M, D), dtype=torch.uint8, device=dev))
+                   ln_ws=torch.empty(ln_bytes, dtype=torch.uint8, device=dev))
     wts = [weight_operand(w_, dt, transposed=True) for w_ in (wqkv, wproj, w1, w2)]
-    fuse_ln = linear_ln_bwd_ok(M, D, H, dt) and linear_ln_bwd_ok(M, D, 3 * D, dt)
-    a = BlockBwdArgs(V=V, N=N, D=D, H=H, heads=heads, reserved=int(fuse_ln), g=_p(g), g_lowp=_p(g_lp), g_lowp_buf=_p(scratch["g_lowp_buf"]),
+    a = BlockBwdArgs(V=V, N=N, D=D, H=H, heads=heads, reserved=flags, g=_p(g), g_lowp=_p(g_lp), g_lowp_buf=_p(scratch["g_lowp_buf"]),
                      x0=_p(x0), x1=_p(x1), xn1=_p(xn1), xn2=_p(xn2), qkv=_p(qkv), o=_p(o), lse=_p(lse), pre=_p(pre), act=_p(act), mean1=_p(mean1),
                      rstd1=_p(rstd1), mean2=_p(mean2), rstd2=_p(rstd2), n1w=_p(n1w), n2w=_p(n2w),
                      wqkv_t=_p(wts[0]), wproj_t=_p(wts[1]), w1_t=_p(wts[2]), w2_t=_p(wts[3]),
diff --git a/include/dinox.h b/include/dinox.h
--- a/include/dinox.h
+++ b/include/dinox.h
@@ -56,6 +56,26 @@
 int64_t dinox_gemm_ws_bytes(const dinox_gemm_args* args);
 const char* dinox_gemm_kernel_name(const dinox_gemm_args* args);
 
+#define DINOX_REDUCE_VEC4 0
+#define DINOX_REDUCE_SCALAR4 1
+#define DINOX_REDUCE_MOD64 2
+#define DINOX_REDUCE_MAX_SEGS 16
+typedef struct dinox_reduce_seg {
+  const float* part;
+  float* dst;
+  int64_t count;
+  int64_t stride;
+  int32_t terms;
+  int32_t order;
+  float alpha;
+  int32_t accumulate;
+} dinox_reduce_seg;
+
+int dinox_gemm_deferred(const dinox_gemm_args* args, dinox_reduce_seg* segs, int* n_segs, void* stream);
+int dinox_reduce_segments(const dinox_reduce_seg* segs, int n_segs, void* stream);
+int dinox_split_reduce(const float* part, int splits, int64_t MN, float alpha, float* C, int accumulate, const float* cs_part,
+                       int cs_terms, int64_t M, float* colsum, void* stream);
+
 int dinox_colsum(const void* x, float* out, int64_t M, int64_t N, int64_t ldx, int dtype, int accumulate,
                  void* stream);
 
@@ -74,6 +94,12 @@
 int dinox_linear_ln_bwd(const void* a, const void* w, const float* x, const float* gamma, const float* mean, const float* rstd,
                         float* dx, const float* dx_add, void* dx_lowp, float* dgamma, float* dbeta, void* ws, int64_t M, int N,
                         int K, int accumulate, void* stream);
+int dinox_layernorm_bwd_deferred(const void* dy, const float* x, const float* w, const float* mean, const float* rstd,
+                                 float* dx, const float* dx_add, void* dx_lowp, float* dw, float* db, void* ws,
+                                 int64_t rows, int dim, int dy_dtype, int accumulate, dinox_reduce_seg* segs, void* stream);
+int dinox_linear_ln_bwd_deferred(const void* a, const void* w, const float* x, const float* gamma, const float* mean, const float* rstd,
+                                 float* dx, const float* dx_add, void* dx_lowp, float* dgamma, float* dbeta, void* ws, int64_t M, int N,
+                                 int K, int accumulate, dinox_reduce_seg* segs, void* stream);
 
 int dinox_attention_fwd(const void* qkv, void* o, float* lse, int B, int N, int heads, int d, int dtype,
                         void* stream);
@@ -226,6 +252,10 @@
 
 int dinox_block_forward(const dinox_block_fwd_args* args, void* stream);
 int dinox_block_backward(const dinox_block_bwd_args* args, void* stream);
+#define DINOX_BLOCK_BWD_FUSE_LN 1
+#define DINOX_BLOCK_BWD_BATCHED 2
+int64_t dinox_block_backward_tn_ws_bytes(int64_t M, int D, int H, int flags);
+int64_t dinox_block_backward_ln_ws_bytes(int64_t M, int D, int flags);
 
 int64_t dinox_retrieval_ws_bytes(int64_t Nq, int64_t Nk, int64_t D);
 int dinox_retrieval_rank(const float* q, int64_t ldq, const float* k, int64_t ldk, const int32_t* target, int64_t Nq, int64_t Nk, int64_t D,
```

After: 7286 samples/s. Within noise of the previous version (-0.1%).
